# chto/linna

Hardware: AMD Instinct MI355X
Metric: emulator log-likelihood evals/sec (higher is better)
Workload: dtype f32; 1 GPU; 33-D Gaussian, 4x512 MLP emulator (33->512x4->33), nwalkers=4096 batched log-likelihood per GPU (BASELINE configs[1]); nwalkers_per_gpu=4096, launch=direct launches, parallelism=walkers sharded, 1 rank(s), no data-path collective

## Files before the change

### include/linna_hip.h

```cpp
#ifndef LINNA_HIP_H
#define LINNA_HIP_H
#include <stddef.h>
#include <stdint.h>

#ifdef __cplusplus
extern "C" {
#endif

#define LINNA_ABI_VERSION 12

typedef struct linna_ctx linna_ctx_t;
typedef struct linna_net linna_net_t;
typedef struct linna_logprob linna_logprob_t;
typedef struct linna_graph linna_graph_t;

int linna_abi_version(void);
const char* linna_last_error(void);
#define LINNA_OK 0
#define LINNA_ERR_INVALID (-1)
#define LINNA_ERR_HIP (-2)
#define LINNA_ERR_UNSUPPORTED (-3)
#define LINNA_ERR_INTERNAL (-4)
int linna_debug_raise(int kind);
int linna_ctx_create(int device, linna_ctx_t** out);
// ... 57 lines not shown
int linna_resblock_fwd(linna_ctx_t* ctx, const float* X, int ldx, const float* W1, const float* b1,
                       const float* W2, const float* b2, const float* Ws, float* T, int ldt,
                       float* Y, int ldy, int B, int K, int C, int N, void* stream);
int linna_linear_bwd(linna_ctx_t* ctx, const float* dY, int lddy, const float* X, int ldx,
                     const float* W, int ldw, float* dX, int lddx, const float* Xmask, int ldxm,
                     float* dW, int lddw, float* db, int B, int K, int N, float scale, void* stream);

#define LINNA_LD(k) (((k) + 3) & ~3)
#define LINNA_OP_LINEAR 0
#define LINNA_OP_RESBLOCK 1
#define LINNA_OP_INSKIP 2

typedef struct {
    uint32_t struct_size;
    int op;
    int K, C, N;
    int relu;
    float alpha;
    const float *W, *b;
    const float *W1, *b1, *W2, *b2, *Ws;
    float *gW, *gb, *gW1, *gb1, *gW2, *gb2, *gWs;
} linna_layer_t;

typedef struct {
    const float* cscale; const float* cshift;
    int cexp; const float* cpost; const float* cshift2;
} linna_colmap_t;

int linna_net_create(linna_ctx_t* ctx, const linna_layer_t* layers, int nlayers, int in_size,
                     linna_net_t** out);
int linna_net_destroy(linna_net_t* net);
int linna_net_prepare(linna_net_t* net, int backward, int input_grad);
size_t linna_net_fwd_ws_bytes(const linna_net_t* net, int B);
size_t linna_net_bwd_ws_bytes(const linna_net_t* net, int B);
int linna_net_forward(linna_net_t* net, const float* X, int ldx, int B, void* ws, float* OUT, int ldo,
                      const linna_colmap_t* outmap, void* stream);
int linna_net_backward(linna_net_t* net, const float* X, int ldx, int B, void* fwd_ws, void* bwd_ws,
                       const float* dOUT, int lddo, float* dX, int lddx, int param_grads, void* stream);
int linna_net_train_launches(const linna_net_t* net, int B);
int linna_net_set_train_precision(linna_net_t* net, int precision);
int linna_net_train_precision(const linna_net_t* net, int* out);
int linna_net_stream_state(const linna_net_t* net, int* fwd, int* dx, int* dx_input);

int linna_prior_map_fwd(linna_ctx_t* ctx, const float* Z, int ldz, int B, int nin, const int* is_flat,
                        const float* a1, const float* a2, const int* log10_flag, const float* xmean,
                        const float* xstd, float* X, int ldx, float* THETA, int ldt, void* stream);
int linna_prior_map_bwd(linna_ctx_t* ctx, const float* Z, int ldz, int B, int nin, const int* is_flat,
                        const float* a1, const float* a2, const int* log10_flag, const float* xstd,
                        const float* dX, int lddx, float* dZ, int lddz, void* stream);

int linna_gauss_loglike_diag(linna_ctx_t* ctx, const float* D, int ldd, int B, int nout, const float* w,
                             const float* Z, int ldz, int nin, float temperature, float* out,
                             void* stream);
int linna_gauss_loglike_dense(linna_ctx_t* ctx, const float* D, int ldd, int B, int nout,
                              const float* S, int lds, const float* Z, int ldz, int nin,
                              float temperature, float* scratch, float* out, void* stream);

typedef struct {
    uint32_t struct_size;
    int nin, nout;
    const int* is_flat; const float* a1; const float* a2;
    const int* log10_flag; const float* xmean; const float* xstd;
    linna_colmap_t outmap;
    const float* S; int lds;
    const float* Ssym;
    const float* w;
    const float* gscale;
    float temperature;
    const float* Sfac;
} linna_logprob_desc_t;

int linna_logprob_create(linna_ctx_t* ctx, linna_net_t* net, const linna_logprob_desc_t* desc,
                         linna_logprob_t** out);
int linna_logprob_destroy(linna_logprob_t* lp);
int linna_weights_changed(linna_ctx_t* ctx);
#define LINNA_PRECISION_FP32 0
#define LINNA_PRECISION_BF16 1
int linna_logprob_set_precision(linna_logprob_t* lp, int precision);
int linna_logprob_precision(const linna_logprob_t* lp, int* out);
int linna_logprob_set_grad_precision(linna_logprob_t* lp, int precision);
int linna_logprob_grad_precision(const linna_logprob_t* lp, int* out);
int linna_engine_rows(int rows);
int linna_dense_tri(int mode);
int linna_slice_fusion(int mask);
int linna_program_describe(const linna_layer_t* layers, int nlayers, int in_size, int rows, int dense_nout, char* buf,
                           size_t n);
int linna_program_describe_grad_bf16(const linna_layer_t* layers, int nlayers, int in_size, int rows, char* buf, size_t n);
size_t linna_logprob_ws_bytes(const linna_logprob_t* lp, int B, int with_grad);
int linna_logprob_eval(linna_logprob_t* lp, const float* Z, int ldz, int B, void* ws, float* lnP,
                       float* THETA, int ldt, void* stream);
int linna_logprob_eval_if(linna_logprob_t* lp, const float* Z, int ldz, int B, void* ws, float* lnP,
                          float* THETA, int ldt, const int* gate, void* stream);
int linna_logprob_eval_slice_points(linna_logprob_t* lp, const float* coords, int ldc, int ndim, const int* S_idx,
                                    int ns, const float* DIR, int ldd, const float* w, int nrep, float* lnP,
                                    const int* gate, void* stream);
int linna_logprob_grad(linna_logprob_t* lp, const float* Z, int ldz, int B, void* ws, float* lnP,
                       float* G, int ldg, void* stream);
int linna_logprob_grad_leapfrog(linna_logprob_t* lp, float* Q, int ldq, int B, void* ws, float* lnP, float* G, int ldg,
                                float* P, int ldp, const float* mass, float eps_kick, float eps_drift, void* stream);

typedef struct {
    uint32_t struct_size;
    int nout;
    const float* sigma; const float* ymean; const float* ystd;
    const float* data_norm;
    const float* Cinv; int ldc;
    int ylog;
} linna_loss_desc_t;

size_t linna_loss_scratch_bytes(int B, int nout);
int linna_chi2_md(linna_ctx_t* ctx, const linna_loss_desc_t* d, const float* Y, int ldy, int nrows,
                  float* scratch, float* den, void* stream);
int linna_chi2_ratio_loss_fwd_bwd(linna_ctx_t* ctx, const linna_loss_desc_t* d, const float* PRED,
                                  int ldp, const float* Y, int ldy, const float* den, const int* ROWS,
                                  int B, float* scratch, float* loss_rows, float* loss_mean,
                                  float* dPRED, int lddp, float inv_batch, void* stream);
int linna_net_prepare_loss(linna_net_t* net, const linna_loss_desc_t* d);
int linna_loss_targets(linna_ctx_t* ctx, const linna_loss_desc_t* d, const float* Y, int ldy, int nrows, float* YN, int ldyn,
                       void* stream);
int linna_net_forward_loss(linna_net_t* net, const linna_loss_desc_t* d, const float* X, int ldx, const int* ROWS, int B,
                           const int* log10_flag, const float* xmean, const float* xstd, float* XB, int ldxb, void* ws,
                           float* PRED, int ldp, const float* YN, int ldyn, const float* den, float inv_batch,
                           float* loss_rows, float* loss_mean, float* dPRED, int lddp,
                           float* hyper, int* step_dev, float beta1, float beta2, void* stream);
int linna_net_train_step(linna_net_t* net, const linna_loss_desc_t* d, const float* X, int ldx, const int* ROWS, int B,
                         const int* log10_flag, const float* xmean, const float* xstd, float* XB, int ldxb, void* fwd_ws,
                         float* PRED, int ldp, const float* YN, int ldyn, const float* den, float inv_batch,
                         float* loss_rows, float* loss_mean, float* dPRED, int lddp, void* bwd_ws,
                         float* hyper, int* step_dev, float beta1, float beta2, void* stream);
int linna_val_rows(linna_ctx_t* ctx, const linna_loss_desc_t* d, const float* PRED, int ldp,
                   const float* Y, int ldy, const float* den, int B, float* scratch, float* loss_rows,
                   float* frac_rows, void* stream);
int linna_val_metrics(linna_ctx_t* ctx, const float* loss_rows, const float* frac_rows, int n, const float* last_train_loss,
                      float* out, void* stream);
int linna_gather_xform(linna_ctx_t* ctx, const float* X, int ldx, const int* ROWS, int B, int nin,
                       const int* log10_flag, const float* xmean, const float* xstd, float* XB, int ldxb,
                       void* stream);
int linna_adamw_step(linna_ctx_t* ctx, float* p, const float* g, float* m, float* v, size_t n,
                     float* hyper, int* step_dev, float beta1, float beta2, float eps,
                     int prepared ,
                     void* stream);
int linna_net_adamw_step(linna_net_t* net, int B, float* p, const float* g, float* m, float* v, size_t n,
                         float* hyper, int* step_dev, float beta1, float beta2, float eps, int prepared, void* stream);
int linna_net_train_step_update(linna_net_t* net, const linna_loss_desc_t* d, const float* X, int ldx, const int* ROWS, int B,
                                const int* log10_flag, const float* xmean, const float* xstd, float* XB, int ldxb,
                                void* fwd_ws, float* PRED, int ldp, const float* YN, int ldyn, const float* den,
                                float inv_batch, float* loss_rows, float* loss_mean, float* dPRED, int lddp, void* bwd_ws,
                                float* params, float* m, float* v, size_t n, float* hyper, int* step_dev, float beta1,
                                float beta2, float eps, void* stream);

int linna_stretch_propose(linna_ctx_t* ctx, const float* coords, int ldc, int ndim, const int* S_idx,
                          int ns, const float* ccoords, int ldcc, const int* C_idx, int nc, uint64_t seed,
                          const int* step_dev, int stream_id, float a, float* Q, int ldq, float* factors,
                          void* stream);
int linna_stretch_accept(linna_ctx_t* ctx, float* coords, int ldc, int ndim, float* logp,
                         const int* S_idx, int ns, const float* Q, int ldq, const float* logp_new,
                         const float* factors, uint64_t seed, const int* step_dev, int stream_id,
                         int* naccept, void* stream);
int linna_stretch_half_step(linna_logprob_t* lp, float* coords, int ldc, int ndim, float* logp,
                            const int* S_idx, int ns, const float* ccoords, int ldcc, const int* C_idx,
                            int nc, uint64_t seed, const int* step_dev, int step_offset, int stream_id,
                            float a, int* naccept, void* stream);
int linna_hmc_init(linna_ctx_t* ctx, int B, int ndim, const float* mass, uint64_t seed,
                   const int* step_dev, const float* lnp, const float* P0, int ldp0, float* P, int ldp,
                   float* H0, void* stream);
int linna_hmc_start(linna_ctx_t* ctx, int B, int ndim, const float* mass, uint64_t seed, const int* step_dev,
// ... 102 lines not shown
```

### linna_amd/_lib.py

```python
import ctypes as C
import os

import torch

_HERE = os.path.dirname(os.path.abspath(__file__))
LIB_PATH = os.environ.get("LINNA_LIB_PATH") or os.path.join(_HERE, "liblinna_hip.so")
ABI_VERSION = 12

c_float_p = C.c_void_p
c_int_p = C.c_void_p


class _Sized(C.Structure):

    def __init__(self, *a, **k):
        C.Structure.__init__(self, *a, **k)
        self.struct_size = C.sizeof(type(self))


def sized_array(cls, n):
    arr = (cls * n)()
    for i in range(n):
        arr[i].struct_size = C.sizeof(cls)
    return arr
# ... 21 lines not shown
                ("gW", C.c_void_p), ("gb", C.c_void_p), ("gW1", C.c_void_p), ("gb1", C.c_void_p),
                ("gW2", C.c_void_p), ("gb2", C.c_void_p), ("gWs", C.c_void_p)]


class ColMap(C.Structure):
    _fields_ = [("cscale", C.c_void_p), ("cshift", C.c_void_p), ("cexp", C.c_int), ("cpost", C.c_void_p),
                ("cshift2", C.c_void_p)]


class LogprobDesc(_Sized):
    _fields_ = [("struct_size", C.c_uint32), ("nin", C.c_int), ("nout", C.c_int), ("is_flat", C.c_void_p), ("a1", C.c_void_p), ("a2", C.c_void_p),
                ("log10_flag", C.c_void_p), ("xmean", C.c_void_p), ("xstd", C.c_void_p), ("outmap", ColMap),
                ("S", C.c_void_p), ("lds", C.c_int), ("Ssym", C.c_void_p), ("w", C.c_void_p), ("gscale", C.c_void_p),
                ("temperature", C.c_float), ("Sfac", C.c_void_p)]


class HmcState(_Sized):
    _fields_ = [("struct_size", C.c_uint32), ("B", C.c_int), ("ld", C.c_int), ("seed", C.c_uint64), ("step_dev", C.c_void_p),
                ("mass", C.c_void_p), ("X", C.c_void_p), ("lnp", C.c_void_p), ("G", C.c_void_p), ("P", C.c_void_p),
                ("Q", C.c_void_p), ("lnp_new", C.c_void_p), ("Gnew", C.c_void_p), ("H0", C.c_void_p)]


class LossDesc(_Sized):
    _fields_ = [("struct_size", C.c_uint32), ("nout", C.c_int), ("sigma", C.c_void_p), ("ymean", C.c_void_p), ("ystd", C.c_void_p),
                ("data_norm", C.c_void_p), ("Cinv", C.c_void_p), ("ldc", C.c_int), ("ylog", C.c_int)]


OP_LINEAR, OP_RESBLOCK, OP_INSKIP = 0, 1, 2
COMM_ID_BYTES = 128
LAY_K, LAY_MN = 0, 1

_V, _I, _F, _SZ, _U64 = C.c_void_p, C.c_int, C.c_float, C.c_size_t, C.c_uint64
_I64, _D = C.c_int64, C.c_double
_PV = C.POINTER(C.c_void_p)

_SIGNATURES = {
    "linna_abi_version": (_I, []),
    "linna_last_error": (C.c_char_p, []),
    "linna_debug_raise": (_I, [_I]),
    "linna_ctx_create": (_I, [_I, _PV]),
    "linna_ctx_destroy": (_I, [_V]),
    "linna_stream_sync": (_I, [_V]),
    "linna_graph_begin": (_I, [_V]),
    "linna_graph_end": (_I, [_V, _PV]),
    "linna_graph_launch": (_I, [_V, _V]),
    "linna_graph_destroy": (_I, [_V]),
    "linna_event_create": (_I, [_PV]),
    "linna_event_record": (_I, [_V, _V]),
    "linna_event_elapsed_ms": (_I, [_V, _V, C.POINTER(C.c_float)]),
    "linna_event_destroy": (_I, [_V]),
    "linna_comm_unique_id": (_I, [_V]),
    "linna_comm_init": (_I, [_V, _I, _I, _V]),
    "linna_comm_destroy": (_I, [_V]),
    "linna_comm_info": (_I, [_V, C.POINTER(C.c_int), C.POINTER(C.c_int), C.POINTER(C.c_int)]),
    "linna_allreduce_sum_f32": (_I, [_V, _V, _SZ, _V]),
    "linna_allgather_f32": (_I, [_V, _V, _V, _SZ, _V]),
    "linna_broadcast_f32": (_I, [_V, _V, _SZ, _I, _V]),
    "linna_gemm_f32": (_I, [_V, C.POINTER(Gemm), _V]),
    "linna_gemm_dot_slots": (_I, [_I, _I]),
    "linna_linear_fwd": (_I, [_V, _V, _I, _V, _I, _V, _V, _I, _I, _I, _I, _I, _F, _V, _I, _V]),
    "linna_resblock_fwd": (_I, [_V, _V, _I, _V, _V, _V, _V, _V, _V, _I, _V, _I, _I, _I, _I, _I, _V]),
    "linna_linear_bwd": (_I, [_V, _V, _I, _V, _I, _V, _I, _V, _I, _V, _I, _V, _I, _V, _I, _I, _I, _F, _V]),
    "linna_net_create": (_I, [_V, C.POINTER(Layer), _I, _I, _PV]),
    "linna_net_destroy": (_I, [_V]),
    "linna_net_prepare": (_I, [_V, _I, _I]),
    "linna_net_fwd_ws_bytes": (_SZ, [_V, _I]),
    "linna_net_bwd_ws_bytes": (_SZ, [_V, _I]),
    "linna_net_forward": (_I, [_V, _V, _I, _I, _V, _V, _I, C.POINTER(ColMap), _V]),
    "linna_net_backward": (_I, [_V, _V, _I, _I, _V, _V, _V, _I, _V, _I, _I, _V]),
    "linna_net_stream_state": (_I, [_V, _V, _V, _V]),
    "linna_prior_map_fwd": (_I, [_V, _V, _I, _I, _I, _V, _V, _V, _V, _V, _V, _V, _I, _V, _I, _V]),
    "linna_prior_map_bwd": (_I, [_V, _V, _I, _I, _I, _V, _V, _V, _V, _V, _V, _I, _V, _I, _V]),
    "linna_gauss_loglike_diag": (_I, [_V, _V, _I, _I, _I, _V, _V, _I, _I, _F, _V, _V]),
    "linna_gauss_loglike_dense": (_I, [_V, _V, _I, _I, _I, _V, _I, _V, _I, _I, _F, _V, _V, _V]),
    "linna_logprob_create": (_I, [_V, _V, C.POINTER(LogprobDesc), _PV]),
    "linna_logprob_destroy": (_I, [_V]),
    "linna_weights_changed": (_I, [_V]),
    "linna_logprob_set_precision": (_I, [_V, _I]),
    "linna_logprob_precision": (_I, [_V, _V]),
    "linna_logprob_set_grad_precision": (_I, [_V, _I]),
    "linna_logprob_grad_precision": (_I, [_V, _V]),
    "linna_engine_rows": (_I, [_I]),
    "linna_dense_tri": (_I, [_I]),
    "linna_slice_fusion": (_I, [_I]),
    "linna_net_train_launches": (_I, [_V, _I]),
    "linna_net_set_train_precision": (_I, [_V, _I]),
    "linna_net_train_precision": (_I, [_V, _V]),
    "linna_program_describe": (_I, [_V, _I, _I, _I, _I, _V, C.c_size_t]),
    "linna_program_describe_grad_bf16": (_I, [_V, _I, _I, _I, _V, C.c_size_t]),
    "linna_logprob_ws_bytes": (_SZ, [_V, _I, _I]),
    "linna_logprob_eval": (_I, [_V, _V, _I, _I, _V, _V, _V, _I, _V]),
    "linna_logprob_grad": (_I, [_V, _V, _I, _I, _V, _V, _V, _I, _V]),
    "linna_logprob_grad_leapfrog": (_I, [_V, _V, _I, _I, _V, _V, _V, _I, _V, _I, _V, _F, _F, _V]),
    "linna_loss_scratch_bytes": (_SZ, [_I, _I]),
    "linna_chi2_md": (_I, [_V, C.POINTER(LossDesc), _V, _I, _I, _V, _V, _V]),
    "linna_chi2_ratio_loss_fwd_bwd": (_I, [_V, C.POINTER(LossDesc), _V, _I, _V, _I, _V, _V, _I, _V, _V, _V, _V, _I, _F, _V]),
    "linna_net_prepare_loss": (_I, [_V, C.POINTER(LossDesc)]),
    "linna_loss_targets": (_I, [_V, C.POINTER(LossDesc), _V, _I, _I, _V, _I, _V]),
    "linna_net_forward_loss": (_I, [_V, C.POINTER(LossDesc), _V, _I, _V, _I, _V, _V, _V, _V, _I, _V, _V, _I, _V, _I, _V, _F, _V, _V, _V, _I,
                                    _V, _V, _F, _F, _V]),
    "linna_net_train_step": (_I, [_V, C.POINTER(LossDesc), _V, _I, _V, _I, _V, _V, _V, _V, _I, _V, _V, _I, _V, _I, _V, _F, _V, _V, _V, _I,
                                  _V, _V, _V, _F, _F, _V]),
    "linna_net_train_step_update": (_I, [_V, C.POINTER(LossDesc), _V, _I, _V, _I, _V, _V, _V, _V, _I, _V, _V, _I, _V, _I, _V, _F, _V, _V, _V, _I,
                                         _V, _V, _V, _V, _SZ, _V, _V, _F, _F, _F, _V]),
    "linna_val_rows": (_I, [_V, C.POINTER(LossDesc), _V, _I, _V, _I, _V, _I, _V, _V, _V, _V]),
    "linna_val_metrics": (_I, [_V, _V, _V, _I, _V, _V, _V]),
    "linna_gather_xform": (_I, [_V, _V, _I, _V, _I, _I, _V, _V, _V, _V, _I, _V]),
    "linna_adamw_step": (_I, [_V, _V, _V, _V, _V, _SZ, _V, _V, _F, _F, _F, _I, _V]),
    "linna_net_adamw_step": (_I, [_V, _I, _V, _V, _V, _V, _SZ, _V, _V, _F, _F, _F, _I, _V]),
    "linna_stretch_propose": (_I, [_V, _V, _I, _I, _V, _I, _V, _I, _V, _I, _U64, _V, _I, _F, _V, _I, _V, _V]),
    "linna_stretch_accept": (_I, [_V, _V, _I, _I, _V, _V, _I, _V, _I, _V, _V, _U64, _V, _I, _V, _V]),
    "linna_logprob_eval_if": (_I, [_V, _V, _I, _I, _V, _V, _V, _I, _V, _V]),
    "linna_logprob_eval_slice_points": (_I, [_V, _V, _I, _I, _V, _I, _V, _I, _V, _I, _V, _V, _V]),
    "linna_stretch_half_step": (_I, [_V, _V, _I, _I, _V, _V, _I, _V, _I, _V, _I, _U64, _V, _I, _I, _F, _V, _V]),
    "linna_stretch_run": (_I, [_V, _V, _I, _I, _V, _I, _V, _I, _I, _U64, _V, _I, _F, _V, _V, _V, _V]),
    "linna_chain_append_t": (_I, [_V, _V, _I, _I, _I, _I, _I, _V, _I, _I64, _V]),
    "linna_acorr_update": (_I, [_V, _V, _I, _I, _I, _I64, _I64, _I64, _I64, _I, _I, _V, _V, _I, _V]),
    "linna_acorr_scratch_bytes": (_SZ, [_I, _I, _I]),
    "linna_acorr_tau": (_I, [_V, _V, _I, _I, _I, _I, _I64, _I64, _I, _V, _V, _D, _V, _V, _V]),
    "linna_chain_meanstd": (_I, [_V, _V, _I, _I, _I, _I64, _I64, _I64, _V, _V]),
    "linna_hmc_init": (_I, [_V, _I, _I, _V, _U64, _V, _V, _V, _I, _V, _I, _V, _V]),
    "linna_hmc_start": (_I, [_V, _I, _I, _V, _U64, _V, _V, _V, _I, _V, _I, _F, _F, _V, _I, _V, _I, _V, _I, _V, _V]),
    "linna_hmc_kick_drift": (_I, [_V, _I, _I, _V, _F, _F, _V, _I, _V, _I, _V, _I, _V]),
    "linna_hmc_accept": (_I, [_V, _I, _I, _V, _U64, _V, _V, _V, _I, _V, _I, _V, _V, _I, _V, _V, _I, _V, _V, _V, _V]),
    "linna_hmc_start_eps": (_I, [_V, _I, _I, _V, _U64, _V, _I, _V, _V, _I, _V, _I, _V, _F, _F, _V, _I, _V, _I, _V, _I, _V, _V]),
    "linna_hmc_kick_drift_eps": (_I, [_V, _I, _I, _V, _V, _F, _F, _V, _I, _V, _I, _V, _I, _V]),
    "linna_logprob_grad_leapfrog_eps": (_I, [_V, _V, _I, _I, _V, _V, _V, _I, _V, _I, _V, _V, _F, _F, _V]),
    "linna_hmc_accept_adapt": (_I, [_V, _I, _I, _V, _U64, _V, _I, _V, _V, _I, _V, _I, _V, _V, _I, _V, _V, _I, _V, _V, _V, _V,
                                    _V, _V, _V, _V, _V, _I, _F, _V, _V, _V]),
    "linna_hmc_run": (_I, [_V, _V, _V, _V, _V, _V, _V, _V, _I, _F, _I, _I, _I, _V, _V, _V, _V, _V]),
    "linna_hmc_find_epsilon": (_I, [_V, _V, _V, _V, _V, _V, _V, _I, _I, _V]),
    "linna_hmc_moments": (_I, [_V, _I, _I, _V, _I, _V, _V]),
    "linna_hmc_mass_from_moments": (_I, [_V, _I, _V, _V, _I, _V]),
    "linna_hmc_run_moments": (_I, [_V, _V, _V, _V, _V, _V, _V, _V, _I, _F, _I, _I, _I, _V, _V, _V, _V, _V, _V]),
    "linna_hmc_comoments_doubles": (_SZ, [_I]),
    "linna_hmc_comoments": (_I, [_V, _I, _I, _V, _I, _V, _V]),
    "linna_hmc_chol_from_comoments": (_I, [_V, _I, _V, _V, _I, _V, _I, _V]),
    "linna_hmc_kick_drift_dense": (_I, [_V, _I, _I, _V, _I, _V, _F, _F, _V, _I, _V, _I, _V, _I, _V, _I, _V]),
    "linna_hmc_run_dense": (_I, [_V, _V, _V, _V, _I, _V, _V, _V, _V, _V, _I, _F, _I, _I, _I, _V, _V, _V, _V, _V, _V]),
    "linna_hmc_find_epsilon_dense": (_I, [_V, _V, _V, _V, _I, _V, _V, _V, _V, _I, _I, _V]),
    "linna_step_increment": (_I, [_V, _V, _V]),
    "linna_slice_init": (_I, [_V, _V, _V, _I, _V, _I, _V, _I, _I, _V, _U64, _V, _I, _V, _I, _V, _V, _V, _V, _I, _V]),
    "linna_slice_points": (_I, [_V, _V, _I, _I, _V, _I, _V, _I, _V, _V, _I, _I, _V]),
    "linna_slice_expand": (_I, [_V, _V, _V, _V, _V, _V, _V, _I, _V, _I, _V]),
    "linna_slice_draw": (_I, [_V, _V, _V, _V, _V, _V, _I, _U64, _V, _I, _I, _I, _V]),
    "linna_slice_shrink": (_I, [_V, _V, _V, _V, _V, _V, _V, _V, _V, _I, _V, _I, _I, _V]),
    "linna_slice_commit": (_I, [_V, _V, _I, _I, _V, _V, _I, _V, _I, _V, _V, _V]),
    "linna_slice_half_step": (_I, [_V, _V, _I, _I, _V, _V, _I, _V, _I, _V, _I, _V, _U64, _V, _I, _V, _I, _V, _I, _V, _I, _V, _V, _V, _V, _V, _V, _V, _I, _I, _V, _I, _V]),
}
EXPORTED = tuple(_SIGNATURES)

_lib = None


class LinnaHipError(RuntimeError):
    pass


def load(missing_ok=False):
    global _lib
    if _lib is not None:
        return _lib
    if not os.path.exists(LIB_PATH):
        raise LinnaHipError("liblinna_hip.so not found at %s -- run `python -c 'import __graft_entry__ as g; g.build()'` "
                            "(hipcc --offload-arch=gfx950); there is no CPU fallback" % LIB_PATH)
    lib = C.CDLL(LIB_PATH)
# ... 45 lines not shown

def ptr(t, dtype=torch.float32):
    if t is None:
        return None
    if not t.is_cuda:
        raise LinnaHipError("expected a device tensor")
    if t.dtype != dtype:
        raise LinnaHipError("expected dtype %s, got %s" % (dtype, t.dtype))
    if not t.is_contiguous():
        raise LinnaHipError("expected a contiguous tensor")
    return C.c_void_p(t.data_ptr())


def iptr(t):
    return ptr(t, torch.int32)


def ld4(w):
    return (int(w) + 3) & ~3


class _Stage(object):
    __slots__ = ("name", "t0")

    def __init__(self, name):
        self.name = name

    def __enter__(self):
        if stage_profile.current is not None:
            import time
            self.t0 = time.perf_counter()
        return self

    def __exit__(self, *exc):
        d = stage_profile.current
        if d is not None:
            import time
            d[self.name] = d.get(self.name, 0.0) + time.perf_counter() - self.t0
        return False


def stage(name):
    return _Stage(name)


class stage_profile(object):
    current = None

    def __init__(self, d):
        self.d = d

    def __enter__(self):
        self.prev, stage_profile.current = stage_profile.current, self.d
        return self.d

    def __exit__(self, *exc):
        stage_profile.current = self.prev
        return False


class quiet_gc(object):

    def __enter__(self):
        import gc
        self.on = gc.isenabled() and os.environ.get("LINNA_QUIET_GC", "1") != "0"
        if self.on:
            gc.freeze()
        return self

    def __exit__(self, *exc):
        import gc
        if self.on:
            gc.unfreeze()
        return False


def slice_fusion(mask=-1):
    prev = load().linna_slice_fusion(int(mask))
    if prev < 0:
        check(prev)
    return prev


def engine_rows(rows=0):
    prev = load().linna_engine_rows(int(rows))
    if prev < 0:
        check(prev)
    return prev
```

### linna_amd/csrc/api.hip

```cpp
#include "common.h"

#include <stdarg.h>
#include <stdio.h>
#include <string.h>
#include <cstring>
#include <string>
#include <vector>
#include <atomic>
#include <new>
#include <stdlib.h>

namespace linna {

static thread_local std::string g_err;

void set_error(const char* fmt, ...) {
    char buf[512];
    va_list ap;
    va_start(ap, fmt);
    vsnprintf(buf, sizeof buf, fmt, ap);
    va_end(ap);
    g_err = buf;
}

// ... 820 lines not shown
    a.M = B; a.N = nout; a.dotwith = D; a.lddot = ldd; a.dot_partial = scratch; a.dot_slots = slots;
    if (cov.factored) a.flags |= LINNA_GEMM_DOT_SELF;
    TRY(gemm_launch(a, S(stream)));
    return launch_loglike_finish(scratch, slots, slots, B, Z, ldz, nin, T, out, S(stream));
}
int linna_gauss_loglike_dense(linna_ctx_t*, const float* D, int ldd, int B, int nout, const float* Sm, int lds,
                              const float* Z, int ldz, int nin, float T, float* scratch, float* out, void* stream) try {
    return loglike_dense_impl(D, ldd, B, nout, NsDense{Sm, lds, nullptr, nullptr}, Z, ldz, nin, T, scratch, out, stream);
} LINNA_CATCH_INT

}

struct linna_logprob {
    linna_ctx* ctx;
    linna_net* net;
    linna_logprob_desc_t d;
    StreamCopy packed;
    bool grad_fused = false;
    StreamCopy packed_g2;
    bool grad2 = false;
    bool dense_fused = false;
    bool fused_on = true;
    int dense_tri = 2;
    NsDense dense() const { return NsDense{d.Sfac ? d.Sfac : d.S, d.lds, d.outmap.cscale, d.outmap.cshift, d.Sfac ? 1 : 0, dense_tri}; }
    int precision = LINNA_PRECISION_FP32;
    StreamCopy packed_bf;
    bool bf16() const { return precision == LINNA_PRECISION_BF16; }
    int grad_precision = LINNA_PRECISION_FP32;
    StreamCopy packed_gbf;
    NsKind kind() const { return bf16() ? NS_SERVE_BF16 : dense_fused ? NS_SERVE_DENSE : NS_SERVE; }
};

struct LpLayout { size_t x0, fwd, d, part, dh, bwd, dx, total; int slots; };
static LpLayout lp_layout(const linna_logprob* lp, int B, int with_grad) {
    LpLayout L;
    size_t off = 0;
    auto take = [&](size_t nfloats) { size_t o = off; off += (nfloats + 3) & ~(size_t)3; return o; };
    L.x0 = take((size_t)B * ld4(lp->d.nin));
    L.fwd = take(linna_net_fwd_ws_bytes(lp->net, B) / sizeof(float));
    L.d = take((size_t)B * ld4(lp->d.nout));
    L.slots = gemm_slots(B, lp->d.nout);
    L.part = take((size_t)B * L.slots);
    L.dh = L.bwd = L.dx = 0;
    if (with_grad) {
        L.dh = take((size_t)B * ld4(lp->d.nout));
        L.bwd = take(linna_net_bwd_ws_bytes(lp->net, B) / sizeof(float));
        L.dx = take((size_t)B * ld4(lp->d.nin));
    }
    L.total = off;
    return L;
}

static int lp_refresh_stream(linna_logprob* lp, int B, void* stream, const float** packed, int* rows) {
    *rows = net_stream_rows(B);
    const NsDense dn = lp->dense();
    return stream_copy_refresh(lp->bf16() ? lp->packed_bf : lp->packed, lp->net, *rows, stream, packed, lp->kind(),
                               lp->kind() == NS_SERVE_DENSE ? &dn : nullptr);
}
static NsInput lp_input(const linna_logprob_desc_t& d) { return NsInput{d.nin, d.is_flat, d.a1, d.a2, d.log10_flag, d.xmean, d.xstd}; }
static NsOutput lp_output(const linna_logprob* lp) {
    const linna_logprob_desc_t& d = lp->d;
    if (lp->kind() == NS_SERVE_DENSE) return NsOutput{nullptr, nullptr, nullptr, nullptr, nullptr, d.temperature};
    return NsOutput{d.outmap.cscale, d.outmap.cshift, d.outmap.cexp ? d.outmap.cpost : nullptr, d.outmap.cexp ? d.outmap.cshift2 : nullptr,
                    d.w, d.temperature};
}
struct LpRun { const float* Z; int ldz; int B; float* lnP; const int* gate = nullptr; float* TH = nullptr; int ldt = 0; float* D = nullptr; int ldd = 0; };
static int lp_launch(const linna_logprob* lp, const float* packed, int rows, const LpRun& r, const NsMove* mv, const NsGrad* gr, void* stream) {
    const NsDense dn = lp->dense();
    return launch_net_stream(lp->kind(), net_layers(lp->net, lp->kind()), packed, r.Z, r.ldz, r.B, lp_input(lp->d), lp_output(lp), r.lnP, r.D,
                             r.ldd, r.TH, r.ldt, mv, gr, r.gate, rows, lp->kind() == NS_SERVE_DENSE ? &dn : nullptr, S(stream));
}
static bool lp_runs_fused_move(const linna_logprob* lp) {
    const linna_logprob_desc_t& d = lp->d;
    return lp->fused_on && (lp->bf16() ? lp->packed_bf.ready() : lp->packed.ready()) &&
           !(d.outmap.cexp && (!d.w || !d.outmap.cpost || !d.outmap.cshift2)) && (d.w || lp->dense_fused) && d.nin <= 64;
}
static int lp_likelihood(const linna_logprob* lp, const LpRun& r, float* w, const LpLayout& L, void* stream) {
    const linna_logprob_desc_t& d = lp->d;
    const int ldd = ld4(d.nout);
    if (d.w) return launch_loglike_diag(w + L.d, ldd, r.B, d.nout, d.w, r.Z, r.ldz, d.nin, d.temperature, r.lnP, S(stream));
    return loglike_dense_impl(w + L.d, ldd, r.B, d.nout, lp->dense(), r.Z, r.ldz, d.nin, d.temperature, w + L.part, r.lnP, stream);
}

static int lp_forward(linna_logprob* lp, const LpRun& r, float* w, const LpLayout& L, void* stream, bool keep_activations) {
    const linna_logprob_desc_t& d = lp->d;
    const int ldx = ld4(d.nin), ldd = ld4(d.nout), B = r.B;
    if (lp->bf16()) {
        if (keep_activations || !lp->fused_on || !lp->packed_bf.ready() || !d.w || (d.outmap.cexp && (!d.outmap.cpost || !d.outmap.cshift2))) {
            set_error("logprob: this bf16 log-probability cannot run the whole-network kernel here (LINNA_DISABLE_FUSED, or no diagonal likelihood)");
            return LINNA_ERR_UNSUPPORTED;
        }
        const float* packed = nullptr; int rows = 16;
        TRY(lp_refresh_stream(lp, B, stream, &packed, &rows));
        return lp_launch(lp, packed, rows, r, nullptr, nullptr, stream);
    }
    if (!keep_activations && lp->fused_on && lp->packed.ready() && (!d.outmap.cexp || (d.outmap.cpost && d.outmap.cshift2 && !lp->dense_fused))) {
        const float* packed = nullptr; int rows = 16;
        TRY(lp_refresh_stream(lp, B, stream, &packed, &rows));
        if (lp->dense_fused) return lp_launch(lp, packed, rows, r, nullptr, nullptr, stream);
        TRY(lp_launch(lp, packed, rows, LpRun{r.Z, r.ldz, B, d.w ? r.lnP : nullptr, r.gate, r.TH, r.ldt, d.w ? nullptr : w + L.d, ldd}, nullptr, nullptr, stream));
        return d.w ? LINNA_OK : lp_likelihood(lp, r, w, L, stream);
    }
    TRY(launch_prior_map_fwd(r.Z, r.ldz, B, d.nin, d.is_flat, d.a1, d.a2, d.log10_flag, d.xmean, d.xstd, w + L.x0, ldx, r.TH, r.ldt, S(stream)));
    TRY(linna_net_forward(lp->net, w + L.x0, ldx, B, w + L.fwd, w + L.d, ldd, &d.outmap, stream));
    return lp_likelihood(lp, r, w, L, stream);
}

extern "C" {

int linna_logprob_create(linna_ctx_t* ctx, linna_net_t* net, const linna_logprob_desc_t* desc, linna_logprob_t** out) try {
    if (!net || !desc || !out) { set_error("logprob_create: null argument"); return LINNA_ERR_INVALID; }
    CHECK_STRUCT(desc, linna_logprob_desc_t, "logprob_create");
    if (desc->nin != net->in_size || desc->nout != net->out_size) {
        set_error("logprob_create: network is %d->%d, descriptor says %d->%d", net->in_size, net->out_size, desc->nin, desc->nout);
        return LINNA_ERR_INVALID;
    }
    if (!desc->w && !desc->S) { set_error("logprob_create: need S (dense) or w (diagonal)"); return LINNA_ERR_INVALID; }
    if (!(desc->temperature > 0.f)) { set_error("logprob_create: temperature must be > 0"); return LINNA_ERR_INVALID; }
    linna_logprob* lp = new linna_logprob{ctx, net, *desc};
    lp->dense_tri = net_stream_dense_tri(-1);
    lp->fused_on = !env_is("LINNA_DISABLE_FUSED", '1');
    const NsDense dn = lp->dense();
    const bool want_dense = !desc->w && desc->S && !desc->outmap.cexp && !env_is("LINNA_DENSE_FUSED", '0');
    const NsPlan dense = want_dense ? net_stream_plan(NS_SERVE_DENSE, net->Lfull.data(), (int)net->Lfull.size(), net->in_size, &dn)
                                    : NsPlan{false, 0, false, nullptr};
    const NsPlan serve = net_stream_plan(NS_SERVE, net->Lfull.data(), (int)net->Lfull.size(), net->in_size);
    if (dense.ok) {
        lp->dense_fused = true;
        if (lp->packed.alloc(dense.packed_floats) != LINNA_OK) {
            set_error("logprob_create: hipMalloc(weight stream) failed");
            delete lp; return LINNA_ERR_HIP;
        }
    } else if (serve.ok) {
        lp->grad_fused = serve.grad_ok && !desc->outmap.cexp && !env_is("LINNA_DISABLE_FUSED_GRAD", '1');
        if (lp->packed.alloc(serve.packed_floats) != LINNA_OK) {
            set_error("logprob_create: hipMalloc(weight stream) failed");
            delete lp; return LINNA_ERR_HIP;
        }
    }
    if (!lp->grad_fused && desc->w && desc->gscale && !desc->outmap.cexp && !net->has_inskip && !env_is("LINNA_DISABLE_FUSED_GRAD", '1')) {
        const NsPlan g2 = net_stream_plan(NS_GRAD_INPUT, net->L.data(), (int)net->L.size(), net->in_size);
        if (g2.ok && lp->packed_g2.alloc(g2.packed_floats) == LINNA_OK) lp->grad2 = true;
    }
    *out = lp;
    return LINNA_OK;
} LINNA_CATCH_INT
int linna_logprob_destroy(linna_logprob_t* lp) try {
    if (lp) { lp->packed.release(); lp->packed_g2.release(); lp->packed_bf.release(); lp->packed_gbf.release(); }
    delete lp;
    return LINNA_OK;
} LINNA_CATCH_INT
int linna_weights_changed(linna_ctx_t*) try { g_weights_epoch.fetch_add(1); return LINNA_OK; } LINNA_CATCH_INT
int linna_logprob_set_precision(linna_logprob_t* lp, int precision) try {
    if (!lp) { set_error("logprob_set_precision: null handle"); return LINNA_ERR_INVALID; }
    TRY(check_precision(precision, "logprob_set_precision"));
    if (precision == LINNA_PRECISION_FP32) { lp->precision = precision; lp->grad_precision = LINNA_PRECISION_FP32; return LINNA_OK; }
    const linna_net* n = lp->net;
    if (!lp->d.w) { set_error("logprob_set_precision: bf16 needs a diagonal likelihood (a dense covariance is served in fp32 only)"); return LINNA_ERR_UNSUPPORTED; }
    const NsPlan bf = net_stream_plan(NS_SERVE_BF16, n->Lfull.data(), (int)n->Lfull.size(), n->in_size);
    if (!bf.ok) {
        set_error("logprob_set_precision: no bf16 engine for this network: %s", bf.why ? bf.why : "not eligible");
        return LINNA_ERR_UNSUPPORTED;
    }
    if (!lp->packed_bf.ready() && lp->packed_bf.alloc(bf.packed_floats) != LINNA_OK) {
        set_error("logprob_set_precision: hipMalloc(bf16 weight stream) failed");
        return LINNA_ERR_HIP;
    }
    lp->precision = precision;
    return LINNA_OK;
} LINNA_CATCH_INT
int linna_logprob_precision(const linna_logprob_t* lp, int* out) try {
    if (!lp || !out) { set_error("logprob_precision: null argument"); return LINNA_ERR_INVALID; }
    *out = lp->precision;
    return LINNA_OK;
} LINNA_CATCH_INT
int linna_logprob_set_grad_precision(linna_logprob_t* lp, int precision) try {
    if (!lp) { set_error("logprob_set_grad_precision: null handle"); return LINNA_ERR_INVALID; }
    TRY(check_precision(precision, "logprob_set_grad_precision"));
    if (precision == LINNA_PRECISION_FP32) { lp->grad_precision = precision; return LINNA_OK; }
    if (!lp->bf16()) {
        set_error("logprob_set_grad_precision: a bf16 gradient needs a bf16 handle (linna_logprob_set_precision first): lnP has one surface per handle");
        return LINNA_ERR_INVALID;
    }
    const linna_net* n = lp->net;
    if (lp->d.outmap.cexp) { set_error("logprob_set_grad_precision: no bf16 gradient: the ypositive (exp) output map has no gradient path"); return LINNA_ERR_UNSUPPORTED; }
    if (!lp->d.w || !lp->d.gscale) { set_error("logprob_set_grad_precision: no bf16 gradient: it needs a diagonal likelihood with gscale"); return LINNA_ERR_UNSUPPORTED; }
    const NsPlan g = net_stream_plan(NS_GRAD_INPUT_BF16, n->Lfull.data(), (int)n->Lfull.size(), n->in_size);
    if (!g.ok) {
        set_error("logprob_set_grad_precision: no bf16 gradient for this network: %s", g.why ? g.why : "not eligible");
        return LINNA_ERR_UNSUPPORTED;
    }
    if (!lp->packed_gbf.ready() && lp->packed_gbf.alloc(g.packed_floats) != LINNA_OK) {
        set_error("logprob_set_grad_precision: hipMalloc(bf16 gradient weight stream) failed");
        return LINNA_ERR_HIP;
    }
    lp->grad_precision = precision;
    return LINNA_OK;
} LINNA_CATCH_INT
int linna_logprob_grad_precision(const linna_logprob_t* lp, int* out) try {
    if (!lp || !out) { set_error("logprob_grad_precision: null argument"); return LINNA_ERR_INVALID; }
    *out = lp->grad_precision;
    return LINNA_OK;
} LINNA_CATCH_INT
int linna_program_describe_grad_bf16(const linna_layer_t* layers, int nlayers, int in_size, int rows, char* buf, size_t n) try {
    if (!layers || nlayers < 1 || !buf || !n) { set_error("program_describe_grad_bf16: bad arguments"); return LINNA_ERR_INVALID; }
    TRY(check_layers(layers, nlayers, "program_describe_grad_bf16"));
    return net_stream_describe(NS_GRAD_INPUT_BF16, layers, nlayers, in_size, nullptr, rows, buf, n);
} LINNA_CATCH_INT
int linna_program_describe(const linna_layer_t* layers, int nlayers, int in_size, int rows, int dense_nout, char* buf, size_t n) try {
    if (!layers || nlayers < 1 || !buf || !n) { set_error("program_describe: bad arguments"); return LINNA_ERR_INVALID; }
    TRY(check_layers(layers, nlayers, "program_describe"));
    static float dummy;
    if (dense_nout == -1) return net_stream_describe(NS_GRAD_INPUT, layers, nlayers, in_size, nullptr, rows, buf, n);
    const int dn_cols = dense_nout < -1 ? -dense_nout : dense_nout;
    NsDense dn{&dummy, (dn_cols + 3) & ~3, nullptr, nullptr, dense_nout < -1 ? 1 : 0, net_stream_dense_tri(-1)};
    if (dn_cols > 0) return net_stream_describe(NS_SERVE_DENSE, layers, nlayers, in_size, &dn, rows, buf, n);
    return net_stream_describe(NS_SERVE, layers, nlayers, in_size, nullptr, rows, buf, n);
} LINNA_CATCH_INT
int linna_dense_tri(int mode) try {
    if (mode < -1 || mode > 2) { set_error("linna_dense_tri: %d (-1 query, 0, 1 or 2)", mode); return LINNA_ERR_INVALID; }
    return net_stream_dense_tri(mode);
} LINNA_CATCH_INT
static std::atomic<int> g_slice_fusion{7};
static bool slice_derive_enabled() { return (g_slice_fusion.load() & 1) != 0; }
int linna_slice_fusion(int mode) try {
    if (mode < -1 || mode > 7) { set_error("linna_slice_fusion: %d (-1 query, or a mask of bits 0-2)", mode); return LINNA_ERR_INVALID; }
    return mode < 0 ? g_slice_fusion.load() : g_slice_fusion.exchange(mode);
} LINNA_CATCH_INT
int linna_engine_rows(int rows) try {
    const int prev = net_stream_force_rows(rows);
    if (prev < 0) { set_error("linna_engine_rows: %d (0, 4, 8 or 16)", rows); return LINNA_ERR_INVALID; }
    if (prev != rows) g_weights_epoch.fetch_add(1);
    return prev;
} LINNA_CATCH_INT
size_t linna_logprob_ws_bytes(const linna_logprob_t* lp, int B, int with_grad) try {
    return (lp_layout(lp, B, with_grad).total + 16) * sizeof(float);
} LINNA_CATCH_SIZE

int linna_logprob_eval(linna_logprob_t* lp, const float* Z, int ldz, int B, void* ws, float* lnP, float* TH, int ldt,
                       void* stream) try {
    if (!lp || !Z || !ws || !lnP || B < 1) { set_error("logprob_eval: bad arguments"); return LINNA_ERR_INVALID; }
    return lp_forward(lp, LpRun{Z, ldz, B, lnP, nullptr, TH, ldt}, static_cast<float*>(ws), lp_layout(lp, B, 0), stream, false);
} LINNA_CATCH_INT

int linna_logprob_eval_if(linna_logprob_t* lp, const float* Z, int ldz, int B, void* ws, float* lnP, float* TH, int ldt,
                          const int* gate, void* stream) try {
    if (!lp || !Z || !ws || !lnP || B < 1) { set_error("logprob_eval_if: bad arguments"); return LINNA_ERR_INVALID; }
    return lp_forward(lp, LpRun{Z, ldz, B, lnP, gate, TH, ldt}, static_cast<float*>(ws), lp_layout(lp, B, 0), stream, false);
} LINNA_CATCH_INT

struct SliceDerive { const float* Z0; const float* L; const float* R; const float* Ze; int m, nt; uint64_t seed; const int* step_dev; int stream_id; const int* flags; };
struct SlicePoints { const float* coords; int ldc, ndim; const int* S_idx; int ns; const float* DIR; int ldd; };
static int lp_eval_slice_points(linna_logprob_t* lp, const SlicePoints& pt, const float* w, int nrep, float* lnP, const int* gate,
                                const int* list, const int* count, int mul, int b_engine, void* stream, const SliceDerive* sd = nullptr,
                                const SliceBegin* sb = nullptr) {
    if (!lp || !pt.coords || !pt.S_idx || !pt.DIR || !w || !lnP || pt.ns < 1 || nrep < 1) {
        set_error("logprob_eval_slice_points: bad arguments"); return LINNA_ERR_INVALID;
    }
    if (pt.ndim != lp->d.nin) { set_error("logprob_eval_slice_points: ndim %d, log-probability has %d parameters", pt.ndim, lp->d.nin); return LINNA_ERR_INVALID; }
    if (!lp_runs_fused_move(lp)) {
        set_error("logprob_eval_slice_points: this log-probability does not run the whole-network kernel");
        return LINNA_ERR_UNSUPPORTED;
    }
    const float* packed = nullptr; int rows = 16;
    TRY(lp_refresh_stream(lp, b_engine > 0 ? b_engine : nrep * pt.ns, stream, &packed, &rows));
    NsMove mv{const_cast<float*>(pt.coords), pt.ldc, nullptr, pt.S_idx, w, 0, list, pt.ns, 0ull, count, mul, 0, 0.f, nullptr, 1};
    mv.sb = sb;
    if (sd) {
        mv.sl_Z0 = sd->Z0; mv.sl_L = sd->L; mv.sl_R = sd->R; mv.sl_Zt = sd->Ze; mv.sl_m = sd->m; mv.sl_nt = sd->nt;
        mv.sl_seed = sd->seed; mv.sl_step = sd->step_dev; mv.sl_stream = sd->stream_id; mv.sl_flags = sd->flags;
    }
    return lp_launch(lp, packed, rows, LpRun{pt.DIR, pt.ldd, nrep * pt.ns, lnP, gate}, &mv, nullptr, stream);
}
int linna_logprob_eval_slice_points(linna_logprob_t* lp, const float* coords, int ldc, int ndim, const int* S_idx, int ns,
                                    const float* DIR, int ldd, const float* w, int nrep, float* lnP, const int* gate,
                                    void* stream) try {
    return lp_eval_slice_points(lp, SlicePoints{coords, ldc, ndim, S_idx, ns, DIR, ldd}, w, nrep, lnP, gate, nullptr, nullptr, 0, 0, stream);
} LINNA_CATCH_INT

int linna_slice_half_step(linna_logprob_t* lp, float* coords, int ldc, int ndim, float* logp, const int* S_idx, int ns,
                          const float* ccoords, int ldcc, const int* C_idx, int nc, const float* mu, uint64_t seed,
                          int* step_dev, int half, const int* m_sched, int nexp_rounds, const int* nt_sched, int nshr_rounds,
                          float* DIR, int ldd, float* state, int* flags, float* W, float* Wd, float* Zt, int* list, int* counters,
                          int zero_totals, int bump_step, const int* expect_rows, int maxsteps, void* stream) try {
    if (!lp || !coords || !logp || !S_idx || !ccoords || !C_idx || !mu || !step_dev || !DIR || !state || !flags || !W || !Wd ||
        !Zt || !list || !counters || ns < 1 || nc < 2 || !m_sched || !nt_sched || nexp_rounds < 1 || nshr_rounds < 1 || (half != 0 && half != 1)) {
        set_error("slice_half_step: bad arguments"); return LINNA_ERR_INVALID;
    }
    if (maxsteps < 1) { set_error("slice_half_step: maxsteps %d < 1", maxsteps); return LINNA_ERR_INVALID; }
    for (int r = 0; r < nexp_rounds; ++r)
        if (m_sched[r] < 1 || m_sched[r] > 32) { set_error("slice_half_step: m_sched[%d] = %d (1 to 32 bracket ends per side)", r, m_sched[r]); return LINNA_ERR_INVALID; }
    for (int r = 0; r < nshr_rounds; ++r)
        if (nt_sched[r] < 1 || nt_sched[r] > 64) { set_error("slice_half_step: nt_sched[%d] = %d (1 to 64 trials)", r, nt_sched[r]); return LINNA_ERR_INVALID; }
    if (ndim != lp->d.nin) { set_error("slice_half_step: ndim %d, log-probability has %d parameters", ndim, lp->d.nin); return LINNA_ERR_INVALID; }
    if (!lp_runs_fused_move(lp)) {
        set_error("slice_half_step: this log-probability does not run the whole-network kernel");
        return LINNA_ERR_UNSUPPORTED;
    }
    float* const Z0 = state; float* const L = state + ns; float* const R = state + 2 * ns;
    float* const Wacc = state + 3 * ns; float* const Zacc = state + 4 * ns;
// ... 610 lines not shown
```

### linna_amd/csrc/common.h

```cpp
#pragma once
#include <hip/hip_runtime.h>
#include <stdint.h>
#include <exception>
#include "../../include/linna_hip.h"


typedef float f32x4 __attribute__((ext_vector_type(4)));
typedef float f32x16 __attribute__((ext_vector_type(16)));

namespace linna {

struct U4 { uint32_t x, y, z, w; };
__device__ __forceinline__ U4 philox4x32_10(U4 c, uint32_t k0, uint32_t k1) {
#pragma unroll
    for (int r = 0; r < 10; ++r) {
        const uint64_t p0 = (uint64_t)0xD2511F53u * c.x;
        const uint64_t p1 = (uint64_t)0xCD9E8D57u * c.z;
        U4 n;
        n.x = (uint32_t)(p1 >> 32) ^ c.y ^ k0;
        n.y = (uint32_t)p1;
        n.z = (uint32_t)(p0 >> 32) ^ c.w ^ k1;
        n.w = (uint32_t)p0;
        c = n;
        k0 += 0x9E3779B9u; k1 += 0xBB67AE85u;
// ... 201 lines not shown
                            float* dP, int lddp, unsigned* counter, hipStream_t s);
int launch_loss_rows(int mode, const float* partial, int slots_ld, int nslots, int B, const float* den, const int* ROWS,
                     float floorv, float* out, hipStream_t s);
int launch_loss_grad(const float* U, int ldu, const float* Y, int ldy, const int* ROWS, int B, int nout,
                     const float* data_norm, const float* den, float inv_batch, float* dP, int lddp, hipStream_t s);
int launch_sum_scale(const float* v, int n, float scale, float* out, hipStream_t s);
int launch_sum_scale_prepare(const float* v, int n, float scale, float* out, int* step_dev, float* hyper, float b1, float b2,
                             hipStream_t s);
int launch_val_frac(const float* partial, int slots_ld, int nslots, int B, const float* den, float* frac, hipStream_t s);
int launch_val_metrics(const float* loss, const float* frac, int n, const float* last, float* out, hipStream_t s);
int launch_gather_xform(const float* X, int ldx, const int* ROWS, int B, int nin, const int* lg, const float* xmean,
                        const float* xstd, float* XB, int ldxb, hipStream_t s);
int launch_colsum(const float* dZ, int ld, int B, int N, float scale, float* db, hipStream_t s);
int launch_adamw(float* p, const float* g, float* m, float* v, size_t n, float* hyper, int* step_dev, float b1, float b2,
                 float eps, hipStream_t s);
int launch_adamw_prepare(float* hyper, int* step_dev, float b1, float b2, hipStream_t s);
int launch_stretch_propose(const float* coords, int ldc, int ndim, const int* S, int ns, const float* ccoords, int ldcc,
                           const int* C, int nc, uint64_t seed, const int* step_dev, int stream_id, float a, float* Q,
                           int ldq, float* factors, hipStream_t s);
int launch_stretch_accept(float* coords, int ldc, int ndim, float* logp, const int* S, int ns, const float* Q, int ldq,
                          const float* lp_new, const float* factors, uint64_t seed, const int* step_dev, int stream_id,
                          int* naccept, hipStream_t s);
int launch_hmc_start(int B, int ndim, const float* mass, uint64_t seed, const int* step_dev, const float* lnp, const float* P0,
                     int ldp0, const float* G, int ldg, float ek, float ed, const float* X, int ldx, float* P, int ldp, float* Q,
                     int ldq, float* H0, hipStream_t s, const float* eps = nullptr, int step_off = 0);
int launch_hmc_kick_drift(int B, int ndim, const float* mass, float ek, float ed, const float* G, int ldg, float* P,
                          int ldp, float* Q, int ldq, hipStream_t s, const float* eps = nullptr);
struct HmcAdapt { float* eps; float* epsbar; float* Hbar; const float* mu; int* m; int Madapt; float delta; };
int launch_hmc_accept(int B, int ndim, const float* mass, uint64_t seed, const int* step_dev, int step_off, const float* H0,
                      const float* P, int ldp, const float* Qn, int ldq, const float* lnp_new, const float* Gn, int ldg,
                      const float* U, float* X, int ldx, float* lnp, float* G, int* naccept, float* alpha,
                      const HmcAdapt& ad, float* chain, float* logps, hipStream_t s);
int launch_hmc_find_eps_init(int B, int ndim, uint64_t seed, const int* step_dev, int step_off, float* R0, int ldr, float* eps,
                             int* state, hipStream_t s);
int launch_hmc_find_eps(int B, int ndim, const float* mass, const float* H0, const float* P, int ldp, const float* lnp_new,
                        const float* Gn, int ldg, float* eps, int* state, int* nactive, hipStream_t s);
int launch_hmc_moments(int B, int ndim, const float* X, int ldx, double* mom, hipStream_t s);
int launch_hmc_mass_from_moments(int ndim, double* mom, float* mass, int reset, hipStream_t s);
int launch_hmc_comoments(int B, int ndim, const float* X, int ldx, double* mom, hipStream_t s);
int launch_hmc_chol_from_comoments(int ndim, double* mom, float* Cm, int ldc, int* info, int reset, hipStream_t s);
int launch_hmc_kick_drift_dense(int B, int ndim, const float* Cm, int ldc, const float* eps, float ek, float ed, const float* G,
                                int ldg, float* W, int ldw, const float* X, int ldx, float* Q, int ldq, hipStream_t s);
int launch_slice_points(const float* coords, int ldc, int ndim, const int* S, int ns, const float* DIR, int ldd,
                        const float* w, float* Q, int ldq, int nrep, hipStream_t s);
int launch_slice_expand(const float* Z0, const float* ZL, const float* ZR, float* L, float* R, int* flags, int ns,
                        int* counters, int slot, hipStream_t s);
int launch_slice_draw(const float* L, const float* R, const int* S, float* W, const int* flags, int ns, uint64_t seed,
                      const int* step_dev, int stream_id, int round, int ntrial, hipStream_t s);
int launch_slice_shrink(const float* Z0, const float* Zt, float* L, float* R, const float* W, int* flags, float* Wacc,
                        float* Zacc, int ns, int* counters, int slot, int ntrial, hipStream_t s);
int launch_slice_begin(const SliceBegin& b, const int* S, int ns, int ndim, float* W, hipStream_t s);
int launch_slice_expand_multi(const float* Z0, const float* Zt, float* L, float* R, const int* S, int* flags, int ns, int m,
                              int m_next, int* counters, int slot, int prev_slot, float* W, float* Wd, int* list, uint64_t seed,
                              const int* step_dev, int stream_id_shrink, int ntrial, hipStream_t s);
int launch_slice_shrink_multi(const SliceRound& a, hipStream_t s);
int launch_slice_commit(float* coords, int ldc, int ndim, float* logp, const int* S, int ns, const float* DIR, int ldd,
                        const float* Wacc, const float* Zacc, hipStream_t s);
int launch_step_increment(int* step, hipStream_t s);

struct NsDense { const float* S; int lds; const float* cscale; const float* cshift; int factored = 0;
                 int tri = 2; };
int net_stream_dense_tri(int mode);
enum NsKind {
    NS_SERVE,
    NS_SERVE_DENSE,
    NS_SERVE_BF16,
    NS_STORE,
    NS_TRAIN_FWD,
    NS_DX,
    NS_DX_INPUT,
    NS_GRAD_INPUT,
    NS_TRAIN_STEP,
    NS_TRAIN_STEP_BF16,
    NS_GRAD_INPUT_BF16,
};
inline bool ns_kind_full_layers(NsKind k) { return k == NS_SERVE || k == NS_SERVE_DENSE || k == NS_SERVE_BF16; }
struct NsPlan { bool ok; size_t packed_floats; bool grad_ok; const char* why; };
NsPlan net_stream_plan(NsKind kind, const linna_layer_t* layers, int nl, int in_size, const NsDense* dn = nullptr);
int net_stream_rows(int B);
int net_stream_force_rows(int rows);
int launch_net_stream_pack(NsKind kind, const linna_layer_t* layers, int nl, int in_size, float* packed, int rows, const NsDense* dn,
                           hipStream_t s);
int net_stream_describe(NsKind kind, const linna_layer_t* layers, int nl, int in_size, const NsDense* dn, int rows, char* buf, size_t n);
struct NsNet { const linna_layer_t* layers; int nl, in_size; };
struct NsInput { int nin; const int* is_flat; const float* a1; const float* a2; const int* lg; const float* xmean; const float* xstd; };
struct NsOutput { const float* cscale; const float* cshift; const float* cpost; const float* cshift2; const float* w; float T; };
struct NsOpBufs { float* y; int ldy; float* t; int ldt; const float* x; int ldx; const float* gate; float* dprev; int ldp; float* dt; int lddt; };
struct NsPost { const float* rows; int n; float scale; float* out; int* step; float* hyper; float b1, b2; };
int launch_net_stream_dx(const NsNet& net, const float* packed, const float* dOUT, int lddo, int B, const NsOpBufs* ops, int with_input,
                         int rows, hipStream_t s, const NsPost* post = nullptr);
struct NsMove {
    float* coords; int ldc; float* logp; const int* S;
    const float* cc; int ldcc; const int* C; int nc;
    unsigned long long seed; const int* step; int step_off; int stream; float a; int* naccept;
    int slice;
    float* chain = nullptr; float* lps = nullptr;
    const float* sl_Z0 = nullptr; const float* sl_L = nullptr; const float* sl_R = nullptr; const float* sl_Zt = nullptr;
    int sl_m = 0, sl_nt = 0; unsigned long long sl_seed = 0; const int* sl_step = nullptr; int sl_stream = 0;
    const int* sl_flags = nullptr;
    const SliceBegin* sb = nullptr;
};
int launch_net_stream_store(const NsNet& net, const float* packed, const float* X, int ldx, int B, const NsOpBufs* ops,
                            const float* cscale, const float* cshift, int rows, hipStream_t s);
struct NsTrainLoss { const float* YN; int ldyn;
                     const float* den; float inv_batch; float* loss_rows; float* dP; int lddp; };
struct NsBatch { const float* X; int ldx; const int* ROWS; int B; const int* lg; const float* xmean; const float* xstd; float* XB; int ldxb; };
int launch_loss_targets(const float* Y, int ldy, int n, const linna_loss_desc_t& d, float* YN, int ldyn, hipStream_t s);
int launch_net_stream_train(const NsNet& net, const float* packed, const NsBatch& b, const NsOpBufs* ops, const NsTrainLoss& L,
                            const NsDense& dn, int rows, hipStream_t s);
int launch_net_stream_train_bwd(const NsNet& net, const float* packed, const NsBatch& b, const NsOpBufs* ops, const NsTrainLoss& L,
                                const NsDense& dn, int rows, hipStream_t s, const NsPost* post,
                                bool bf = false);
struct NsLeap { float* P; int ldp; float* Q; const float* mass; float ek, ed; const float* eps; };
struct NsGrad { const float* gscale; float* G; int ldg; NsLeap leap; };
constexpr int AS_MAXR = 26, AS_MAXW = 14, AS_MAXB = 12;
struct AsPlace { float* out; float scale; int trans, koff, ncols, type, ncg, steps, G, first0, first1; };
struct AsMat { int N, ld; AsPlace pl[2]; };
struct AsBias { float* out; float scale; int N; };
struct AsRange { unsigned off4, n4, blk0; short kind, idx; };
struct AsArgs { AsRange r[AS_MAXR]; AsMat w[AS_MAXW]; AsBias b[AS_MAXB]; int nr, small; unsigned nblocks; };
__device__ __forceinline__ size_t as_slot(const AsPlace& q, int small, int nn, int kk) {
    const int nl = nn & 63, ks = kk >> 4, kr = kk & 15;
    int w, g;
    if (q.type == 0) { w = (nn & 511) >> 6; g = ((nn >> 9) ? q.first1 : q.first0) + ks; }
    else { const int kp = ks / q.steps; w = kp * q.ncg + (nn >> 6); g = q.first0 + (ks - kp * q.steps); }
    const int t = small ? kr >> 2 : nl >> 4, lane = small ? nl : (nl & 15) + 16 * (kr >> 2);
    return ((((size_t)w * q.G + g) * 4 + t) * 64 + lane) * 4 + (kr & 3);
}
__device__ __forceinline__ size_t as_slot_bf16(const AsPlace& q, int nn, int kk) {
    const int nl = nn & 63, ks = kk >> 5, kr = kk & 31;
    int w, g;
    if (q.type == 0) { w = (nn & 511) >> 6; g = ((nn >> 9) ? q.first1 : q.first0) + ks; }
    else { const int kp = ks / q.steps; w = kp * q.ncg + (nn >> 6); g = q.first0 + (ks - kp * q.steps); }
    return ((((size_t)w * q.G + g) * 4 + (kr >> 3)) * 64 + nl) * 8 + (kr & 7);
}
typedef __bf16 bf16x4_t __attribute__((ext_vector_type(4)));
__device__ __forceinline__ void adamw_one(float& pi, float gi, float& mi, float& vi, float lr, float wd, float bc1, float sbc2,
                                          float beta1, float beta2, float eps) {
    pi = pi * (1.f - lr * wd);
    mi = mi + (gi - mi) * (1.f - beta1);
    vi = vi * beta2 + (1.f - beta2) * gi * gi;
    const float denom = sqrtf(vi) / sbc2 + eps;
    pi = pi - (lr / bc1) * (mi / denom);
}
int net_stream_adamw_args(const linna_layer_t* layers, int nl, int in_size, int rows, const float* params, size_t nflat,
                          float* s_fwd, const NsDense* dn, float* s_dx, AsArgs* out, int merged = 0);
int launch_adamw_streams(const AsArgs& a, float* p, const float* g, float* m, float* v, const float* hyper, float b1, float b2,
                         float eps, hipStream_t s, bool bf = false);
int launch_net_stream_grad2(const NsNet& net, const float* packed, const float* Z, int ldz, int B, const NsInput& in, const NsOutput& out,
                            float* lnP, const NsGrad& gr, int rows, hipStream_t s, bool bf = false);
int launch_net_stream(NsKind kind, const NsNet& net, const float* packed, const float* Z, int ldz, int B, const NsInput& in,
                      const NsOutput& out, float* lnP, float* D, int ldd, float* TH, int ldt, const NsMove* mv, const NsGrad* gr,
                      const int* gate, int rows, const NsDense* dn, hipStream_t s);

int launch_chain_append_t(const float* block, int ldb, int nsteps, int nw, int ndim, int wstride, float* CT, int nwp,
                          int64_t row0, hipStream_t s);
int launch_acorr_update(const float* CT, int nd, int nwp, int nwc, int64_t a0, int64_t a1, int64_t lo, int64_t hi, int k0, int k1,
                        double* S, double* T, int remove, hipStream_t s);
size_t acorr_scratch_doubles(int nser, int kuse, int nd);
int launch_acorr_tau(const float* CT, int ndim, int nwp, int nwc, int nlive, int64_t lo, int64_t hi, int kuse, const double* S,
                     const double* T, double c, double* scratch, double* out, hipStream_t s);
int launch_chain_meanstd(const float* CT, int ndim, int nwp, int nws, int64_t t0, int64_t tm, int64_t t1, double* out,
                         hipStream_t s);

int gemm_slots(int M, int N);
int gemm_launch(const GemmArgs& a, hipStream_t stream);
struct GemmGroupProb { const float* A; const float* B; float* C; float* db; int lda, ldb, ldc, K, M, N; float alpha; int first; };
constexpr int GEMM_GROUP_MAX = 48;
struct GemmGroupArgs { GemmGroupProb p[GEMM_GROUP_MAX]; int nprob; };
constexpr int GEMM_UPD_MAX = 16;
struct GemmGroupArgsS { GemmGroupProb p[GEMM_UPD_MAX]; int nprob; };
struct GemmUpdate { long long pdiff, mdiff, vdiff;
                    const float* hyper; float beta1, beta2, eps; int small;
                    AsPlace pl[GEMM_UPD_MAX][2]; AsBias bias[GEMM_UPD_MAX]; };
struct GemmUpd1 { long long pdiff, mdiff, vdiff; const float* hyper; float beta1, beta2, eps; int small; AsPlace pl[2]; AsBias bias; };
struct GemmPost { const float* rows; int n; float scale; float* out; };
int gemm_launch_group_update(const GemmGroupArgsS& g, const GemmUpdate& u, int nblocks, hipStream_t stream, const GemmPost* post = nullptr,
                             bool bf = false);
bool gemm_group_ok(const GemmArgs& a);
int gemm_group_blocks(const GemmArgs& a);
int gemm_launch_group(const GemmGroupArgs& g, int nblocks, hipStream_t stream, const GemmPost* post = nullptr);

}
```

### linna_amd/csrc/net_program.h

```cpp
#pragma once
#include "common.h"
#include <memory>
#include <vector>

namespace linna {

constexpr int NS_ROWS = 16;
constexpr int NS_NW = 8;
constexpr int NS_NT = 4;
constexpr int NS_MAXSEG = 20;
constexpr int NS_MAXRUN = 40;
constexpr unsigned NS_STEP_B = NS_NT * 1024;
constexpr int NS_LDS_BYTES = 160 * 1024;
constexpr int AS_BLOCK = 64;
enum { NS_WIDE = 0, NS_SPLIT = 1, NS_SIDE = 2 };

struct NsSeg {
    int type, steps, passes, bias_off;
    int dst_col, relu, kslice, zext;
    int ncg_log2;
    int mask_store, mask_apply;
    int x0_n;
    int x0_col;
    int kcl, side_off;
};

struct NsPackSeg {
    const float* Wa; int lda, Ka, Kapad;
    const float* Wb; int ldb, Kb; float alpha;
    const float* b; float bscale;
    const float* b2; float b2scale;
    int N, type, steps, passes, bias_off, bias_pad, ncg;
    int transA;
    int transB;
    const float* rscale; const float* rshift;
    int kc, side_off;
    int koff2;
};

struct NsProgram {
    std::vector<NsPackSeg> pack;
    std::vector<NsSeg> seg;
    int G = 0, LD = 0, kpad0 = 0, nout = 0, bias_total = 0;
    int Gstride = 0, nseg_f = 0, mask_slots = 0;
    size_t packed_floats = 0;
    int dense = 0, u_col = 0, u_same = 0;
    int x0_keep = 0;
    size_t side_f4 = 0;
    bool bf = false;
    int f32seg = -1;
    bool ok = false, grad_ok = false;
    bool dxi_ok = false;
    bool train_ok = false;
    std::vector<int> seg_op, seg_hidden;
    size_t lds_for(int rows, bool grad) const;
};

int ns_seg_steps(const NsSeg& s);
int ns_forced_rows_resolved();
typedef std::shared_ptr<const NsProgram> NsProgramRef;
NsProgramRef ns_program(NsKind kind, const linna_layer_t* layers, int nl, int in_size, const NsDense* dn, int rows);

int ns_seg_cols(const NsProgram& p, const linna_layer_t* layers, int i);
struct NsGates {
    int gbit[NS_MAXSEG], mbit[NS_MAXSEG];
    int ncols = 0;
    bool ok = true;
    size_t lds0 = 0, lds = 0;
};
NsGates ns_gates(const NsProgram& p, const linna_layer_t* layers, int nl, int rows);
}
```

### linna_amd/csrc/net_program.hip

```cpp
#include "net_program.h"
#include <stdlib.h>
#include <algorithm>
#include <atomic>
#include <cstring>
#include <mutex>
#include <string>
#include <unordered_map>

namespace linna {

size_t NsProgram::lds_for(int rows, bool grad) const {
    size_t b = (size_t)(2 * rows * LD + ((bias_total + 3) & ~3)) * sizeof(float) + 128 + (x0_keep ? 4096 : 0);
#ifdef NS_STAMPS
    b += NS_NW * 32 * 8;
#endif
    return b + (grad ? (size_t)mask_slots * 64 * NS_NW * sizeof(unsigned) : 0);
}

static int ceil16(int k) { return (k + 15) & ~15; }
int ns_seg_steps(const NsSeg& s) {
    if (s.type == NS_WIDE && s.zext < 0) return 2 * s.steps - 60;
    return s.type == NS_WIDE && s.zext > 0 ? s.steps + (s.passes - 1) * s.zext : s.steps * s.passes;
}
static int ns_switch(std::atomic<int>& sw, const char* name, int dflt, bool (*valid)(int)) {
// ... 296 lines not shown
    NsLowered lo = ns_lower(layers, nl, in_size, o, dn);
    p.x0_keep = lo.x0_keep; p.dense = lo.dense; p.u_col = lo.u_col; p.u_same = lo.u_same;
    if (!lo.ok) return p;
    const int nfwd = lo.nfwd;
    int x0_seg = -1;
    for (int i = 0; i < (int)lo.lins.size(); ++i) if (lo.lins[i].x0_col) x0_seg = i;
    const NsShapeCtx ctx{o, o.dense ? dn : nullptr, nfwd, lo.f32seg, o.forward && !lo.mlp_grad && o.bwd != NS_BWD_INPUT && o.bwd != NS_BWD_TRAIN, x0_seg};
    NsShaper sh;
    for (const Lin& L : lo.lins) if (!ns_shape(sh, L, ctx)) return p;
    const int slots = lo.mlp_grad ? ns_append_mlp_grad(sh, lo.lins, ctx) : -1;
    p.seg = std::move(sh.seg); p.pack = std::move(sh.pack);
    int maxext = 0;
    if (!ns_written_columns(p, sh.in_ext, &maxext)) return p;
    if (p.kpad0 > (!o.forward ? 1024 : o.bf ? 512 : 256)) return p;
    p.bf = o.bf; p.f32seg = lo.f32seg;
    p.nout = lo.lins[nfwd - 1].N;
    p.Gstride = sh.G; p.nseg_f = nfwd; p.grad_ok = slots >= 0; p.mask_slots = std::max(slots, 0);
    for (int i = 0; i < nfwd; ++i) if (p.seg[i].type != NS_SIDE) p.G += ns_seg_steps(p.seg[i]);
    for (const Lin& L : lo.lins) { p.seg_op.push_back(L.op); p.seg_hidden.push_back(L.same_buf ? 1 : 0); }
    p.dxi_ok = o.bwd == NS_BWD_INPUT;
    p.train_ok = o.bwd == NS_BWD_TRAIN;
    p.bias_total = sh.bias_off;
    p.ok = ns_sizes(p, maxext);
    return p;
}

static std::atomic<int> g_forced_rows{-1};
int ns_forced_rows_resolved() { return ns_switch(g_forced_rows, "LINNA_NS_ROWS", 0, [](int v) { return v == 4 || v == 8 || v == 16; }); }
int net_stream_force_rows(int rows) {
    if (rows != 0 && rows != 4 && rows != 8 && rows != 16) return -1;
    (void)ns_forced_rows_resolved();
    return g_forced_rows.exchange(rows);
}

static bool ns_side(NsKind kind, int rows) {
    return rows == 16 && (kind == NS_SERVE || kind == NS_SERVE_DENSE || kind == NS_GRAD_INPUT);
}

static NsProgram ns_build_kind(NsKind kind, const linna_layer_t* layers, int nl, int in_size, const NsDense* dn, bool side) {
    NsBuildOpts o;
    o.side = side;
    switch (kind) {
    case NS_SERVE: case NS_STORE: o.bwd = NS_BWD_MLP; break;
    case NS_SERVE_DENSE: case NS_TRAIN_FWD: o.dense = true; break;
    case NS_SERVE_BF16: o.bf = true; if (dn) return NsProgram(); break;
    case NS_DX: o.forward = false; break;
    case NS_DX_INPUT: o.forward = false; o.dx_first = 0; break;
    case NS_GRAD_INPUT: o.bwd = NS_BWD_INPUT; break;
    case NS_GRAD_INPUT_BF16: o.bwd = NS_BWD_INPUT; o.bf = true; if (dn) return NsProgram(); break;
    case NS_TRAIN_STEP: case NS_TRAIN_STEP_BF16: o.dense = true; o.bwd = NS_BWD_TRAIN; o.bf = kind == NS_TRAIN_STEP_BF16; break;
    }
    NsProgram p = ns_build_one(layers, nl, in_size, o, dn);
    if (!p.ok && o.bwd == NS_BWD_MLP) {
        o.bwd = NS_BWD_NONE;
        p = ns_build_one(layers, nl, in_size, o, dn);
    }
    if (side && !(p.ok && (kind != NS_GRAD_INPUT || p.dxi_ok))) return ns_build_kind(kind, layers, nl, in_size, dn, false);
    return p;
}
NsProgramRef ns_program(NsKind kind, const linna_layer_t* layers, int nl, int in_size, const NsDense* dn, int rows) {
    static std::mutex mu;
    static std::unordered_map<std::string, NsProgramRef> cache;
    const bool side = ns_side(kind, rows);
    std::string key;
    key.reserve((size_t)nl * sizeof(linna_layer_t) + 64);
    key.append(reinterpret_cast<const char*>(layers), (size_t)nl * sizeof(linna_layer_t));
    const int hdr[4] = {nl, in_size, (int)kind, side ? 1 : 0};
    key.append(reinterpret_cast<const char*>(hdr), sizeof(hdr));
    if (dn) {
        const void* const ptrs[3] = {dn->S, dn->cscale, dn->cshift};
        key.append(reinterpret_cast<const char*>(ptrs), sizeof(ptrs));
        key.append(reinterpret_cast<const char*>(&dn->lds), sizeof(int));
        key.append(reinterpret_cast<const char*>(&dn->factored), sizeof(int));
        key.append(reinterpret_cast<const char*>(&dn->tri), sizeof(int));
    }
    std::lock_guard<std::mutex> lock(mu);
    auto it = cache.find(key);
    if (it != cache.end()) return it->second;
    if (cache.size() >= 256) cache.clear();
    NsProgramRef p = std::make_shared<const NsProgram>(ns_build_kind(kind, layers, nl, in_size, dn, side));
    cache.emplace(std::move(key), p);
    return p;
}

int ns_seg_cols(const NsProgram& p, const linna_layer_t* layers, int i) {
    const linna_layer_t& l = layers[p.seg_op[i]];
    return p.seg_hidden[i] ? l.C : i < p.nseg_f ? l.N : l.K;
}
NsGates ns_gates(const NsProgram& p, const linna_layer_t* layers, int nl, int rows) {
    NsGates g;
    for (int i = 0; i < NS_MAXSEG; ++i) g.gbit[i] = g.mbit[i] = -1;
    for (int i = 0; i < p.nseg_f; ++i) {
        const int op = p.seg_op[i];
        if (op >= nl || (!p.seg_hidden[i] && op == nl - 1)) continue;
        g.gbit[i] = g.ncols;
        g.ncols += (ns_seg_cols(p, layers, i) + 63) & ~63;
    }
    for (int i = p.nseg_f; i < (int)p.seg.size(); ++i) {
        const int op = p.seg_op[i];
        const bool hidden = p.seg_hidden[i] != 0;
        if (!hidden && !(op > 0 && (layers[op - 1].op == LINNA_OP_RESBLOCK || layers[op - 1].relu))) continue;
        const int src = hidden ? op : op - 1;
        for (int j = 0; j < p.nseg_f; ++j)
            if (p.seg_op[j] == src && (p.seg_hidden[j] != 0) == hidden) g.mbit[i] = g.gbit[j];
        if (g.mbit[i] < 0) g.ok = false;
    }
    g.lds0 = (p.lds_for(rows, true) + 7) & ~(size_t)7;
    g.lds = g.lds0 + (size_t)rows * (g.ncols / 32) * sizeof(unsigned);
    return g;
}

static const char* ns_bf16_refusal(const NsProgram& p, const linna_layer_t* layers, int nl, int in_size) {
    int width = 0;
    for (int i = 0; i < nl; ++i) width = std::max(width, std::max(layers[i].N, layers[i].op == LINNA_OP_RESBLOCK ? layers[i].C : 0));
    if (in_size > 256) return "more than 256 network inputs: outside the whole-network kernel";
    if (width > 1024) return "a layer wider than 1024: outside the whole-network kernel";
    if (nl < 1 || layers[0].op != LINNA_OP_LINEAR) return "the first op is not a linear layer (the bf16 input split needs one)";
    if (!p.ok) return "the network does not fit the bf16 program of the whole-network kernel";
    return nullptr;
}
NsPlan net_stream_plan(NsKind kind, const linna_layer_t* layers, int nl, int in_size, const NsDense* dn) {
    const NsProgramRef pref = ns_program(kind, layers, nl, in_size, dn, 0);
    const NsProgram& p = *pref;
    NsPlan r{p.ok, p.packed_floats, p.grad_ok, nullptr};
    if (kind == NS_TRAIN_STEP) r.ok = p.ok && p.train_ok;
    if (kind == NS_TRAIN_STEP_BF16) {
        r.why = ns_bf16_refusal(p, layers, nl, in_size);
        if (!r.why && !p.train_ok) r.why = "the network has no merged training step (one layer only)";
        r.ok = r.why == nullptr;
    }
    if (kind == NS_GRAD_INPUT) {
        r.ok = p.ok && p.dxi_ok && ns_gates(p, layers, nl, NS_ROWS).lds <= (size_t)NS_LDS_BYTES;
        r.packed_floats = std::max(r.packed_floats, ns_program(kind, layers, nl, in_size, dn, 16)->packed_floats);
    }
    if (kind == NS_SERVE_BF16) { r.why = ns_bf16_refusal(p, layers, nl, in_size); r.ok = r.why == nullptr; }
    if (kind == NS_GRAD_INPUT_BF16) {
        bool inskip = false;
        for (int i = 0; i < nl; ++i) inskip = inskip || layers[i].op == LINNA_OP_INSKIP;
        if (inskip) r.why = "an input-skip network has no one-launch gradient";
        else if (in_size > 64 || (nl >= 1 && layers[nl - 1].N > 64)) r.why = "more than 64 network inputs or outputs: outside the one-launch gradient";
        else r.why = ns_bf16_refusal(p, layers, nl, in_size);
        if (!r.why && !p.dxi_ok) r.why = "the network has no forward + dX program";
        if (!r.why && ns_gates(p, layers, nl, NS_ROWS).lds > (size_t)NS_LDS_BYTES) r.why = "the sign bits of the one-launch gradient do not fit the LDS";
        r.ok = r.why == nullptr;
    }
    return r;
}

int net_stream_describe(NsKind kind, const linna_layer_t* layers, int nl, int in_size, const NsDense* dn, int rows, char* buf, size_t n) {
    const NsProgramRef pref = ns_program(kind, layers, nl, in_size, dn, rows);
    const NsProgram& p = *pref;
    std::string out = p.ok ? "ok" : "not eligible";
    char line[160];
    snprintf(line, sizeof line, " G %d Gstride %d nseg_f %d LD %d kpad0 %d packed_floats %zu grad %d\n", p.G, p.Gstride, p.nseg_f, p.LD,
             p.kpad0, p.packed_floats, (int)p.grad_ok);
    out += line;
    for (size_t i = 0; p.ok && i < p.seg.size(); ++i) {
        const NsSeg& g = p.seg[i];
        snprintf(line, sizeof line, "%s steps %d passes %d ncg %d kc %d dst %d zext %d N %d\n",
                 g.type == NS_WIDE ? "WIDE" : g.type == NS_SPLIT ? "SPLIT" : "SIDE", g.steps, g.passes, 1 << g.ncg_log2, 1 << g.kcl, g.dst_col,
                 g.zext, p.pack[i].N);
        out += line;
    }
    if (p.ok && (kind == NS_GRAD_INPUT || kind == NS_GRAD_INPUT_BF16)) {
        const NsGates g = ns_gates(p, layers, nl, NS_ROWS);
        snprintf(line, sizeof line, "lds %zu of %d bytes with %d sign-bit columns: %s\n", g.lds, NS_LDS_BYTES, g.ncols,
// ... 104 lines not shown
```

### linna_amd/csrc/net_stream.hip

```cpp
#include "net_program.h"
#include <stdlib.h>
#include <type_traits>
#include <cstring>
#include <algorithm>

namespace linna {

typedef __bf16 bf16x8 __attribute__((ext_vector_type(8)));
typedef short s16x4 __attribute__((ext_vector_type(4)));

#ifndef NS_R
#define NS_R 6
#endif
#ifndef NS_PRE
#define NS_PRE 2
#endif
struct NsArgs {
    const float* Z; int ldz; int B; int nin;
    const int* is_flat; const float* a1; const float* a2; const int* lg;
    const float* xmean; const float* xstd;
    const float* packed;
    int G, nseg, LD, kpad0, nout, bias_total;
    int Gstride, nseg_f;
    const float* gscale; float* Gout; int ldg;
// ... 78 lines not shown
        const int g = (int)(q % p.G);
        const int w = (int)(q / p.G);
        int r = 0;
        while (r + 1 < p.nrun && g >= p.run_first[r + 1]) ++r;
        const NsPackSeg& S = p.seg[p.run_seg[r]];
        const int s = g - p.run_first[r];
        const int nl = p.small ? lane : 16 * t + (lane & 15), kl = p.small ? 4 * t : 4 * (lane >> 4);
        int n, k0;
        if (S.type == NS_WIDE && S.koff2 < 0) {
            const int n0 = S.steps - 4 * w, blk = s < n0 ? w : 15 - w;
            n = 64 * blk + nl; k0 = 16 * (s < n0 ? s : s - n0) + 64 * blk + kl;
        } else if (S.type == NS_WIDE) { n = 512 * p.run_pass[r] + 64 * w + nl; k0 = 16 * s + kl + (p.run_pass[r] ? S.koff2 : 0); }
        else { n = 64 * (w % S.ncg) + nl; k0 = 16 * ((w / S.ncg) * S.steps + s) + kl; }
        f32x4 v = {0.f, 0.f, 0.f, 0.f};
        if (n < S.N && S.Wa && !S.transA && k0 + 3 < S.Ka && (S.lda & 3) == 0 && (reinterpret_cast<uintptr_t>(S.Wa) & 15) == 0) {
            v = *reinterpret_cast<const f32x4*>(S.Wa + (size_t)n * S.lda + k0);
            if (S.rscale) { const float r = S.rscale[n]; v = f32x4{v[0] * r, v[1] * r, v[2] * r, v[3] * r}; }
        } else if (n < S.N) {
#pragma unroll
            for (int e = 0; e < 4; ++e) {
                const int k = k0 + e;
                if (k < S.Kapad) {
                    if (k < S.Ka) v[e] = !S.Wa ? (k == n ? 1.f : 0.f) : S.transA ? S.Wa[(size_t)k * S.lda + n] : S.Wa[(size_t)n * S.lda + k];
                } else if (k - S.Kapad < S.Kb) {
                    v[e] = S.alpha * (S.transB ? S.Wb[(size_t)(k - S.Kapad) * S.ldb + n] : S.Wb[(size_t)n * S.ldb + (k - S.Kapad)]);
                }
            }
            if (S.rscale) { const float r = S.rscale[n]; v = f32x4{v[0] * r, v[1] * r, v[2] * r, v[3] * r}; }
        }
        reinterpret_cast<f32x4*>(p.out)[idx] = v;
        return;
    }
    const size_t j = idx - nw4;
    if (j >= (size_t)p.bias_total) return;
    int si = 0;
    while (si + 1 < p.nseg && (int)j >= p.seg[si + 1].bias_off) ++si;
    const NsPackSeg& S = p.seg[si];
    const int c = (int)j - S.bias_off;
    float bv = (c < S.N && S.b) ? S.bscale * S.b[c] : 0.f;
    if (c < S.N && S.b2) bv += S.b2scale * S.b2[c];
    if (c < S.N && S.rscale) bv *= S.rscale[c];
    if (c < S.N && S.rshift) bv += S.rshift[c];
    p.out[nw4 * 4 + j] = bv;
}

__global__ void ns_pack_side_kernel(NsPackArgs p) {
    const size_t idx = (size_t)blockIdx.x * blockDim.x + threadIdx.x;
    size_t base = 0;
    for (int si = 0; si < p.nseg; ++si) {
        const NsPackSeg& S = p.seg[si];
        if (S.type != NS_SIDE) continue;
        const size_t n4 = (size_t)NS_NW * S.steps * NS_NT * 64;
        if (idx >= base + n4) { base += n4; continue; }
        size_t q = idx - base;
        const int lane = (int)(q & 63); q >>= 6;
        const int t = (int)(q % NS_NT); q /= NS_NT;
        const int st = (int)(q % S.steps);
        const int w = (int)(q / S.steps);
        const int tpc = NS_NT / S.kc;
        const int n = 16 * (t % tpc) + (lane & 15);
        const int k0 = 16 * (S.kc * (w * S.steps + st) + t / tpc) + 4 * (lane >> 4);
        f32x4 v = {0.f, 0.f, 0.f, 0.f};
        if (n < S.N) {
#pragma unroll
            for (int e = 0; e < 4; ++e) {
                const int k = k0 + e;
                if (S.Wa) { if (k < S.Ka) v[e] = S.Wa[(size_t)n * S.lda + k]; }
                else if (k < S.Kb) v[e] = S.alpha * (S.transB ? S.Wb[(size_t)k * S.ldb + n] : S.Wb[(size_t)n * S.ldb + k]);
            }
        }
        reinterpret_cast<f32x4*>(p.out + S.side_off)[idx - base] = v;
        return;
    }
}

__device__ __forceinline__ float ns_prior_theta(float z, int flat, float a1, float a2) {
    float u = 0.5f * (1.f + erff(z / 1.41421356237309515f));
    asm volatile("" : "+v"(u));
    return (flat ? u : z) * a2 + a1;
}

template <int R, int MOVE, bool GRAD, int STORE, int ROWS, bool BF = false>
__global__ __launch_bounds__(64 * NS_NW, 1) void net_stream_kernel(NsArgs a) {
    constexpr bool EPS = false;
#include "net_stream_body.inc"
}
template <int R, int MOVE, bool GRAD, int STORE, int ROWS, bool BF>
__global__ __launch_bounds__(64 * NS_NW, 1) void net_stream_eps_kernel(NsArgs a) {
    static_assert(!BF && GRAD && (STORE == 0 || STORE == 2) && MOVE == 0, "the fp32 one-launch gradients only");
    constexpr bool EPS = true;
#include "net_stream_body.inc"
}
template <int R, int MOVE, bool GRAD, int STORE, int ROWS, bool BF>
__global__ __launch_bounds__(64 * NS_NW, 1) void net_stream_train_bf16_kernel(NsArgs a) {
    static_assert(BF && GRAD && STORE == 3 && ROWS == 4 && MOVE == 0, "the bf16 training step only");
    constexpr bool EPS = false;
#include "net_stream_body.inc"
}
template <int R, int MOVE, bool GRAD, int STORE, int ROWS, bool BF>
__global__ __launch_bounds__(64 * NS_NW, 1) void net_stream_slice_bf16_kernel(NsArgs a) {
    static_assert(BF && !GRAD && STORE == 0 && MOVE == 2, "the bf16 slice evaluation only");
    constexpr bool EPS = false;
#define NS_BODY_SLICE_BF16
#include "net_stream_body.inc"
#undef NS_BODY_SLICE_BF16
}
template <int R, int MOVE, bool GRAD, int STORE, int ROWS, bool BF>
__global__ __launch_bounds__(64 * NS_NW, 1) void net_stream_grad_bf16_kernel(NsArgs a) {
    static_assert(BF && GRAD && STORE == 2 && MOVE == 0, "the bf16 one-launch gradient only");
    constexpr bool EPS = false;
#define NS_BODY_GRAD_BF16
#include "net_stream_body.inc"
#undef NS_BODY_GRAD_BF16
}
template <int R, int MOVE, bool GRAD, int STORE, int ROWS, bool BF>
__global__ __launch_bounds__(64 * NS_NW, 1) void net_stream_eps_bf16_kernel(NsArgs a) {
    static_assert(BF && GRAD && STORE == 2 && MOVE == 0, "the bf16 one-launch gradient only");
    constexpr bool EPS = true;
#define NS_BODY_GRAD_BF16
#include "net_stream_body.inc"
#undef NS_BODY_GRAD_BF16
}

int net_stream_rows(int B) {
    const int forced = ns_forced_rows_resolved();
    if (forced) return forced;
    static int ncu = 0;
    if (!ncu) {
        int dev = 0; hipDeviceProp_t pr;
        ncu = (hipGetDevice(&dev) == hipSuccess && hipGetDeviceProperties(&pr, dev) == hipSuccess && pr.multiProcessorCount > 0)
                  ? pr.multiProcessorCount : 256;
    }
    return B <= 4 * ncu ? 4 : B <= 8 * ncu ? 8 : 16;
}

int launch_net_stream_pack(NsKind kind, const linna_layer_t* layers, int nl, int in_size, float* packed, int rows, const NsDense* dn,
                           hipStream_t s) {
    const NsProgramRef pref = ns_program(kind, layers, nl, in_size, dn, rows);
    const NsProgram& p = *pref;
    if (!p.ok) { set_error("net_stream: network not eligible"); return LINNA_ERR_UNSUPPORTED; }
    NsPackArgs a;
    ::memset(static_cast<void*>(&a), 0, sizeof(a));
    a.nseg = (int)p.seg.size(); a.G = p.Gstride; a.bias_total = p.bias_total; a.out = packed;
    a.small = rows < 16;
    a.bf = p.bf ? 1 : 0; a.f32seg = p.f32seg;
    int nrun = 0, first = 0;
    for (int i = 0; i < a.nseg; ++i) {
        a.seg[i] = p.pack[i];
        if (p.seg[i].type == NS_SIDE) continue;
        if (p.seg[i].type == NS_WIDE && p.seg[i].zext < 0) {
            a.run_seg[nrun] = i; a.run_pass[nrun] = 0; a.run_first[nrun] = first;
            first += ns_seg_steps(p.seg[i]); ++nrun;
            continue;
        }
        for (int ps = 0; ps < p.seg[i].passes; ++ps) {
            a.run_seg[nrun] = i; a.run_pass[nrun] = ps; a.run_first[nrun] = first;
            first += (ps > 0 && p.seg[i].type == NS_WIDE && p.seg[i].zext > 0) ? p.seg[i].zext : p.seg[i].steps; ++nrun;
        }
    }
    a.run_first[nrun] = first; a.nrun = nrun;
    const size_t total = (size_t)NS_NW * p.Gstride * NS_NT * 64 + (size_t)p.bias_total;
    hipLaunchKernelGGL(ns_pack_kernel, dim3((unsigned)((total + 255) / 256)), dim3(256), 0, s, a);
    if (p.side_f4) hipLaunchKernelGGL(ns_pack_side_kernel, dim3((unsigned)((p.side_f4 + 255) / 256)), dim3(256), 0, s, a);
    return check_hip(hipGetLastError(), "net_stream pack launch");
}

template <void (*Kernel)(NsArgs)>
static int ns_launch(const NsArgs& a, int nblocks, size_t lds_bytes, hipStream_t s, const char* what) {
    static bool attr_set = false;
    if (!attr_set) {
        const int rc = check_hip(hipFuncSetAttribute(reinterpret_cast<const void*>(Kernel), hipFuncAttributeMaxDynamicSharedMemorySize, NS_LDS_BYTES),
                                 "hipFuncSetAttribute");
        if (rc != LINNA_OK) return rc;
        attr_set = true;
    }
    hipLaunchKernelGGL(Kernel, dim3(nblocks), dim3(64 * NS_NW), lds_bytes, s, a);
    return check_hip(hipGetLastError(), what);
}
template <int MOVE, bool GRAD, int STORE, int ROWS, bool BF = false, bool EPS = false>
static int ns_launch_rows(const NsArgs& a, int B, size_t lds_bytes, hipStream_t s, int extra = 0) {
    if constexpr (EPS) return ns_launch<net_stream_eps_kernel<NS_R, MOVE, GRAD, STORE, ROWS, BF>>(a, (B + ROWS - 1) / ROWS + extra, lds_bytes, s, "net_stream launch");
    else return ns_launch<net_stream_kernel<NS_R, MOVE, GRAD, STORE, ROWS, BF>>(a, (B + ROWS - 1) / ROWS + extra, lds_bytes, s, "net_stream launch");
}
template <int MOVE, bool GRAD, int STORE = 0, bool BF = false, bool EPS = false>
static int ns_launch_kernel(const NsArgs& a0, int B, const NsProgram& p, int rows, hipStream_t s, int extra = 0, size_t lds_extra = 0) {
    const size_t lds = p.lds_for(rows, GRAD) + lds_extra;
#ifdef NS_STAMPS
    NsArgs a = a0;
    a.stamps = getenv("LINNA_FUSED_STAMPS") ? reinterpret_cast<unsigned long long*>(strtoull(getenv("LINNA_FUSED_STAMPS"), nullptr, 16)) : nullptr;
    if (!a.stamps) { set_error("net_stream: NS_STAMPS build needs LINNA_FUSED_STAMPS"); return LINNA_ERR_INVALID; }
#else
    const NsArgs& a = a0;
#endif
    if (rows == 4) return ns_launch_rows<MOVE, GRAD, STORE, 4, BF, EPS>(a, B, lds, s, extra);
    if constexpr (BF) {
        if (rows == 8) return ns_launch_rows<MOVE, GRAD, STORE, 8, BF, EPS>(a, B, lds, s, extra);
        if (rows == 16) return ns_launch_rows<MOVE, GRAD, STORE, 16, BF, EPS>(a, B, lds, s, extra);
    } else if constexpr (STORE == 3 && GRAD) {
    } else {
        if (rows == 8) return ns_launch_rows<MOVE, GRAD, STORE, 8, false, EPS>(a, B, lds, s, extra);
        if (rows == 16) return ns_launch_rows<MOVE, GRAD, STORE, 16, false, EPS>(a, B, lds, s, extra);
    }
    set_error("net_stream: %d rows per workgroup", rows);
    return LINNA_ERR_INVALID;
}
template <int ROWS>
static int ns_launch_slice_bf16_rows(const NsArgs& a, int B, size_t lds_bytes, hipStream_t s) {
    return ns_launch<net_stream_slice_bf16_kernel<NS_R, 2, false, 0, ROWS, true>>(a, (B + ROWS - 1) / ROWS, lds_bytes, s, "net_stream bf16 slice launch");
}
static int ns_launch_slice_bf16(const NsArgs& a, int B, const NsProgram& p, int rows, hipStream_t s) {
#ifdef NS_STAMPS
    set_error("net_stream: the NS_STAMPS build has no bf16 slice evaluation"); return LINNA_ERR_UNSUPPORTED;
#endif
    const size_t lds = p.lds_for(rows, false);
    if (rows == 4) return ns_launch_slice_bf16_rows<4>(a, B, lds, s);
    if (rows == 8) return ns_launch_slice_bf16_rows<8>(a, B, lds, s);
    if (rows == 16) return ns_launch_slice_bf16_rows<16>(a, B, lds, s);
    set_error("net_stream: %d rows per workgroup", rows);
    return LINNA_ERR_INVALID;
}

__device__ __forceinline__ void as_update(f32x4& P4, const f32x4& G4, f32x4& M4, f32x4& V4, float lr, float wd, float bc1,
                                          float sbc2, float beta1, float beta2, float eps) {
#pragma unroll
    for (int e = 0; e < 4; ++e) {
        const float gi = G4[e];
        float pi = P4[e] * (1.f - lr * wd);
        float mi = M4[e];
        mi = mi + (gi - mi) * (1.f - beta1);
        const float vi = V4[e] * beta2 + (1.f - beta2) * gi * gi;
        const float denom = sqrtf(vi) / sbc2 + eps;
        pi = pi - (lr / bc1) * (mi / denom);
        P4[e] = pi; M4[e] = mi; V4[e] = vi;
    }
}

template <bool BF = false>
__global__ __launch_bounds__(AS_BLOCK) void adamw_streams_kernel(AsArgs a, float* __restrict__ p, const float* __restrict__ g,
                                                            float* __restrict__ m, float* __restrict__ v,
                                                            const float* __restrict__ hyper, float beta1, float beta2, float eps) {
    int ri = 0;
    while (ri + 1 < a.nr && blockIdx.x >= a.r[ri + 1].blk0) ++ri;
    const AsRange R = a.r[ri];
    const unsigned it = (blockIdx.x - R.blk0) * AS_BLOCK + threadIdx.x;
    if (it >= R.n4) return;
    const float lr = hyper[0], wd = hyper[1], bc1 = hyper[2], sbc2 = hyper[3];
    if (R.kind == 1) {
        const size_t i = ((size_t)R.off4 + it) * 4;
        const f32x4 G4 = *reinterpret_cast<const f32x4*>(g + i);
        f32x4 P4 = *reinterpret_cast<const f32x4*>(p + i), M4 = *reinterpret_cast<const f32x4*>(m + i), V4 = *reinterpret_cast<const f32x4*>(v + i);
        as_update(P4, G4, M4, V4, lr, wd, bc1, sbc2, beta1, beta2, eps);
        *reinterpret_cast<f32x4*>(p + i) = P4; *reinterpret_cast<f32x4*>(m + i) = M4; *reinterpret_cast<f32x4*>(v + i) = V4;
        const AsBias B = a.b[R.idx];
        if (B.out) {
#pragma unroll
            for (int e = 0; e < 4; ++e)
                if ((int)(4 * it) + e < B.N) B.out[4 * it + e] = B.scale * P4[e];
        }
        return;
    }
    const AsMat& W = a.w[R.idx];
    const unsigned ld4 = (unsigned)W.ld >> 2;
    const int n0 = 4 * (int)(it / ld4), k0 = 4 * (int)(it % ld4);
    f32x4 P4[4], G4[4], M4[4], V4[4];
#pragma unroll
    for (int r = 0; r < 4; ++r) {
        const size_t i = (size_t)R.off4 * 4 + (size_t)min(n0 + r, W.N - 1) * W.ld + k0;
        G4[r] = *reinterpret_cast<const f32x4*>(g + i); P4[r] = *reinterpret_cast<const f32x4*>(p + i);
        M4[r] = *reinterpret_cast<const f32x4*>(m + i); V4[r] = *reinterpret_cast<const f32x4*>(v + i);
    }
#pragma unroll
    for (int r = 0; r < 4; ++r) {
        as_update(P4[r], G4[r], M4[r], V4[r], lr, wd, bc1, sbc2, beta1, beta2, eps);
        if (n0 + r < W.N) {
            const size_t i = (size_t)R.off4 * 4 + (size_t)(n0 + r) * W.ld + k0;
            *reinterpret_cast<f32x4*>(p + i) = P4[r]; *reinterpret_cast<f32x4*>(m + i) = M4[r]; *reinterpret_cast<f32x4*>(v + i) = V4[r];
// ... 3 lines not shown
    }
#pragma unroll
    for (int j = 0; j < 2; ++j) {
        const AsPlace& q = W.pl[j];
        if (!q.out) continue;
        if constexpr (BF) {
            __bf16* const ob = reinterpret_cast<__bf16*>(q.out);
            if (!q.trans) {
#pragma unroll
                for (int r = 0; r < 4; ++r)
#pragma unroll
                    for (int e = 0; e < 4; ++e)
                        if (n0 + r < W.N && k0 + e < q.ncols) ob[as_slot_bf16(q, n0 + r, q.koff + k0 + e)] = (__bf16)(q.scale * P4[r][e]);
            } else {
#pragma unroll
                for (int e = 0; e < 4; ++e)
                    if (k0 + e < q.ncols)
                        *reinterpret_cast<bf16x4_t*>(ob + as_slot_bf16(q, k0 + e, q.koff + n0)) =
                            bf16x4_t{(__bf16)(q.scale * P4[0][e]), (__bf16)(q.scale * P4[1][e]), (__bf16)(q.scale * P4[2][e]), (__bf16)(q.scale * P4[3][e])};
            }
            continue;
        }
        if (!q.trans) {
#pragma unroll
            for (int r = 0; r < 4; ++r)
                if (n0 + r < W.N)
                    *reinterpret_cast<f32x4*>(q.out + as_slot(q, a.small, n0 + r, q.koff + k0)) =
                        f32x4{q.scale * P4[r][0], q.scale * P4[r][1], q.scale * P4[r][2], q.scale * P4[r][3]};
        } else {
#pragma unroll
            for (int e = 0; e < 4; ++e)
                if (k0 + e < q.ncols)
                    *reinterpret_cast<f32x4*>(q.out + as_slot(q, a.small, k0 + e, q.koff + n0)) =
                        f32x4{q.scale * P4[0][e], q.scale * P4[1][e], q.scale * P4[2][e], q.scale * P4[3][e]};
        }
    }
}
int launch_adamw_streams(const AsArgs& a, float* p, const float* g, float* m, float* v, const float* hyper, float b1, float b2,
                         float eps, hipStream_t s, bool bf) {
    if (bf) hipLaunchKernelGGL(adamw_streams_kernel<true>, dim3(a.nblocks), dim3(AS_BLOCK), 0, s, a, p, g, m, v, hyper, b1, b2, eps);
    else hipLaunchKernelGGL(adamw_streams_kernel<false>, dim3(a.nblocks), dim3(AS_BLOCK), 0, s, a, p, g, m, v, hyper, b1, b2, eps);
    return check_hip(hipGetLastError(), "adamw_streams launch");
}

static NsArgs ns_args(const NsProgram& p, const float* packed, const float* Z, int ldz, int B, int nin, bool full) {
    NsArgs a;
    ::memset(static_cast<void*>(&a), 0, sizeof(a));
    a.Z = Z; a.ldz = ldz; a.B = B; a.nin = nin;
    a.packed = packed;
    a.Gstride = p.Gstride; a.nseg_f = p.nseg_f;
    a.G = full ? p.Gstride : p.G;
    a.nseg = full ? (int)p.seg.size() : p.nseg_f;
    a.LD = p.LD; a.kpad0 = p.kpad0; a.nout = p.nout; a.bias_total = p.bias_total;
    a.T = 1.f;
    for (int i = 0; i < (int)p.seg.size(); ++i) a.seg[i] = p.seg[i];
    return a;
}
static void ns_store_table(NsArgs& a, const NsProgram& p, const NsNet& net, const NsOpBufs* ops, int lo, int hi, bool dx) {
    for (int i = lo; i < hi; ++i) {
        const int op = p.seg_op[i];
        if (op >= net.nl) continue;
        const NsOpBufs& b = ops[op];
        const linna_layer_t& l = net.layers[op];
        a.gn[i] = p.seg_hidden[i] ? l.C : dx ? l.K : l.N;
        if (!dx) { a.gout[i] = p.seg_hidden[i] ? b.t : b.y; a.gld[i] = p.seg_hidden[i] ? b.ldt : b.ldy; }
        else if (p.seg_hidden[i]) { a.gout[i] = b.dt; a.gld[i] = b.lddt; a.gmask[i] = b.t; a.gmld[i] = b.ldt; }
        else { a.gout[i] = b.dprev; a.gld[i] = b.ldp; a.gmask[i] = b.gate; a.gmld[i] = b.ldx; }
    }
}
static bool ns_set_gates(NsArgs& a, const NsGates& g, const NsProgram& p, int rows, size_t* lds_extra) {
    for (int i = 0; i < NS_MAXSEG; ++i) { a.gbit[i] = g.gbit[i]; a.mbit[i] = g.mbit[i]; }
    a.nbw = g.ncols / 32;
    a.bits_off = (int)(g.lds0 / sizeof(float));
    *lds_extra = g.lds - p.lds_for(rows, true);
    return g.ok && g.lds <= (size_t)NS_LDS_BYTES;
}
static void ns_set_input(NsArgs& a, const NsInput& in) {
    a.is_flat = in.is_flat; a.a1 = in.a1; a.a2 = in.a2; a.lg = in.lg; a.xmean = in.xmean; a.xstd = in.xstd;
}
static void ns_set_grad(NsArgs& a, const NsGrad& gr) {
    a.gscale = gr.gscale; a.Gout = gr.G; a.ldg = gr.ldg;
    const NsLeap& l = gr.leap;
    a.hm_p = l.P; a.hm_ldp = l.ldp; a.hm_q = l.Q; a.hm_mass = l.mass; a.hm_ek = l.ek; a.hm_ed = l.ed; a.hm_eps = l.eps;
}

int launch_net_stream(NsKind kind, const NsNet& net, const float* packed, const float* Z, int ldz, int B, const NsInput& in,
                      const NsOutput& out, float* lnP, float* D, int ldd, float* TH, int ldt, const NsMove* mv, const NsGrad* gr,
                      const int* gate, int rows, const NsDense* dn, hipStream_t s) {
    const bool bf = kind == NS_SERVE_BF16;
    if ((kind == NS_SERVE_DENSE) != (dn != nullptr) || !(kind == NS_SERVE || kind == NS_SERVE_DENSE || bf)) {
        set_error("net_stream: not a serving program"); return LINNA_ERR_INVALID;
    }
    const NsProgramRef pref = ns_program(kind, net.layers, net.nl, net.in_size, dn, rows);
    const NsProgram& p = *pref;
    if ((out.cpost != nullptr) != (out.cshift2 != nullptr) || (out.cpost && (dn || gr))) {
        set_error("net_stream: the exp output map needs cpost and cshift2, and has no dense / gradient program"); return LINNA_ERR_INVALID;
    }
    if (!p.ok) { set_error("net_stream: network not eligible"); return LINNA_ERR_UNSUPPORTED; }
    if (dn && (out.w || gr || out.cscale || out.cshift)) { set_error("net_stream: the dense program carries its own output map and has no fused gradient"); return LINNA_ERR_INVALID; }
    if (mv && (in.nin > 64 || (!out.w && !dn))) { set_error("net_stream: fused sampler moves need <= 64 parameters and a log-likelihood in the launch"); return LINNA_ERR_UNSUPPORTED; }
    if (gr && (!p.grad_ok || !out.w || !lnP || !gr->gscale || !gr->G || mv)) { set_error("net_stream: no fused gradient for this network / likelihood"); return LINNA_ERR_UNSUPPORTED; }
    NsArgs a = ns_args(p, packed, Z, ldz, B, in.nin, gr != nullptr);
    ns_set_input(a, in);
    a.cscale = out.cscale; a.cshift = out.cshift; a.w = out.w; a.T = out.T;
    a.cpost = out.cpost; a.cshift2 = out.cshift2;
    a.dense = p.dense ? (dn && dn->factored ? 2 : 1) : 0; a.u_col = p.u_col; a.u_same = p.u_same; a.x0_keep = p.x0_keep;
    a.lnP = lnP; a.D = D; a.ldd = ldd; a.TH = TH; a.ldt = ldt;
    a.gate = gate;
    if (mv) {
        a.mv_coords = mv->coords; a.mv_ldc = mv->ldc; a.mv_logp = mv->logp; a.mv_S = mv->S;
        a.mv_cc = mv->cc; a.mv_ldcc = mv->ldcc; a.mv_C = mv->C; a.mv_nc = mv->nc;
        a.mv_seed = mv->seed; a.mv_step = mv->step; a.mv_step_off = mv->step_off; a.mv_stream = mv->stream; a.mv_a = mv->a; a.mv_naccept = mv->naccept;
        a.mv_chain = mv->chain; a.mv_lps = mv->lps;
        a.sl_Z0 = mv->sl_Z0; a.sl_L = mv->sl_L; a.sl_R = mv->sl_R; a.sl_Zt = mv->sl_Zt; a.sl_m = mv->sl_m; a.sl_nt = mv->sl_nt;
        a.sl_seed = mv->sl_seed; a.sl_step = mv->sl_step; a.sl_stream = mv->sl_stream; a.sl_flags = mv->sl_flags;
        if (mv->sb) a.sb = *mv->sb;
        if (mv->slice) {
            if (bf) return ns_launch_slice_bf16(a, B, p, rows, s);
            return ns_launch_kernel<2, false>(a, B, p, rows, s);
        }
        if (bf) return ns_launch_kernel<1, false, 0, true>(a, B, p, rows, s);
        return ns_launch_kernel<1, false>(a, B, p, rows, s);
    }
    if (bf && gr) { set_error("net_stream: no bf16 gradient"); return LINNA_ERR_UNSUPPORTED; }
    if (bf) return ns_launch_kernel<0, false, 0, true>(a, B, p, rows, s);
    if (gr) {
        ns_set_grad(a, *gr);
        if (a.hm_p && a.hm_eps) return ns_launch_kernel<0, true, 0, false, true>(a, B, p, rows, s);
        return ns_launch_kernel<0, true>(a, B, p, rows, s);
    }
    return ns_launch_kernel<0, false>(a, B, p, rows, s);
}

int launch_net_stream_store(const NsNet& net, const float* packed, const float* X, int ldx, int B, const NsOpBufs* ops,
                            const float* cscale, const float* cshift, int rows, hipStream_t s) {
    const NsProgramRef pref = ns_program(NS_STORE, net.layers, net.nl, net.in_size, nullptr, rows);
    const NsProgram& p = *pref;
    if (!p.ok) { set_error("net_stream: network not eligible"); return LINNA_ERR_UNSUPPORTED; }
    NsArgs a = ns_args(p, packed, X, ldx, B, net.in_size, false);
    a.is_flat = reinterpret_cast<const int*>(X); a.a1 = X; a.a2 = X; a.lg = nullptr; a.xmean = X; a.xstd = X;
    a.cscale = cscale; a.cshift = cshift;
    ns_store_table(a, p, net, ops, 0, p.nseg_f, false);
    return ns_launch_kernel<0, false, 1>(a, B, p, rows, s);
}


int launch_net_stream_grad2(const NsNet& net, const float* packed, const float* Z, int ldz, int B, const NsInput& in, const NsOutput& out,
                            float* lnP, const NsGrad& gr, int rows, hipStream_t s, bool bf) {
    const NsProgramRef pref = ns_program(bf ? NS_GRAD_INPUT_BF16 : NS_GRAD_INPUT, net.layers, net.nl, net.in_size, nullptr, rows);
    const NsProgram& p = *pref;
    if (!p.ok || !p.dxi_ok) { set_error("net_stream: no forward + dX program for this network"); return LINNA_ERR_UNSUPPORTED; }
    if (!out.w || !lnP || !gr.gscale || !gr.G) { set_error("net_stream: the one-launch gradient needs a diagonal covariance"); return LINNA_ERR_INVALID; }
    NsArgs a = ns_args(p, packed, Z, ldz, B, in.nin, true);
    ns_set_input(a, in);
    a.cscale = out.cscale; a.cshift = out.cshift; a.w = out.w; a.T = out.T; a.lnP = lnP;
    ns_set_grad(a, gr);
    const NsGates g = ns_gates(p, net.layers, net.nl, rows);
    for (int i = 0; i < (int)p.seg.size(); ++i) if (i >= p.nseg_f || g.gbit[i] >= 0) a.gn[i] = ns_seg_cols(p, net.layers, i);
    size_t lds_extra = 0;
    if (!ns_set_gates(a, g, p, rows, &lds_extra)) {
        set_error(g.ok ? "net_stream: the one-launch gradient's sign bits do not fit the LDS" : "net_stream: a gate of the one-launch gradient has no producer");
        return LINNA_ERR_UNSUPPORTED;
    }
    if (bf) {
#ifdef NS_STAMPS
        set_error("net_stream: the NS_STAMPS build has no bf16 gradient"); return LINNA_ERR_UNSUPPORTED;
#endif
        const size_t lds = p.lds_for(rows, true) + lds_extra;
        const char* const what = "net_stream bf16 gradient launch";
        if (a.hm_p && a.hm_eps) {
            if (rows == 4) return ns_launch<net_stream_eps_bf16_kernel<NS_R, 0, true, 2, 4, true>>(a, (B + 3) / 4, lds, s, what);
            if (rows == 8) return ns_launch<net_stream_eps_bf16_kernel<NS_R, 0, true, 2, 8, true>>(a, (B + 7) / 8, lds, s, what);
            if (rows == 16) return ns_launch<net_stream_eps_bf16_kernel<NS_R, 0, true, 2, 16, true>>(a, (B + 15) / 16, lds, s, what);
        }
        if (rows == 4) return ns_launch<net_stream_grad_bf16_kernel<NS_R, 0, true, 2, 4, true>>(a, (B + 3) / 4, lds, s, what);
        if (rows == 8) return ns_launch<net_stream_grad_bf16_kernel<NS_R, 0, true, 2, 8, true>>(a, (B + 7) / 8, lds, s, what);
        if (rows == 16) return ns_launch<net_stream_grad_bf16_kernel<NS_R, 0, true, 2, 16, true>>(a, (B + 15) / 16, lds, s, what);
        set_error("net_stream: %d rows per workgroup", rows);
        return LINNA_ERR_INVALID;
    }
    if (a.hm_p && a.hm_eps) return ns_launch_kernel<0, true, 2, false, true>(a, B, p, rows, s, 0, lds_extra);
    return ns_launch_kernel<0, true, 2>(a, B, p, rows, s, 0, lds_extra);
}

static NsArgs ns_train_args(const NsProgram& p, bool full, const NsNet& net, const float* packed, const NsBatch& b, const NsOpBufs* ops,
                            const NsTrainLoss& L) {
    NsArgs a = ns_args(p, packed, b.X, b.ldx, b.B, net.in_size, full);
    a.is_flat = reinterpret_cast<const int*>(b.xmean); a.a1 = b.xmean; a.a2 = b.xmean;
    a.lg = b.lg; a.xmean = b.xmean; a.xstd = b.xstd;
    a.dense = p.dense; a.u_col = p.u_col; a.u_same = p.u_same;
    ns_store_table(a, p, net, ops, 0, p.nseg_f, false);
    a.t_rows = b.ROWS; a.t_xb = b.XB; a.t_ldxb = b.ldxb;
    a.t_Y = L.YN; a.t_ldy = L.ldyn;
    a.t_den = L.den; a.t_inv_batch = L.inv_batch; a.t_loss_rows = L.loss_rows; a.t_dP = L.dP; a.t_lddp = L.lddp;
    return a;
}

int launch_net_stream_train(const NsNet& net, const float* packed, const NsBatch& b, const NsOpBufs* ops, const NsTrainLoss& L,
                            const NsDense& dn, int rows, hipStream_t s) {
    const NsProgramRef pref = ns_program(NS_TRAIN_FWD, net.layers, net.nl, net.in_size, &dn, rows);
    const NsProgram& p = *pref;
    if (!p.ok || !p.dense) { set_error("net_stream: network + loss not eligible"); return LINNA_ERR_UNSUPPORTED; }
    const NsArgs a = ns_train_args(p, false, net, packed, b, ops, L);
    return ns_launch_kernel<0, false, 3>(a, b.B, p, rows, s);
}

int launch_net_stream_train_bwd(const NsNet& net, const float* packed, const NsBatch& b, const NsOpBufs* ops, const NsTrainLoss& L,
                                const NsDense& dn, int rows, hipStream_t s, const NsPost* post, bool bf) {
    const NsProgramRef pref = ns_program(bf ? NS_TRAIN_STEP_BF16 : NS_TRAIN_STEP, net.layers, net.nl, net.in_size, &dn, rows);
    const NsProgram& p = *pref;
    if (!p.ok || !p.train_ok || !p.dense) { set_error("net_stream: network + loss have no one-launch training program"); return LINNA_ERR_UNSUPPORTED; }
    if (rows != 4) { set_error(bf ? "net_stream: the bf16 training step runs on the 4-row engine (batches of up to 1024 rows)"
                                  : "net_stream: the one-launch training step runs on the 4-row engine"); return LINNA_ERR_UNSUPPORTED; }
    NsArgs a = ns_train_args(p, true, net, packed, b, ops, L);
// ... 36 lines not shown
```

### linna_amd/csrc/net_stream_body.inc

```
    constexpr int NT = NS_NT, NW = NS_NW;
    constexpr int RG = 32;
    constexpr bool SM = ROWS < 16;
    constexpr int RS = SM ? ROWS / 4 : 1;
    constexpr int NQ = SM ? RS : NT;
    constexpr int NACC = SM ? 4 * RS : NT;
#ifdef NS_BODY_SLICE_BF16
    static_assert(BF && !GRAD && STORE == 0 && MOVE == 2, "bf16: the slice evaluation");
#elif defined(NS_BODY_GRAD_BF16)
    static_assert(BF && GRAD && STORE == 2 && MOVE == 0, "bf16: lnP and its gradient in one launch");
#else
    static_assert(!BF || (!GRAD && STORE == 0 && MOVE != 2) || (GRAD && STORE == 3 && MOVE == 0 && ROWS == 4),
                  "bf16: serving, the fused stretch move and the merged training step (4-row engine)");
#endif
    constexpr bool BFT = BF && GRAD && STORE == 3;
    constexpr int AK = BF ? 2 : 1;
    constexpr bool K4 = !SM && !BF && (STORE == 0 || (GRAD && STORE == 2));
    constexpr bool TRB = GRAD && STORE == 3;
    constexpr bool DXE = STORE == 2 || TRB;
    constexpr bool G2 = GRAD && STORE == 2;
    constexpr bool LB = G2;
    constexpr bool LATE_REFILL = true;
    constexpr bool RNAN = STORE == 1;
    auto relu_f = [](float v) { if constexpr (RNAN) return isnan(v) ? v : fmaxf(v, 0.f); else return fmaxf(v, 0.f); };
    static_assert(ROWS == 16 || ROWS == 8 || ROWS == 4, "rows per workgroup");
    static_assert(R % 2 == 0, "the A double buffer alternates with the ring slot parity");
    extern __shared__ __attribute__((aligned(16))) float smem[];
    const int LD = a.LD, ABUF = ROWS * LD;
    constexpr bool KA = STORE == 3 || STORE == 1 || GRAD;
    const NsArgs* const ka = KA ? reinterpret_cast<const NsArgs*>((const void*)__builtin_amdgcn_kernarg_segment_ptr()) : &a;
    float* const act = smem;
    float* const lbias = smem + 2 * ABUF;
    unsigned* const lbits = reinterpret_cast<unsigned*>(smem + a.bits_off);
    const int nbw = a.nbw;
    const int tid = threadIdx.x, lane = tid & 63;
    const int wave = __builtin_amdgcn_readfirstlane(tid >> 6);
    const int li = lane & 15, kq = lane >> 4;
    const int row0 = blockIdx.x * ROWS;
    if (a.gate && a.gate[0] == 0) return;
    int mv_rows = a.B;
    if constexpr (MOVE == 2) {
        if (a.mv_C) {
            mv_rows = a.mv_step[0] * a.mv_step_off;
            if (row0 >= mv_rows) return;
        }
    }
    if constexpr ((STORE == 2 && !GRAD) || TRB) {
        if ((a.p_n > 0 || a.p_step) && blockIdx.x == gridDim.x - 1) {
            float* const part = smem;
            float acc0 = 0.f, acc1 = 0.f;
            for (int i = tid; i < a.p_n; i += 1024) acc0 += a.p_rows[i];
            for (int i = tid + 512; i < a.p_n; i += 1024) acc1 += a.p_rows[i];
#pragma unroll
            for (int o = 32; o >= 1; o >>= 1) { acc0 += __shfl_xor(acc0, o, 64); acc1 += __shfl_xor(acc1, o, 64); }
            if (lane == 0) { part[wave] = acc0; part[8 + wave] = acc1; }
            __syncthreads();
            if (tid == 0 && a.p_out) {
                float t = 0.f;
                for (int w = 0; w < 16; ++w) t += part[w];
                a.p_out[0] = t * a.p_scale;
            }
            if (tid == 64 && a.p_step) {
                const int t = ++a.p_step[0];
                a.p_hyper[2] = (float)(1.0 - pow((double)a.p_b1, (double)t));
                a.p_hyper[3] = (float)sqrt(1.0 - pow((double)a.p_b2, (double)t));
            }
            return;
        }
    }
#ifdef NS_STAMPS
    unsigned long long* const lstamp = reinterpret_cast<unsigned long long*>(lbias + ((a.bias_total + 3) & ~3) + 32 + (a.x0_keep ? 1024 : 0)) + wave * 32;
    int nstamp = 0;
#define NS_STAMP() do { const unsigned long long t_ = __builtin_readcyclecounter(); \
        if (lane == 0 && nstamp < 32) lstamp[nstamp] = t_; ++nstamp; } while (0)
#define NS_STAMPS_FLUSH() do { if (lane < 32) a.stamps[((size_t)blockIdx.x * NW + wave) * 32 + lane] = lane < nstamp ? lstamp[lane] : 0ull; } while (0)
#else
#define NS_STAMP() do {} while (0)
#define NS_STAMPS_FLUSH() do {} while (0)
#endif
    NS_STAMP();

    const int prt = tid / RG, pc0 = tid % RG;
    const bool prow = prt < ROWS;
    const int pr = SM ? min(prt, ROWS - 1) : prt;
    int grow = min(row0 + pr, a.B - 1);
    if constexpr (MOVE == 2) {
        if (a.mv_C) grow = a.mv_C[min(row0 + pr, mv_rows - 1)];
    }
    int zsrc = grow;
    float zden = 1.f;
    if constexpr (STORE == 3) {
        zsrc = a.t_rows ? a.t_rows[grow] : grow;
        zden = a.t_den[zsrc];
    }
    const int kpad0 = a.kpad0, nin = a.nin, nout = a.nout, nseg = a.nseg;
    const int nlast = (TRB ? a.nseg_f : nseg) - 2;
    constexpr int ZPRE = 2;
    float zr[ZPRE], za1[ZPRE], za2[ZPRE], zxm[ZPRE], zxs[ZPRE]; int zfl[ZPRE], zlg[ZPRE];
    const int* const lgp = a.lg ? a.lg : a.is_flat;
    int mv_wk = 0; float mv_factor = 0.f, mv_lnp_old = 0.f, mv_logu = 0.f;
    if constexpr (MOVE == 1) {
        mv_wk = a.mv_S[grow];
        const U4 rb = walker_bits(a.mv_seed, (uint32_t)mv_wk, (uint32_t)(a.mv_step[0] + a.mv_step_off), (uint32_t)a.mv_stream, 0u);
        const float t = (a.mv_a - 1.f) * u01(rb.x) + 1.f;
        const float zf = t * t / a.mv_a;
        const int j = (int)(((uint64_t)rb.y * (uint64_t)a.mv_nc) >> 32);
        const int wc = a.mv_C[j];
        mv_factor = ((float)nin - 1.f) * logf(zf);
        mv_logu = logf(u01(rb.z));
        mv_lnp_old = a.mv_logp[mv_wk];
#pragma unroll
        for (int i = 0; i < ZPRE; ++i) {
            const int c = min(pc0 + i * RG, nin - 1);
            const float cr = a.mv_cc[(size_t)wc * a.mv_ldcc + c], sx = a.mv_coords[(size_t)mv_wk * a.mv_ldc + c];
            zr[i] = cr - (cr - sx) * zf;
        }
    }
    if constexpr (MOVE == 2) {
        const int k = grow % a.mv_nc;
        const int wk = a.mv_S[k];
        float wgt;
        if (a.sb.logp) {
            const SliceBegin& b = a.sb;
            const int jt = grow / a.mv_nc;
            const U4 rb = walker_bits(b.seed, (uint32_t)wk, (uint32_t)b.step[0], (uint32_t)b.half, 0u);
            const int ia = (int)(((uint64_t)rb.x * (uint64_t)b.nc) >> 32);
            int ib = (int)(((uint64_t)rb.y * (uint64_t)(b.nc - 1)) >> 32);
            ib += (ib >= ia);
            const int wa = b.C[ia], wb = b.C[ib];
            const float mu = b.mu[0];
            const float l = -u01(rb.w);
            wgt = jt < b.m ? l - (float)jt : l + 1.f + (float)(jt - b.m);
            const bool first = jt == 0 && prow && row0 + pr < a.B;
#pragma unroll
            for (int i = 0; i < ZPRE; ++i) {
                const int c = min(pc0 + i * RG, nin - 1);
                const float dir = mu * (b.cc[(size_t)wa * b.ldcc + c] - b.cc[(size_t)wb * b.ldcc + c]);
                zr[i] = a.mv_coords[(size_t)wk * a.mv_ldc + c] + wgt * dir;
                if (first && pc0 + i * RG < nin) b.DIR[(size_t)k * b.ldd + c] = dir;
            }
            if (first && pc0 == 0) {
                b.Z0[k] = b.logp[wk] + logf(u01(rb.z));
                b.L[k] = l; b.R[k] = l + 1.f;
                int J, K;
                slice_budget(b.seed, (uint32_t)wk, (uint32_t)b.step[0], (uint32_t)b.half, b.maxsteps, J, K);
                b.flags[3 * k] = J; b.flags[3 * k + 1] = K; b.flags[3 * k + 2] = 1;
            }
            if (blockIdx.x == 0 && tid == 0) {
                for (int i = 0; i < b.nslots; ++i) {
                    b.counters[4 + b.nslots + i] += b.counters[4 + i];
                    b.counters[4 + i] = 0;
                }
                b.counters[4 + 2 * b.nslots] += 1;
                if (b.zero_totals) { b.counters[0] = 0; b.counters[1] = 0; }
            }
        } else {
        if (a.sl_Zt) {
            const int ns_ = a.mv_nc, m = a.sl_m, jt = grow / ns_;
            const float z0 = a.sl_Z0[k];
            const float zend = a.sl_Zt[(size_t)min(pc0, 2 * m - 1) * ns_ + k];
            const unsigned long long bal = __ballot(pc0 < 2 * m && zend > z0);
            const unsigned bits = (unsigned)(bal >> (lane & 32));
            const unsigned lm = bits & ((1u << m) - 1u), rm = (bits >> m) & ((1u << m) - 1u);
            const int nl = min(__builtin_ctz(~lm), a.sl_flags[3 * k]), nr = min(__builtin_ctz(~rm), a.sl_flags[3 * k + 1]);
            float l = a.sl_L[k], r = a.sl_R[k];
            for (int j = 0; j < m; ++j) {
                if (j < nl) l -= 1.f;
                if (j < nr) r += 1.f;
            }
            const U4 tb = walker_bits(a.sl_seed, (uint32_t)wk, (uint32_t)a.sl_step[0], (uint32_t)a.sl_stream, (uint32_t)(pc0 + 1));
            const int myu = __float_as_int(u01(tb.x));
            wgt = 0.f;
            for (int jj = 0; jj < a.sl_nt; ++jj) {
                const int ulo = __builtin_amdgcn_readlane(myu, jj), uhi = __builtin_amdgcn_readlane(myu, 32 + jj);
                const float u = __int_as_float((lane & 32) ? uhi : ulo);
                const float w = l + u * (r - l);
                if (jj == jt) wgt = w;
                if (jj < jt) { if (w < 0.f) l = w; else r = w; }
            }
        } else {
            wgt = a.mv_cc[grow];
        }
#pragma unroll
        for (int i = 0; i < ZPRE; ++i) {
            const int c = min(pc0 + i * RG, nin - 1);
            zr[i] = a.mv_coords[(size_t)wk * a.mv_ldc + c] + wgt * a.Z[(size_t)k * a.ldz + c];
        }
        }
    }
#pragma unroll
    for (int i = 0; i < ZPRE; ++i) {
        const int c = min(pc0 + i * RG, nin - 1);
        if constexpr (MOVE == 0) zr[i] = a.Z[(size_t)(STORE == 3 ? zsrc : grow) * a.ldz + c];
        zfl[i] = a.is_flat[c]; za1[i] = a.a1[c]; za2[i] = a.a2[c];
        zlg[i] = lgp[c]; zxm[i] = a.xmean[c]; zxs[i] = a.xstd[c];
    }
    const int nb4 = (a.bias_total + 3) >> 2;
    const f32x4* const bsrc = reinterpret_cast<const f32x4*>(a.packed + (size_t)NW * a.Gstride * NT * 256);
    constexpr int BMAX = 3;
    f32x4 breg[BMAX];
#pragma unroll
    for (int i = 0; i < BMAX; ++i) {
        const int j = tid + i * 64 * NW;
        breg[i] = bsrc[min(j, nb4 - 1)];
    }
    constexpr int FIN = 2;
    const float* const csp = a.cscale ? a.cscale : a.xmean;
    const float* const ctp = a.cshift ? a.cshift : a.xmean;
    const float* const wtp = a.w ? a.w : a.xmean;
    float fcs[FIN], fct[FIN], fw[FIN], fgs[FIN];
#pragma unroll
    for (int i = 0; i < FIN; ++i) {
        const int cc = min(pc0 + i * RG, nout - 1);
        if constexpr (GRAD && !TRB) fgs[i] = a.gscale[cc]; else fgs[i] = 0.f;
        const int c1 = a.cscale ? cc : 0, c2 = a.cshift ? cc : 0, c3 = a.w ? cc : 0;
        const float cs = csp[c1], ct = ctp[c2], ww = wtp[c3];
        fcs[i] = a.cscale ? cs : 1.f; fct[i] = a.cshift ? ct : 0.f; fw[i] = a.w ? ww : 0.f;
    }

    const char* const wbase = reinterpret_cast<const char*>(a.packed) + (size_t)wave * a.Gstride * NS_STEP_B;
    const unsigned wlast = (unsigned)(a.G - 1) * NS_STEP_B;
    unsigned woff = 0;
    const unsigned voff = 16u * (unsigned)lane;
    f32x4 Bq[R][NT];
    auto wload = [&](int t) { return *reinterpret_cast<const f32x4*>(wbase + (size_t)(voff + woff) + t * 1024); };
    auto wadvance = [&]() { woff = min(woff + NS_STEP_B, wlast); };
    constexpr int PRE = NS_PRE < R ? NS_PRE : R;
    auto prefetch = [&](auto Uc) {
        constexpr int U = decltype(Uc)::value;
#pragma unroll
        for (int t = 0; t < NT; ++t) {
            Bq[U][t] = wload(t);
            __builtin_amdgcn_sched_barrier(0);
        }
        wadvance();
    };
#define NS_PF(U, LO, HI) if constexpr (U >= LO && U < HI) prefetch(std::integral_constant<int, U>{});
#define NS_PF_ALL(LO, HI) NS_PF(0, LO, HI) NS_PF(1, LO, HI) NS_PF(2, LO, HI) NS_PF(3, LO, HI) NS_PF(4, LO, HI) NS_PF(5, LO, HI) \
    NS_PF(6, LO, HI) NS_PF(7, LO, HI)
    NS_PF_ALL(0, PRE)
#ifdef NS_STAMPS_FINE
    NS_STAMP();
#endif

    float zz = 0.f;
    float theta[ZPRE];
#pragma unroll
    for (int i = 0; i < ZPRE; ++i) {
        const int c = pc0 + i * RG;
        const bool in = c < nin;
        const float z = in ? zr[i] : 0.f;
        zz += z * z;
        float th = ns_prior_theta(z, zfl[i], za1[i], za2[i]);
        float lt = log10f(th);
        asm volatile("" : "+v"(lt));
        theta[i] = th;
        const float t = (a.lg && zlg[i]) ? lt : th;
        float x = in ? (t - zxm[i]) / zxs[i] : 0.f;
        zz += 0.f * x;
        if constexpr ((STORE == 1 || STORE == 2) && !GRAD) x = z;
        if constexpr (STORE == 3) {
            float lz = log10f(z);
            asm volatile("" : "+v"(lz));
            const float tz = (a.lg && zlg[i]) ? lz : z;
            x = in ? (tz - zxm[i]) / zxs[i] : 0.f;
            if (prow && row0 + pr < a.B && c < a.t_ldxb)
                asm volatile("global_store_dword %0, %1, off" :: "v"(a.t_xb + (size_t)(row0 + pr) * a.t_ldxb + c), "v"(x) : "memory");
        }
        if constexpr (BF) {
            if (prow) {
                if (in) { const float hi = (float)(__bf16)x; act[pr * LD + c] = hi; act[pr * LD + nin + c] = x - hi; }
                else if (c >= 2 * nin && c < kpad0) act[pr * LD + c] = 0.f;
            }
        } else {
            if (c < kpad0 && prow) act[pr * LD + c] = x;
        }
    }
#ifdef NS_STAMPS_FINE
    NS_STAMP();
#endif
    if constexpr ((STORE == 1 || STORE == 2) && !GRAD) {
        const int wcols = kpad0 - ZPRE * RG;
        if (wcols > 0) {
            constexpr int CP = 4;
            for (int base = 0; base < ROWS * wcols; base += CP * 64 * NW) {
                float v[CP];
#pragma unroll
                for (int u = 0; u < CP; ++u) {
                    const int idx = min(base + u * 64 * NW + tid, ROWS * wcols - 1);
                    const int r = idx / wcols, c = ZPRE * RG + idx % wcols;
                    v[u] = a.Z[(size_t)min(row0 + r, a.B - 1) * a.ldz + min(c, nin - 1)];
                }
#pragma unroll
                for (int u = 0; u < CP; ++u) {
                    const int idx = base + u * 64 * NW + tid;
                    if (idx < ROWS * wcols) {
                        const int r = idx / wcols, c = ZPRE * RG + idx % wcols;
                        act[r * LD + c] = c < nin ? v[u] : 0.f;
                    }
                }
            }
        }
    } else
#pragma unroll 1
    for (int c = pc0 + ZPRE * RG; c < kpad0; c += RG) {
        float x = 0.f;
        if (c < nin) {
            const float z = a.Z[(size_t)grow * a.ldz + c];
            zz += z * z;
            const float th = ns_prior_theta(z, a.is_flat[c], a.a1[c], a.a2[c]);
            const float t = (a.lg && a.lg[c]) ? log10f(th) : th;
            x = (t - a.xmean[c]) / a.xstd[c];
            zz += 0.f * x;
            if constexpr ((STORE == 1 || STORE == 2) && !GRAD) x = z;
            if constexpr (STORE == 3) {
                const float zz3 = a.Z[(size_t)zsrc * a.ldz + c];
                x = (((a.lg && a.lg[c]) ? log10f(zz3) : zz3) - a.xmean[c]) / a.xstd[c];
            }
        }
        if constexpr (STORE == 3) {
            if (prow && row0 + pr < a.B && c < a.t_ldxb)
                asm volatile("global_store_dword %0, %1, off" :: "v"(a.t_xb + (size_t)(row0 + pr) * a.t_ldxb + c), "v"(x) : "memory");
        }
        if constexpr (BF) {
            if (prow) {
                if (c < nin) { const float hi = (float)(__bf16)x; act[pr * LD + c] = hi; act[pr * LD + nin + c] = x - hi; }
                else if (c >= 2 * nin) act[pr * LD + c] = 0.f;
            }
        } else {
            if (prow) act[pr * LD + c] = x;
        }
    }
    __builtin_amdgcn_sched_barrier(0);
#ifdef NS_STAMPS_FINE
    NS_STAMP();
#endif
    NS_PF_ALL(PRE, (LATE_REFILL ? R - 1 : R))
#undef NS_PF_ALL
#undef NS_PF
#pragma unroll
    for (int o = RG / 2; o >= 1; o >>= 1) zz += __shfl_xor(zz, o, 64);
#pragma unroll
    for (int i = 0; i < BMAX; ++i) {
        const int j = tid + i * 64 * NW;
        if (j < nb4) reinterpret_cast<f32x4*>(lbias)[j] = breg[i];
    }
    int* const lsrc = reinterpret_cast<int*>(lbias + ((a.bias_total + 3) & ~3));
    float* const lden = reinterpret_cast<float*>(lsrc + 16);
    if constexpr (STORE == 3) {
        if (prow && pc0 == 0) { lsrc[pr] = zsrc; lden[pr] = zden; }
    }
    float* const lx0 = lden + 16;
    if (a.x0_keep && prow) {
#pragma unroll
        for (int i = 0; i < ZPRE; ++i) {
            const int c = pc0 + i * RG;
            if constexpr (BF) lx0[pr * 64 + c] = c < nin ? act[pr * LD + c] + act[pr * LD + nin + c] : 0.f;
            else lx0[pr * 64 + c] = (c < kpad0) ? act[pr * LD + c] : 0.f;
        }
    }
    asm volatile("s_waitcnt lgkmcnt(0)" ::: "memory");
    __builtin_amdgcn_s_barrier();
    asm volatile("" ::: "memory");
    NS_STAMP();

    const uint32_t act_lds = (uint32_t)(uintptr_t)(__attribute__((address_space(3))) void*)act;
    f32x4 acc[NACC];
    f32x4 Aq[2][AK];
    const int sm_arow = (4 * ((lane >> 2) & 3) + (lane & 3)) % ROWS, sm_achunk = lane >> 4;
    int si = 0, pass = 0, P = 0, kleft;
    int s_type, s_steps, s_passes, s_bias, s_dst, s_relu, s_kslice, s_zext, s_ncgl, s_mstore = 0, s_mapply = 0, s_x0col = 0, s_x0n = 0, s_kcl = 0;
    unsigned* const lmask = reinterpret_cast<unsigned*>(lbias + ((a.bias_total + 3) & ~3));
    float lnp_grad = 0.f;
    float* s_gout = nullptr; int s_gld = 0, s_gn = 0;
    const float* s_gmask = nullptr; int s_gmld = 0;
    int s_gbit = -1, s_mbit = -1;
    auto gstore = [&](float* p, float v) { asm volatile("global_store_dword %0, %1, off" :: "v"(p), "v"(v) : "memory"); };
    uint32_t ap;
    auto a_read = [&](f32x4* dst) {
        asm volatile("ds_read_b128 %0, %1" : "=v"(dst[0]) : "v"(ap) : "memory");
        if constexpr (BF) asm volatile("ds_read_b128 %0, %1 offset:16" : "=v"(dst[1]) : "v"(ap) : "memory");
        if constexpr (BFT) ap += si == a.nseg_f - 1 ? 64 : 64 * AK;
        else ap += 64 * AK;
    };
    auto load_seg = [&]() {
        const NsSeg S = ka->seg[__builtin_amdgcn_readfirstlane(si)];
        s_type = S.type; kleft = s_steps = S.steps; s_passes = S.passes; s_bias = S.bias_off;
        s_dst = S.dst_col; s_relu = S.relu; s_kslice = S.kslice; s_zext = S.zext; s_ncgl = S.ncg_log2; s_x0col = S.x0_col; s_x0n = S.x0_n;
        if constexpr (GRAD) { s_mstore = S.mask_store; s_mapply = S.mask_apply; }
        if constexpr (STORE) { const int j = __builtin_amdgcn_readfirstlane(si); s_gout = ka->gout[j]; s_gld = ka->gld[j]; s_gn = ka->gn[j]; }
        if constexpr (DXE) { const int j = __builtin_amdgcn_readfirstlane(si); s_gmask = ka->gmask[j]; s_gmld = ka->gmld[j]; }
        if constexpr (LB) { const int j = __builtin_amdgcn_readfirstlane(si); s_gbit = ka->gbit[j]; s_mbit = ka->mbit[j]; }
    };
    auto begin_run = [&]() {
        const int arow = SM ? sm_arow : li, ak = AK * (SM ? 4 * sm_achunk : 4 * kq);
#pragma unroll
        for (int t = 0; t < NACC; ++t) acc[t] = f32x4{0.f, 0.f, 0.f, 0.f};
        if (s_type == NS_WIDE) {
            const int blk = s_zext < 0 ? (pass ? 15 - wave : wave) : 8 * pass + wave;
            if constexpr (SM) {
                const float b = lbias[s_bias + 64 * blk + lane];
#pragma unroll
                for (int r = 0; r < RS; ++r) acc[4 * r] = f32x4{b, b, b, b};
            } else {
#pragma unroll
                for (int t = 0; t < NT; ++t) {
                    const float b = lbias[s_bias + 16 * (4 * blk + t) + li];
                    acc[t] = f32x4{b, b, b, b};
                }
            }
            if (s_zext < 0) kleft = s_steps - 4 * blk;
            ap = act_lds + 4u * (uint32_t)(P * ABUF + arow * LD + ak + (s_zext < 0 ? 64 * blk : (pass ? s_kslice : 0)));
        } else {
            ap = act_lds + 4u * (uint32_t)(P * ABUF + arow * LD + ak + (wave >> s_ncgl) * s_kslice);
        }
        if constexpr (BFT) {
            if (si == a.nseg_f - 1) ap -= 4u * (uint32_t)(ak / 2);
        }
    };
    auto lds_barrier = [&]() {
        asm volatile("s_waitcnt lgkmcnt(0)" ::: "memory");
        __builtin_amdgcn_s_barrier();
        asm volatile("" ::: "memory");
    };
    load_seg();
    begin_run();
    a_read(Aq[0]);

    auto step = [&](auto Uc, auto Refill) {
        constexpr int U = decltype(Uc)::value;
        constexpr bool refill = decltype(Refill)::value;
        constexpr int RU = LATE_REFILL ? (U + R - 1) % R : U;
        if constexpr (BF) asm volatile("s_waitcnt lgkmcnt(0)" : "+v"(Aq[U & 1][0]), "+v"(Aq[U & 1][AK - 1]) :: "memory");
        else asm volatile("s_waitcnt lgkmcnt(0)" : "+v"(Aq[U & 1][0]) :: "memory");
        a_read(Aq[(U + 1) & 1]);
        const f32x4 av = Aq[U & 1][0];
        if constexpr (BF) {
            bf16x8 ab;
#pragma unroll
            for (int e = 0; e < 4; ++e) { ab[e] = (__bf16)Aq[U & 1][0][e]; ab[4 + e] = (__bf16)Aq[U & 1][AK - 1][e]; }
            if constexpr (SM) {
                auto bf_small = [&]() {
                    const s16x4 alo = __builtin_bit_cast(s16x4, __builtin_shufflevector(ab, ab, 0, 1, 2, 3));
                    const s16x4 ahi = __builtin_bit_cast(s16x4, __builtin_shufflevector(ab, ab, 4, 5, 6, 7));
#define NS_B4(r, c, h, A4) acc[4 * (r) + (c)] = __builtin_amdgcn_mfma_f32_4x4x4bf16_1k(A4, \
                __builtin_bit_cast(s16x4, __builtin_shufflevector(__builtin_bit_cast(bf16x8, Bq[U][c]), __builtin_bit_cast(bf16x8, Bq[U][c]), \
                                                                  4 * (h), 4 * (h) + 1, 4 * (h) + 2, 4 * (h) + 3)), acc[4 * (r) + (c)], 4, 4 * (c) + (r), 0);
#define NS_B4R(r, h, A4) NS_B4(r, 0, h, A4) NS_B4(r, 1, h, A4) NS_B4(r, 2, h, A4) NS_B4(r, 3, h, A4)
                    NS_B4R(0, 0, alo)
                    if constexpr (RS > 1) { NS_B4R(1, 0, alo) }
                    NS_B4R(0, 1, ahi)
                    if constexpr (RS > 1) { NS_B4R(1, 1, ahi) }
#undef NS_B4R
#undef NS_B4
                };
                if constexpr (BFT) {
                    if (si == a.nseg_f - 1) {
#define NS_M4(r, c, e) acc[4 * (r) + (c)] = __builtin_amdgcn_mfma_f32_4x4x1f32(av[e], Bq[U][c][e], acc[4 * (r) + (c)], 4, 4 * (c) + (r), 0);
#define NS_M4R(r, e) NS_M4(r, 0, e) NS_M4(r, 1, e) NS_M4(r, 2, e) NS_M4(r, 3, e)
#pragma unroll
                        for (int e = 0; e < 4; ++e) {
                            NS_M4R(0, e)
                            if constexpr (RS > 1) { NS_M4R(1, e) }
                        }
#undef NS_M4R
#undef NS_M4
                    } else {
                        bf_small();
                    }
                } else {
                    bf_small();
                }
                if constexpr (refill) {
#pragma unroll
                    for (int t = 0; t < NT; ++t) Bq[RU][t] = wload(t);
                }
            } else {
#pragma unroll
                for (int h = 0; h < NT; h += 2) {
                    acc[h] = __builtin_amdgcn_mfma_f32_16x16x32_bf16(ab, __builtin_bit_cast(bf16x8, Bq[U][h]), acc[h], 0, 0, 0);
                    acc[h + 1] = __builtin_amdgcn_mfma_f32_16x16x32_bf16(ab, __builtin_bit_cast(bf16x8, Bq[U][h + 1]), acc[h + 1], 0, 0, 0);
                    if constexpr (refill) {
                        Bq[RU][h] = wload(h);
                        Bq[RU][h + 1] = wload(h + 1);
                    }
                }
            }
        } else if constexpr (SM) {
#define NS_M4(r, c, e) acc[4 * (r) + (c)] = __builtin_amdgcn_mfma_f32_4x4x1f32(av[e], Bq[U][c][e], acc[4 * (r) + (c)], 4, 4 * (c) + (r), 0);
#define NS_M4R(r, e) NS_M4(r, 0, e) NS_M4(r, 1, e) NS_M4(r, 2, e) NS_M4(r, 3, e)
#pragma unroll
            for (int e = 0; e < 4; ++e) {
                NS_M4R(0, e)
                if constexpr (RS > 1) { NS_M4R(1, e) }
            }
#undef NS_M4R
#undef NS_M4
            if constexpr (refill) {
#pragma unroll
                for (int t = 0; t < NT; ++t) Bq[RU][t] = wload(t);
            }
        } else {
#pragma unroll
            for (int h = 0; h < NT; h += 2) {
#pragma unroll
                for (int s = 0; s < 4; ++s) {
                    acc[h] = __builtin_amdgcn_mfma_f32_16x16x4f32(av[s], Bq[U][h][s], acc[h], 0, 0, 0);
                    acc[h + 1] = __builtin_amdgcn_mfma_f32_16x16x4f32(av[s], Bq[U][h + 1][s], acc[h + 1], 0, 0, 0);
                }
                if constexpr (refill) {
                    Bq[RU][h] = wload(h);
                    Bq[RU][h + 1] = wload(h + 1);
                }
            }
        }
        if constexpr (refill) wadvance();
        if (--kleft == 0) {
            const int nxi = __builtin_amdgcn_readfirstlane(min(si + 1, nseg - 1));
            const NsSeg NX = ka->seg[nxi];
            float* nx_gout = nullptr; int nx_gld = 0, nx_gn = 0;
            const float* nx_gmask = nullptr; int nx_gmld = 0;
            if constexpr (STORE) { nx_gout = ka->gout[nxi]; nx_gld = ka->gld[nxi]; nx_gn = ka->gn[nxi]; }
            if constexpr (DXE) { nx_gmask = ka->gmask[nxi]; nx_gmld = ka->gmld[nxi]; }
            int nx_gbit = -1, nx_mbit = -1;
            if constexpr (LB) { nx_gbit = ka->gbit[nxi]; nx_mbit = ka->mbit[nxi]; }
            const int cur_steps = s_steps;
            auto take_seg = [&](const NsSeg& X) {
                s_type = X.type; s_steps = X.steps; s_passes = X.passes; s_bias = X.bias_off;
                s_dst = X.dst_col; s_relu = X.relu; s_kslice = X.kslice; s_zext = X.zext; s_ncgl = X.ncg_log2; s_x0col = X.x0_col; s_x0n = X.x0_n;
                if constexpr (K4) s_kcl = X.kcl;
                if constexpr (GRAD) { s_mstore = X.mask_store; s_mapply = X.mask_apply; }
                kleft = X.steps;
            };
            auto take_next = [&]() {
                take_seg(NX);
                if constexpr (STORE) { s_gout = nx_gout; s_gld = nx_gld; s_gn = nx_gn; }
                if constexpr (DXE) { s_gmask = nx_gmask; s_gmld = nx_gmld; }
                if constexpr (LB) { s_gbit = nx_gbit; s_mbit = nx_mbit; }
            };
            f32x4 sdw[2][NT];
            bool side_next = false;
            if constexpr (K4) {
#pragma unroll
                for (int s2 = 0; s2 < 2; ++s2)
#pragma unroll
                    for (int t = 0; t < NT; ++t) sdw[s2][t] = f32x4{0.f, 0.f, 0.f, 0.f};
                if (NX.type == NS_SIDE && si + 1 < nseg && (s_type != NS_WIDE || pass + 1 == s_passes)) {
                    side_next = true;
                    const char* const sb = reinterpret_cast<const char*>(a.packed + NX.side_off) + (size_t)wave * NX.steps * NS_STEP_B + voff;
#pragma unroll
                    for (int t = 0; t < NT; ++t)
                        asm volatile("global_load_dwordx4 %0, %1, off" : "=v"(sdw[0][t]) : "v"(sb + t * 1024) : "memory");
                    if (NX.steps > 1) {
#pragma unroll
                        for (int t = 0; t < NT; ++t)
                            asm volatile("global_load_dwordx4 %0, %1, off" : "=v"(sdw[1][t]) : "v"(sb + NS_STEP_B + t * 1024) : "memory");
                    }
                }
            }
            bool seg_done = true;
#ifdef NS_STAMPS_FINE
            const bool fine = si >= NS_STAMPS_FINE && si < NS_STAMPS_FINE + 4;
            if (fine) NS_STAMP();
#endif
            if constexpr (SM) {
#pragma unroll
                for (int q = 0; q < NQ; ++q) acc[q] = (acc[4 * q] + acc[4 * q + 1]) + (acc[4 * q + 2] + acc[4 * q + 3]);
            }
#define fin acc
#define q_row(q, e) (SM ? 4 * (q) + (e) : 4 * kq + (e))
#define q_col(q) (SM ? lane : 16 * (q) + li)
            if (s_type == NS_WIDE) {
                float* const nxt = act + (P ^ 1) * ABUF + s_dst + (s_zext < 0 ? 64 * (pass ? 15 - wave : wave) : 512 * pass + 64 * wave);
                float ty[NQ][4];
                if constexpr (STORE == 3) {
                    if (si == nlast) {
#pragma unroll
                        for (int t = 0; t < NQ; ++t) {
                            const int dc = min(512 * pass + 64 * wave + q_col(t), nout - 1);
#pragma unroll
                            for (int e = 0; e < 4; ++e) {
                                const float* py = a.t_Y + (size_t)lsrc[q_row(t, e)] * a.t_ldy + dc;
                                asm volatile("global_load_dword %0, %1, off" : "=v"(ty[t][e]) : "v"(py) : "memory");
                            }
                        }
#pragma unroll
                        for (int t = 0; t < NQ; ++t)
                            asm volatile("s_waitcnt vmcnt(0)" : "+v"(ty[t][0]), "+v"(ty[t][1]), "+v"(ty[t][2]), "+v"(ty[t][3]) :: "memory");
                    }
                }
                unsigned long long gw[SM ? NQ : 1][4];
                if constexpr (LB) {
                    if (s_mbit >= 0) {
                        const int cw = 512 * pass + 64 * wave, w0 = (s_mbit + cw) >> 5;
                        const bool mine = cw < ((s_gn + 63) & ~63);
#pragma unroll
                        for (int t = 0; t < (SM ? NQ : 1); ++t)
#pragma unroll
                            for (int e = 0; e < 4; ++e)
                                gw[t][e] = mine ? *reinterpret_cast<const unsigned long long*>(lbits + (SM ? 4 * t + e : 4 * kq + e) * nbw + w0) : 0ull;
                    }
                }
                if constexpr (DXE && !LB) {
                    if (s_gmask) {
#pragma unroll
                        for (int t = 0; t < NQ; ++t) {
                            const int mc = min(512 * pass + 64 * wave + q_col(t), s_gn - 1);
#pragma unroll
                            for (int e = 0; e < 4; ++e) {
                                const float* pg = s_gmask + (size_t)min(row0 + q_row(t, e), a.B - 1) * s_gmld + mc;
                                if constexpr (GRAD)
                                    asm volatile("global_load_dword %0, %1, off sc1" : "=v"(ty[t][e]) : "v"(pg) : "memory");
                                else
                                    asm volatile("global_load_dword %0, %1, off" : "=v"(ty[t][e]) : "v"(pg) : "memory");
                            }
                        }
#pragma unroll
                        for (int t = 0; t < NQ; ++t)
                            asm volatile("s_waitcnt vmcnt(0)" : "+v"(ty[t][0]), "+v"(ty[t][1]), "+v"(ty[t][2]), "+v"(ty[t][3]) :: "memory");
                    }
                }
                unsigned mbits = 0xFFFFu;
                if constexpr (GRAD) {
                    if (s_mapply) mbits = lmask[(s_mapply - 1 + pass) * (64 * NW) + threadIdx.x];
                    if (s_mstore) {
                        unsigned m = 0;
#pragma unroll
                        for (int t = 0; t < NQ; ++t)
#pragma unroll
                            for (int e = 0; e < 4; ++e) m |= (fin[t][e] > 0.f ? 1u : 0u) << (4 * t + e);
                        lmask[(s_mstore - 1 + pass) * (64 * NW) + threadIdx.x] = m;
                    }
                }
#pragma unroll
                for (int t = 0; t < NQ; ++t)
#pragma unroll
                    for (int e = 0; e < 4; ++e) {
                        float v = fin[t][e];
                        if constexpr (GRAD) v = ((mbits >> (4 * t + e)) & 1u) ? v : 0.f;
                        v = s_relu ? relu_f(v) : v;
                        if constexpr (LB) {
                            if (s_mbit >= 0 && !((gw[SM ? t : 0][e] >> (SM ? lane : 16 * t + li)) & 1ull)) v = 0.f;
                        } else if constexpr (DXE) {
                            if (s_gmask && !(ty[t][e] > 0.f)) v = 0.f;
                        }
                        float v_lds = v;
                        if constexpr (STORE == 3) {
                            if (si == nlast) {
                                const int dc = 512 * pass + 64 * wave + q_col(t);
                                const float yn = ty[t][e];
                                v_lds = dc < nout ? (isnan(yn) ? -0.f : (yn - v) + 0.f) : 0.f;
                            }
                        }
                        nxt[q_row(t, e) * LD + q_col(t)] = v_lds;
                        if constexpr (LB) {
                            if (s_gbit >= 0) {
                                const unsigned long long bb = __ballot(v > 0.f);
                                const int cw = 512 * pass + 64 * wave;
                                const bool mine = cw < ((s_gn + 63) & ~63);
                                const int c0 = s_gbit + cw;
                                if constexpr (SM) {
                                    if (lane == 0 && mine) *reinterpret_cast<unsigned long long*>(lbits + (4 * t + e) * nbw + (c0 >> 5)) = bb;
                                } else {
                                    if (li == 0 && mine) reinterpret_cast<unsigned short*>(lbits + (4 * kq + e) * nbw)[(c0 + 16 * t) >> 4] = (unsigned short)(bb >> (16 * kq));
                                }
                            }
                        }
                        if constexpr (STORE && !G2) {
                            const int grow_ = row0 + q_row(t, e), gcol = 512 * pass + 64 * wave + q_col(t);
                            if (s_gout && grow_ < a.B && gcol < s_gn) {
                                float vs = v;
                                if constexpr (STORE == 1)
                                    if (si == nseg - 1) vs = vs * (a.cscale ? a.cscale[gcol] : 1.f) + (a.cshift ? a.cshift[gcol] : 0.f);
                                gstore(s_gout + (size_t)grow_ * s_gld + gcol, vs);
                            }
                        }
                    }
#ifdef NS_STAMPS_FINE
                if (fine) NS_STAMP();
#endif
                if (++pass == s_passes) {
                    lds_barrier();
                    NS_STAMP();
                    P ^= 1; pass = 0; ++si;
                    take_next();
                } else {
                    kleft = s_zext > 0 ? s_zext : cur_steps;
                    seg_done = false;
                }
            } else {
                float* const part = act + (P ^ 1) * ABUF;
                constexpr int PW = ROWS * 64;
#pragma unroll
                for (int t = 0; t < NQ; ++t)
#pragma unroll
                    for (int e = 0; e < 4; ++e) {
                        const int rr = q_row(t, e);
                        part[wave * PW + rr * 64 + (q_col(t) ^ (SM ? 32 * (rr & 1) : 16 * kq))] = fin[t][e];
                    }
#ifdef NS_STAMPS_FINE
                if (fine) NS_STAMP();
#endif
                lds_barrier();
#ifdef NS_STAMPS_FINE
                if (fine) NS_STAMP();
#endif
                constexpr int RGS = SM ? 64 * NW / ROWS : RG;
                const int sr = SM ? tid / RGS : pr, sc0 = SM ? tid % RGS : pc0;
                const bool srow = SM ? true : prow;
                float* const cur = act + P * ABUF + sr * LD + s_dst;
                const int ncol = 64 << s_ncgl, nkp = NW >> s_ncgl;
                const int sw = SM ? 32 * (sr & 1) : 16 * (sr >> 2);
                constexpr int NGJ = 256 / RGS;
                float sg[NGJ];
                if constexpr (DXE && !LB) {
                    if (s_gmask) {
#pragma unroll
                        for (int j = 0; j < NGJ; ++j) {
                            const float* pg = s_gmask + (size_t)min(row0 + sr, a.B - 1) * s_gmld + min(sc0 + RGS * j, s_gn - 1);
                            if constexpr (GRAD)
                                asm volatile("global_load_dword %0, %1, off sc1" : "=v"(sg[j]) : "v"(pg) : "memory");
                            else
                                asm volatile("global_load_dword %0, %1, off" : "=v"(sg[j]) : "v"(pg) : "memory");
                        }
#pragma unroll
                        for (int j = 0; j < NGJ; ++j) asm volatile("s_waitcnt vmcnt(0)" : "+v"(sg[j]) :: "memory");
                    }
                }
                int gj = 0;
                if constexpr ((!LB && !DXE && !STORE) || (LB && !SM)) {
                    auto reduce4 = [&](auto NKc) {
                        constexpr int NK = decltype(NKc)::value;
                        for (int c = 4 * sc0; c < (srow ? s_zext : 0); c += 4 * RGS) {
                            f32x4 v = f32x4{0.f, 0.f, 0.f, 0.f};
                            if (c < ncol) {
                                const float* src = part + (c >> 6) * PW + sr * 64 + ((c & 63) ^ sw);
                                constexpr int CH = LB && NK > 4 ? 4 : NK;
                                const f32x4 b = *reinterpret_cast<const f32x4*>(lbias + s_bias + c);
#pragma unroll
                                for (int k0 = 0; k0 < NK; k0 += CH) {
                                    f32x4 x[CH];
#pragma unroll
                                    for (int kp = 0; kp < CH; ++kp) x[kp] = *reinterpret_cast<const f32x4*>(src + ((k0 + kp) << s_ncgl) * PW);
#pragma unroll
                                    for (int kp = 0; kp < CH; ++kp) v += x[kp];
                                }
                                v += b;
                                if (s_relu) v = f32x4{fmaxf(v[0], 0.f), fmaxf(v[1], 0.f), fmaxf(v[2], 0.f), fmaxf(v[3], 0.f)};
                            }
                            if constexpr (LB) {
                                const bool mine = c < ((s_gn + 63) & ~63);
                                if (s_mbit >= 0) {
                                    const unsigned nib = mine ? (lbits[sr * nbw + ((s_mbit + c) >> 5)] >> (c & 31)) & 0xFu : 0u;
#pragma unroll
                                    for (int e = 0; e < 4; ++e) v[e] = ((nib >> e) & 1u) ? v[e] : 0.f;
                                }
                                *reinterpret_cast<f32x4*>(cur + c) = v;
                                if (s_gbit >= 0) {
                                    unsigned w32 = ((v[0] > 0.f ? 1u : 0u) | (v[1] > 0.f ? 2u : 0u) | (v[2] > 0.f ? 4u : 0u) | (v[3] > 0.f ? 8u : 0u)) << (c & 31);
                                    w32 |= __shfl_xor(w32, 1, 64); w32 |= __shfl_xor(w32, 2, 64); w32 |= __shfl_xor(w32, 4, 64);
                                    if ((sc0 & 7) == 0 && mine) lbits[sr * nbw + ((s_gbit + c) >> 5)] = w32;
                                }
                            } else {
                                *reinterpret_cast<f32x4*>(cur + c) = v;
                            }
                        }
                    };
                    if (nkp == NW) reduce4(std::integral_constant<int, NW>{});
                    else if (nkp == NW / 2) reduce4(std::integral_constant<int, NW / 2>{});
                    else reduce4(std::integral_constant<int, 2>{});
// ... 52 lines not shown
                        constexpr int NJ = NGJ;
                        const int ysrc = lsrc[sr];
                        float sy[NJ];
#pragma unroll
                        for (int j = 0; j < NJ; ++j) {
                            const int c = min(sc0 + RGS * j, nout - 1);
                            asm volatile("global_load_dword %0, %1, off" : "=v"(sy[j]) : "v"(a.t_Y + (size_t)ysrc * a.t_ldy + c) : "memory");
                        }
#pragma unroll
                        for (int j = 0; j < NJ; ++j) asm volatile("s_waitcnt vmcnt(0)" : "+v"(sy[j]) :: "memory");
#pragma unroll
                        for (int j = 0; j < NJ; ++j) {
                            const int c = sc0 + RGS * j;
                            if (c < nout && srow) cur[c] = isnan(sy[j]) ? -0.f : (sy[j] - cur[c]) + 0.f;
                        }
                    }
                }
#ifdef NS_STAMPS_FINE
                if (fine) { asm volatile("s_waitcnt lgkmcnt(0)" ::: "memory"); NS_STAMP(); }
#endif
                lds_barrier();
                NS_STAMP();
                ++si;
                take_next();
            }
            if constexpr (GRAD) {
                if (seg_done && si == a.nseg_f) {
                    if constexpr (DXE && !LB)
                        asm volatile("s_waitcnt vmcnt(0)" ::: "memory");
                    if constexpr (TRB) {
                        {
                            const float* const F = act + P * ABUF + pr * LD;
                            const bool rok = prow && row0 + pr < a.B;
                            const float* const Dv = a.u_same ? F : act + (P ^ 1) * ABUF + pr * LD;
                            const float* const Uv = a.u_same ? F + a.u_col : F;
                            float chi = 0.f;
                            for (int c = pc0; c < nout; c += RG) chi += Dv[c] * Uv[c];
#pragma unroll
                            for (int o = RG / 2; o >= 1; o >>= 1) chi += __shfl_xor(chi, o, 64);
                            if (rok && pc0 == 0) gstore(a.t_loss_rows + row0 + pr, chi / lden[pr]);
                        }
                        lds_barrier();
                        {
                            constexpr int TPR = 64 * NW / ROWS;
                            const int fr = tid / TPR, fc = tid % TPR;
                            float* const Fr = act + P * ABUF + fr * LD;
                            const float* const Dr = a.u_same ? Fr : act + (P ^ 1) * ABUF + fr * LD;
                            const float* const Ur = a.u_same ? Fr + a.u_col : Fr;
                            const float dr = lden[fr];
                            const bool rowok = row0 + fr < a.B;
                            for (int c = fc; c < a.t_lddp; c += TPR) {
                                float g = 0.f;
                                if (c < nout && rowok) {
                                    const bool masked = __float_as_uint(Dr[c]) == 0x80000000u;
                                    g = masked ? 0.f : (-2.f * Ur[c]) * a.t_inv_batch / dr;
                                }
                                if (rowok) gstore(a.t_dP + (size_t)(row0 + fr) * a.t_lddp + c, g);
                                if (c < nout) Fr[c] = g;
                            }
                        }
                        lds_barrier();
                    } else {
                    float* const F = act + P * ABUF + pr * LD;
                    float chi = 0.f;
#pragma unroll
                    for (int i = 0; i < FIN; ++i) {
                        const int c = pc0 + i * RG;
                        if (c < nout && prow) {
                            const float d = F[c] * fcs[i] + fct[i];
                            chi += (d * fw[i]) * d;
                            F[c] = -(d * fw[i]) * fgs[i] / a.T;
                        }
                    }
#pragma unroll
                    for (int o = RG / 2; o >= 1; o >>= 1) chi += __shfl_xor(chi, o, 64);
                    lnp_grad = (-0.5f * chi) / a.T + (-0.5f * zz);
                    lds_barrier();
                    }
                }
            }
#undef fin
#undef q_row
#undef q_col
            if (seg_done && si < nseg && s_x0col > 0) {
                if (prow) {
                    float* const dstp = act + P * ABUF + pr * LD + s_x0col;
#pragma unroll
                    for (int i = 0; i < ZPRE; ++i)
                        if (pc0 + i * RG < s_x0n) dstp[pc0 + i * RG] = lx0[pr * 64 + pc0 + i * RG];
                }
                lds_barrier();
            }
            if constexpr (K4) {
                if (side_next && seg_done) {
#pragma unroll
                    for (int t = 0; t < NT; ++t) acc[t] = f32x4{0.f, 0.f, 0.f, 0.f};
                    const bool kc4 = s_kcl == 2, kc1 = s_kcl == 0;
                    const uint32_t abase = act_lds + 4u * (uint32_t)(P * ABUF + li * LD + 4 * kq + wave * s_kslice);
#pragma unroll
                    for (int s2 = 0; s2 < 2; ++s2) {
                        if (s2 < s_steps) {
                            const uint32_t as = abase + (uint32_t)s2 * (64u << s_kcl);
                            f32x4 af0, af1, af2 = f32x4{0.f, 0.f, 0.f, 0.f}, af3 = f32x4{0.f, 0.f, 0.f, 0.f};
                            asm volatile("ds_read_b128 %0, %1" : "=v"(af0) : "v"(as) : "memory");
                            af1 = f32x4{0.f, 0.f, 0.f, 0.f};
                            if (!kc1) asm volatile("ds_read_b128 %0, %1 offset:64" : "=v"(af1) : "v"(as) : "memory");
                            if (kc4) {
                                asm volatile("ds_read_b128 %0, %1 offset:128" : "=v"(af2) : "v"(as) : "memory");
                                asm volatile("ds_read_b128 %0, %1 offset:192" : "=v"(af3) : "v"(as) : "memory");
                            }
                            if (s2 == 0)
                                asm volatile("s_waitcnt vmcnt(0) lgkmcnt(0)"
                                             : "+v"(af0), "+v"(af1), "+v"(af2), "+v"(af3), "+v"(sdw[0][0]), "+v"(sdw[0][1]), "+v"(sdw[0][2]),
                                               "+v"(sdw[0][3]), "+v"(sdw[1][0]), "+v"(sdw[1][1]), "+v"(sdw[1][2]), "+v"(sdw[1][3]) :: "memory");
                            else
                                asm volatile("s_waitcnt lgkmcnt(0)" : "+v"(af0), "+v"(af1), "+v"(af2), "+v"(af3) :: "memory");
                            const f32x4 f1 = kc4 ? af1 : af0, f2 = kc4 ? af2 : kc1 ? af0 : af1, f3 = kc4 ? af3 : kc1 ? af0 : af1;
#pragma unroll
                            for (int e = 0; e < 4; ++e) {
                                acc[0] = __builtin_amdgcn_mfma_f32_16x16x4f32(af0[e], sdw[s2][0][e], acc[0], 0, 0, 0);
                                acc[1] = __builtin_amdgcn_mfma_f32_16x16x4f32(f1[e], sdw[s2][1][e], acc[1], 0, 0, 0);
                            }
#pragma unroll
                            for (int e = 0; e < 4; ++e) {
                                acc[2] = __builtin_amdgcn_mfma_f32_16x16x4f32(f2[e], sdw[s2][2][e], acc[2], 0, 0, 0);
                                acc[3] = __builtin_amdgcn_mfma_f32_16x16x4f32(f3[e], sdw[s2][3][e], acc[3], 0, 0, 0);
                            }
                        }
                    }
                    int treal = NT;
                    if (kc4) { acc[0] = (acc[0] + acc[1]) + (acc[2] + acc[3]); treal = 1; }
                    else if (!kc1) { acc[0] = acc[0] + acc[2]; acc[1] = acc[1] + acc[3]; treal = 2; }
                    float* const part = act + (P ^ 1) * ABUF;
                    constexpr int PW = ROWS * 64;
#pragma unroll
                    for (int t = 0; t < NT; ++t)
                        if (t < treal) {
#pragma unroll
                            for (int e = 0; e < 4; ++e) part[wave * PW + (4 * kq + e) * 64 + ((16 * t + li) ^ (16 * kq))] = acc[t][e];
                        }
#ifdef NS_STAMPS_FINE
                    if (fine) NS_STAMP();
#endif
                    lds_barrier();
#ifdef NS_STAMPS_FINE
                    if (fine) NS_STAMP();
#endif
                    {
                        float* const cur = act + P * ABUF + pr * LD + s_dst;
                        const int ncol = 16 * treal, sw = 16 * (pr >> 2);
                        for (int c = 4 * pc0; c < s_zext; c += 4 * RG) {
                            f32x4 v = f32x4{0.f, 0.f, 0.f, 0.f};
                            if (c < ncol) {
                                const float* src = part + pr * 64 + (c ^ sw);
                                constexpr int CH = LB ? 4 : NW;
                                const f32x4 b = *reinterpret_cast<const f32x4*>(lbias + s_bias + c);
#pragma unroll
                                for (int k0 = 0; k0 < NW; k0 += CH) {
                                    f32x4 x[CH];
#pragma unroll
                                    for (int kp = 0; kp < CH; ++kp) x[kp] = *reinterpret_cast<const f32x4*>(src + (k0 + kp) * PW);
#pragma unroll
                                    for (int kp = 0; kp < CH; ++kp) v += x[kp];
                                }
                                v += b;
                                if (s_relu) v = f32x4{fmaxf(v[0], 0.f), fmaxf(v[1], 0.f), fmaxf(v[2], 0.f), fmaxf(v[3], 0.f)};
                            }
                            if constexpr (LB) {
                                const bool mine = c < ((s_gn + 63) & ~63);
                                if (s_mbit >= 0) {
                                    const unsigned nib = mine ? (lbits[pr * nbw + ((s_mbit + c) >> 5)] >> (c & 31)) & 0xFu : 0u;
#pragma unroll
                                    for (int e = 0; e < 4; ++e) v[e] = ((nib >> e) & 1u) ? v[e] : 0.f;
                                }
                                *reinterpret_cast<f32x4*>(cur + c) = v;
                                if (s_gbit >= 0) {
                                    unsigned w32 = ((v[0] > 0.f ? 1u : 0u) | (v[1] > 0.f ? 2u : 0u) | (v[2] > 0.f ? 4u : 0u) | (v[3] > 0.f ? 8u : 0u)) << (c & 31);
                                    w32 |= __shfl_xor(w32, 1, 64); w32 |= __shfl_xor(w32, 2, 64); w32 |= __shfl_xor(w32, 4, 64);
                                    if ((pc0 & 7) == 0 && mine) lbits[pr * nbw + ((s_gbit + c) >> 5)] = w32;
                                }
                            } else {
                                *reinterpret_cast<f32x4*>(cur + c) = v;
                            }
                        }
                    }
#ifdef NS_STAMPS_FINE
                    if (fine) { asm volatile("s_waitcnt lgkmcnt(0)" ::: "memory"); NS_STAMP(); }
#endif
                    lds_barrier();
                    NS_STAMP();
                    ++si;
                    const int n2i = __builtin_amdgcn_readfirstlane(min(si, nseg - 1));
                    const NsSeg N2 = ka->seg[n2i];
                    take_seg(N2);
                    if constexpr (LB) { s_gbit = ka->gbit[n2i]; s_mbit = ka->mbit[n2i]; s_gn = ka->gn[n2i]; }
                }
            }
            if (si < nseg) {
                begin_run();
                a_read(Aq[(U + 1) & 1]);
            }
#ifdef NS_STAMPS_FINE
            if (fine) { asm volatile("s_waitcnt lgkmcnt(0)" ::: "memory"); NS_STAMP(); }
#endif
        }
    };
    using T_ = std::true_type; using F_ = std::false_type;
#define NS_STEP(U, RF) if constexpr (U < R) step(std::integral_constant<int, U>{}, RF{});
    const int ngroups = a.G / R, rem = a.G - ngroups * R;
#pragma unroll 1
    for (int it = 0; it < ngroups; ++it) {
        NS_STEP(0, T_) NS_STEP(1, T_) NS_STEP(2, T_) NS_STEP(3, T_) NS_STEP(4, T_) NS_STEP(5, T_) NS_STEP(6, T_) NS_STEP(7, T_)
    }
#define NS_TAIL(U) if constexpr (U < R - 1) { if (rem > U) step(std::integral_constant<int, U>{}, F_{}); }
    NS_TAIL(0) NS_TAIL(1) NS_TAIL(2) NS_TAIL(3) NS_TAIL(4) NS_TAIL(5) NS_TAIL(6)
#undef NS_STEP
#undef NS_TAIL
    if constexpr (BF) asm volatile("s_waitcnt lgkmcnt(0)" : "+v"(Aq[0][0]), "+v"(Aq[0][AK - 1]), "+v"(Aq[1][0]), "+v"(Aq[1][AK - 1]) :: "memory");
    else asm volatile("s_waitcnt lgkmcnt(0)" : "+v"(Aq[0][0]), "+v"(Aq[1][0]) :: "memory");
    NS_STAMP();

    if constexpr (((STORE == 1 || STORE == 2) && !GRAD) || TRB) { NS_STAMPS_FLUSH(); return; }
    if constexpr (STORE == 3) {
        const float* const F = act + P * ABUF + pr * LD;
        const bool rok = prow && row0 + pr < a.B;
        const float* const Dv = a.u_same ? F : act + (P ^ 1) * ABUF + pr * LD;
        const float* const Uv = a.u_same ? F + a.u_col : F;
        float chi = 0.f;
        for (int c = pc0; c < nout; c += RG) chi += Dv[c] * Uv[c];
#pragma unroll
        for (int o = RG / 2; o >= 1; o >>= 1) chi += __shfl_xor(chi, o, 64);
        if (rok && pc0 == 0) a.t_loss_rows[row0 + pr] = chi / lden[pr];
        {
            constexpr int TPR = 64 * NW / ROWS;
            const int fr = tid / TPR, fc = tid % TPR;
            if (row0 + fr < a.B) {
                const float* const Fr = act + P * ABUF + fr * LD;
                const float* const Dr = a.u_same ? Fr : act + (P ^ 1) * ABUF + fr * LD;
                const float* const Ur = a.u_same ? Fr + a.u_col : Fr;
                const float dr = lden[fr];
                for (int c = fc; c < a.t_lddp; c += TPR) {
                    float g = 0.f;
                    if (c < nout) {
                        const bool masked = __float_as_uint(Dr[c]) == 0x80000000u;
                        g = masked ? 0.f : (-2.f * Ur[c]) * a.t_inv_batch / dr;
                    }
                    a.t_dP[(size_t)(row0 + fr) * a.t_lddp + c] = g;
                }
            }
        }
        NS_STAMP();
        NS_STAMPS_FLUSH();
        return;
    }
    if constexpr (GRAD) {
        const float* const F = act + P * ABUF + pr * LD;
        const bool rok = prow && row0 + pr < a.B;
        if (rok) {
            float hm_ek = a.hm_ek, hm_ed = a.hm_ed;
            if constexpr (EPS) { const float e = a.hm_eps[row0 + pr]; hm_ek *= e; hm_ed *= e; }
#pragma unroll
            for (int j = 0; j < ZPRE; ++j) {
                const int c = pc0 + j * RG;
                if (c < nin) {
                    float g = F[c] / zxs[j];
                    if (a.lg && zlg[j]) g = g / (theta[j] * 2.30258509299404568f);
                    const float z = zr[j];
                    const float dth = zfl[j] ? za2[j] * (expf(-0.5f * z * z) * 0.398942280401432678f) : za2[j];
                    const float gz = g * dth - z;
                    a.Gout[(size_t)(row0 + pr) * a.ldg + c] = gz;
                    if (a.hm_p) {
                        float* const pp = a.hm_p + (size_t)(row0 + pr) * a.hm_ldp + c;
                        float pm = *pp;
                        if (a.hm_ek != 0.f) { pm += hm_ek * gz; *pp = pm; }
                        if (a.hm_ed != 0.f) a.hm_q[(size_t)(row0 + pr) * a.ldz + c] = z + hm_ed * (pm / a.hm_mass[c]);
                    }
                }
            }
            if (pc0 == 0) a.lnP[row0 + pr] = isnan(lnp_grad) ? -INFINITY : lnp_grad;
        }
        if constexpr (STORE == 2) { NS_STAMP(); NS_STAMPS_FLUSH(); }
        return;
    }
    {
        const float* const F = act + P * ABUF + pr * LD;
        const bool rok = prow && row0 + pr < a.B;
        float chi = 0.f;
        auto column = [&](int c, float cs, float ct, float ww) {
            float d = F[c] * cs + ct;
            if (a.cpost) d = expf(d) * a.cpost[c] + a.cshift2[c];
            if (a.D && rok) a.D[(size_t)(row0 + pr) * a.ldd + c] = isnan(zz) ? zz : d;
            chi += (d * ww) * d;
        };
        if (a.dense) {
            const float* const Dv = a.u_same ? F : act + (P ^ 1) * ABUF + pr * LD;
            const float* const U = a.u_same ? F + a.u_col : F;
            const bool fac = a.dense == 2;
            for (int c = pc0; c < nout; c += RG) {
                const float d = Dv[c];
                if (a.D && rok) a.D[(size_t)(row0 + pr) * a.ldd + c] = isnan(zz) ? zz : d;
                const float u = U[c];
                chi += (fac ? u : d) * u;
            }
        } else {
#pragma unroll
            for (int i = 0; i < FIN; ++i)
                if (pc0 + i * RG < nout) column(pc0 + i * RG, fcs[i], fct[i], fw[i]);
            for (int c = pc0 + FIN * RG; c < nout; c += RG)
                column(c, a.cscale ? a.cscale[c] : 1.f, a.cshift ? a.cshift[c] : 0.f, a.w ? a.w[c] : 0.f);
        }
#pragma unroll
        for (int o = RG / 2; o >= 1; o >>= 1) chi += __shfl_xor(chi, o, 64);
        float lnp_new = (-0.5f * chi) / a.T + (-0.5f * zz);
        lnp_new = isnan(lnp_new) ? -INFINITY : lnp_new;
        if constexpr (MOVE == 2) {
            if (a.lnP && pc0 == 0 && prow && row0 + pr < mv_rows) a.lnP[a.mv_C ? grow : row0 + pr] = lnp_new;
        } else {
            if (a.lnP && (a.w || a.dense) && pc0 == 0 && rok) a.lnP[row0 + pr] = lnp_new;
        }
        if constexpr (MOVE == 1) {
            const bool mv_acc = rok && mv_factor + lnp_new - mv_lnp_old > mv_logu;
            if (mv_acc) {
#pragma unroll
                for (int j = 0; j < ZPRE; ++j)
                    if (pc0 + j * RG < nin) a.mv_coords[(size_t)mv_wk * a.mv_ldc + pc0 + j * RG] = zr[j];
                if (pc0 == 0) {
                    a.mv_logp[mv_wk] = lnp_new;
                    if (a.mv_naccept) a.mv_naccept[mv_wk] += 1;
                }
            }
            if (a.mv_chain && rok) {
#pragma unroll
                for (int j = 0; j < ZPRE; ++j)
                    if (pc0 + j * RG < nin)
                        a.mv_chain[(size_t)mv_wk * nin + pc0 + j * RG] = mv_acc ? zr[j] : a.mv_coords[(size_t)mv_wk * a.mv_ldc + pc0 + j * RG];
                if (pc0 == 0) a.mv_lps[mv_wk] = mv_acc ? lnp_new : mv_lnp_old;
            }
        }
        if (a.TH && rok) {
#pragma unroll
            for (int j = 0; j < ZPRE; ++j)
                if (pc0 + j * RG < nin) a.TH[(size_t)(row0 + pr) * a.ldt + pc0 + j * RG] = theta[j];
            for (int c = pc0 + ZPRE * RG; c < nin; c += RG)
                a.TH[(size_t)(row0 + pr) * a.ldt + c] = ns_prior_theta(a.Z[(size_t)grow * a.ldz + c], a.is_flat[c], a.a1[c], a.a2[c]);
        }
    }
    NS_STAMP();
    NS_STAMPS_FLUSH();
#undef NS_STAMP
#undef NS_STAMPS_FLUSH
```

### linna_amd/nn.py

```python
import collections
import ctypes as C
import math

import numpy as np
import torch

from . import _lib

__all__ = ["ChtoModelv2", "ChtoModelv2_linear", "ChtoModelsimple", "MLP", "MLP4x512", "ResBlock_batchnorm"]


def _hidden(out_size):
    return 1000 if out_size > 30 else max(32, int(out_size * 32))


def _xavier_uniform(shape):
    bound = math.sqrt(3.0) * math.sqrt(2.0 / float(shape[0] + shape[1]))
    return torch.empty(shape, dtype=torch.float32).uniform_(-bound, bound)


def _consume(n):
    if n > 0:
        torch.empty(int(n), dtype=torch.float32).uniform_()

# ... 300 lines not shown
        h = _hidden(self.out_size)
        ops = [_Op(L, "layer1", self.in_size, h, relu=1)]
        for i, mult in enumerate((1, 2, 4)):
            ops.append(_Op(R, "layer%d" % (i + 2), h, h // 2, C=self.channel * mult))
            h //= 2
        h6 = 4 * h if self.wide_layer6 else h
        ops.append(_Op(L, "layer6", h, h6, relu=1))
        ops.append(_Op(L, "layer7", h6, self.out_size, relu=1))
        ops.append(_Op(L, "layer8", self.out_size, self.out_size, relu=0))
        return ops


class ChtoModelsimple(ChtoModelv2):
    channel = 4
    wide_layer6 = False


class ChtoModelv2_linear(ChtoModelv2):

    def _build_ops(self):
        ops = ChtoModelv2._build_ops(self)
        ops.append(_Op(_lib.OP_INSKIP, "linearlayer", self.in_size, self.out_size, alpha=1e-3))
        return ops

    def _post_init(self):
        self._view(self._flat, "linearlayer.bias").zero_()
        self._view(self._flat, "linearlayer.weight").fill_(1e-5)


class MLP(_Emulator):

    def __init__(self, in_size, out_size, linearmodel=None, docpu=False, width=512, depth=4):
        self.width, self.depth = int(width), int(depth)
        _Emulator.__init__(self, in_size, out_size, linearmodel, docpu)

    def _build_ops(self):
        ops, k = [], self.in_size
        for i in range(self.depth):
            ops.append(_Op(_lib.OP_LINEAR, "layer%d" % (i + 1), k, self.width, relu=1))
            k = self.width
        ops.append(_Op(_lib.OP_LINEAR, "layer%d" % (self.depth + 1), k, self.out_size, relu=0))
        return ops


MLP4x512 = MLP


class ResBlock_batchnorm(object):

    def __init__(self, in_size, channel, out_size):
        self.in_size, self.channel, self.out_size = in_size, channel, out_size
        self.op = _Op(_lib.OP_RESBLOCK, "block", in_size, out_size, C=channel)


def program_layers(model):
    arr = _lib.sized_array(_lib.Layer, len(model.ops))
    nxt = [4096]

    def fake(n):
        p = nxt[0]
        nxt[0] += 16 * ((int(n) + 3) // 4 + 1)
        return C.c_void_p(p)
    for i, op in enumerate(model.ops):
        L = arr[i]
        L.op, L.K, L.C, L.N, L.relu, L.alpha = op.op, op.K, op.C, op.N, op.relu, op.alpha
        if op.op == _lib.OP_RESBLOCK:
            L.W1, L.b1, L.W2, L.b2 = fake(op.C * op.K), fake(op.C), fake(op.N * op.C), fake(op.N)
            if op.K != op.N:
                L.Ws = fake(op.N * op.K)
        else:
            L.W, L.b = fake(op.N * op.K), fake(op.N)
    return arr


def describe_program(model, rows=16, dense_nout=0):
    arr = program_layers(model)
    buf = C.create_string_buffer(8192)
    n = _lib.load().linna_program_describe(arr, len(model.ops), model.in_size, int(rows), int(dense_nout), buf, len(buf))
    if n < 0:
        _lib.check(n)
    return n, buf.value.decode()


def describe_grad_bf16_program(model, rows=16):
    arr = program_layers(model)
    buf = C.create_string_buffer(8192)
    n = _lib.load().linna_program_describe_grad_bf16(arr, len(model.ops), model.in_size, int(rows), buf, len(buf))
    if n < 0:
        _lib.check(n)
    return n, buf.value.decode()
```

### linna_amd/util.py

```python
import ctypes as C
import io
import os
import pickle
from collections import OrderedDict
from copy import deepcopy

import numpy as np
import torch

from . import _lib
from . import nn as lnn
from . import predictor_gpu
from .nn import *

SQRT2 = float(np.sqrt(2.0))


def cpu_quota():
    try:
        n = len(os.sched_getaffinity(0))
    except Exception:
        n = os.cpu_count() or 1
    for path, parse in (("/sys/fs/cgroup/cpu.max", lambda t: t.split()),
                        ("/sys/fs/cgroup/cpu/cpu.cfs_quota_us", lambda t: (t.strip(), open("/sys/fs/cgroup/cpu/cpu.cfs_period_us").read().strip()))):
# ... 299 lines not shown
            k["S"] = f32(pad(S))
            k["Ssym"] = f32(pad(0.5 * (S.astype(np.float64) + S.astype(np.float64).T)))
            d.S, d.lds, d.Ssym = _lib.ptr(k["S"]), ldS, _lib.ptr(k["Ssym"])
            if os.environ.get("LINNA_DENSE_FACTORED", "1") != "0":
                try:
                    Lf = np.linalg.cholesky(0.5 * (S.astype(np.float64) + S.astype(np.float64).T))
                    k["Sfac"] = f32(pad(Lf))
                    d.Sfac = _lib.ptr(k["Sfac"])
                except np.linalg.LinAlgError:
                    pass
        d.gscale = _lib.ptr(k["gscale"])
        d.temperature = self.T
        h = C.c_void_p()
        _lib.call("linna_logprob_create", _lib.ctx(dev.index), net.net_handle(), C.byref(d), C.byref(h))
        rc = _lib.load().linna_logprob_set_precision(h, _lib.PRECISION[self.precision])
        if rc != 0:
            msg = _lib.load().linna_last_error().decode()
            _lib.load().linna_logprob_destroy(h)
            if rc == _lib.ERR_UNSUPPORTED:
                raise ValueError("Log_prob(precision=%r): %s" % (self.precision, msg))
            _lib.check(rc)
        if self._grad_precision != "fp32":
            rc = _lib.load().linna_logprob_set_grad_precision(h, _lib.PRECISION[self._grad_precision])
            if rc != 0:
                msg = _lib.load().linna_last_error().decode()
                _lib.load().linna_logprob_destroy(h)
                if rc in (_lib.ERR_UNSUPPORTED, _lib.ERR_INVALID):
                    raise ValueError("Log_prob(grad_precision=%r): %s" % (self._grad_precision, msg))
                _lib.check(rc)
        self._plan = dict(handle=h, keep=k, desc=d, dev=dev, nin=nin, nout=nout, net_sig=net._net_sig)
        self._ws = {}

    def _ensure(self):
        net = self.model.model
        if self._plan is None or self._plan["dev"] != net.device or net._net is None or net._net_sig != self._plan["net_sig"]:
            if self._plan is not None:
                _lib.load().linna_logprob_destroy(self._plan["handle"])
                self._plan = None
            self._build()
        return self._plan

    def _workspace(self, B, with_grad):
        key = (int(B), bool(with_grad))
        ws = self._ws.get(key)
        if ws is None:
            n = _lib.load().linna_logprob_ws_bytes(self._plan["handle"], int(B), 1 if with_grad else 0)
            ws = torch.empty(n // 4 + 4, dtype=torch.float32, device=self._plan["dev"])
            self._ws[key] = ws
        return ws

    def _to_device(self, x):
        p = self._ensure()
        if not torch.is_tensor(x):
            x = torch.from_numpy(np.ascontiguousarray(x, dtype=np.float32))
        z = x.detach().to(device=p["dev"], dtype=torch.float32)
        one = z.dim() == 1
        z = z.view(1, -1) if one else z
        if z.shape[1] != p["nin"]:
            raise ValueError("expected %d parameters per walker, got %d" % (p["nin"], z.shape[1]))
        return z.contiguous(), one

    @staticmethod
    def _check_rows(z, p):
        if not (torch.is_tensor(z) and z.is_cuda and z.dtype == torch.float32 and z.dim() == 2):
            raise _lib.LinnaHipError("expected a 2-D float32 device tensor of walker positions")
        if z.device != p["dev"]:
            raise _lib.LinnaHipError("walker positions on %s, log-probability on %s" % (z.device, p["dev"]))
        if z.shape[1] < p["nin"] or (z.shape[0] > 1 and z.stride(1) != 1) or (z.shape[1] > 1 and z.stride(1) != 1):
            raise _lib.LinnaHipError("walker rows must hold >= %d contiguous columns (got shape %s, strides %s)"
                                     % (p["nin"], tuple(z.shape), tuple(z.stride())))

    def evaluate(self, z, out=None, theta=None):
        p = self._ensure()
        self._check_rows(z, p)
        B = z.shape[0]
        if out is None:
            out = torch.empty(B, dtype=torch.float32, device=z.device)
        _lib.call("linna_logprob_eval", p["handle"], _lib.ptr(z) if z.is_contiguous() else C.c_void_p(z.data_ptr()),
                  z.stride(0), B, _lib.ptr(self._workspace(B, False)), _lib.ptr(out),
                  C.c_void_p(theta.data_ptr()) if theta is not None else None,
                  theta.stride(0) if theta is not None else 0, _lib.stream())
        return out

    def evaluate_with_grad(self, z, out=None, grad=None):
        if self.precision != "fp32" and self._grad_precision == "fp32":
            raise ValueError("Log_prob.evaluate_with_grad: no gradient in %s (serving only); use precision='fp32'" % self.precision)
        p = self._ensure()
        self._check_rows(z, p)
        B = z.shape[0]
        if out is None:
            out = torch.empty(B, dtype=torch.float32, device=z.device)
        if grad is None:
            grad = torch.empty((B, p["nin"]), dtype=torch.float32, device=z.device)
        _lib.call("linna_logprob_grad", p["handle"], C.c_void_p(z.data_ptr()), z.stride(0), B,
                  _lib.ptr(self._workspace(B, True)), _lib.ptr(out), C.c_void_p(grad.data_ptr()), grad.stride(0),
                  _lib.stream())
        return out, grad

    @property
    def grad_precision(self):
        return self._grad_precision

    @property
    def device_only(self):
        return self.loglikelihoodfunc is gaussianlogliklihood and self.externalloglike is None

    def evaluate_any(self, z):
        p = self._ensure()
        if self.device_only:
            return self.evaluate(z)
        zc = z[:, :p["nin"]].contiguous()
        if self.loglikelihoodfunc is not gaussianlogliklihood:
            return self._generic(zc).to(z.device)
        theta = torch.empty_like(zc)
        like = self.evaluate(zc, theta=theta)
        th = theta.cpu().numpy()
        ext = np.array([np.float32(self.externalloglike(t)) for t in th], np.float32)
        like = like + torch.from_numpy(ext).to(like.device)
        return torch.where(torch.isnan(like), torch.full_like(like, -float("inf")), like)

    def __call__(self, x, returntorch=True, inputnumpy=True):
        z, one = self._to_device(x)
        if z.shape[0] == 0:
            like = torch.empty(0, dtype=torch.float32)
            return like if returntorch else like.numpy()
        like = self.evaluate_any(z).cpu()
        if one:
            like = like[0]
        return like if returntorch else like.numpy()

    def _generic(self, z):
        theta = self.transform(z.cpu(), inputnumpy=False, returnnumpy=False).reshape(z.shape[0], -1)
        m = self.y_invtransform_data(self.model.predict(theta, no_grad=True)).cpu()
        data = torch.as_tensor(_np32(self.data_new))
        invcov = torch.as_tensor(_np32(self.invcov_new))
        out = []
        for i in range(z.shape[0]):
            v = self.loglikelihoodfunc(m[i:i + 1], data, invcov) / self.T + lnprior(z[i].cpu())
            if self.externalloglike is not None:
                v = v + np.float32(self.externalloglike(theta[i].numpy()))
            out.append(float(v))
        out = torch.tensor(out, dtype=torch.float32)
        return torch.where(torch.isnan(out), torch.full_like(out, -float("inf")), out)


class Dlnp(object):

    def __init__(self, data_new, invcov_new, model, y_invtransform_data, transform, temperature):
        self.log_prob = Log_prob(data_new, invcov_new, model, y_invtransform_data, transform, temperature)

    def __call__(self, x, lnP=None, returntorch=None, inputnumpy=None):
        z, one = self.log_prob._to_device(x)
        _, g = self.log_prob.evaluate_with_grad(z)
        g = g.cpu().numpy()
        return g[0] if one else g


class Ddlnp(object):

    def __init__(self, data_new, invcov_new, model, y_invtransform_data, transform, temperature, eps=1e-2):
        self.log_prob = Log_prob(data_new, invcov_new, model, y_invtransform_data, transform, temperature)
        self.eps = float(eps)

    def __call__(self, x):
        z, _ = self.log_prob._to_device(x)
        n = z.shape[1]
# ... 474 lines not shown
```

Baseline: 73.19 million evals/s.

## Add specialized plain fp32 serve kernel with compile-time pruned branches

Adds a dedicated net_stream_plain_kernel instantiation, selected when the serve program is a simple wide/split MLP with a diagonal Gaussian likelihood, 16 rows, and no gate, theta, data or cpost outputs. Inside it, runtime checks for gating, x0 columns, zext/kslice handling, side loads, dense likelihood and optional outputs are removed at compile time, and segment descriptors are prefetched one segment ahead by packing ncg_log2 into the type field. The aim is lower scalar and branch overhead and fewer registers in the hot serve loop. The cost is another kernel variant to maintain, plus eligibility logic that must exactly match the pruned assumptions, with a global toggle that is on by default.

New measurement: 75.49 million evals/s (median of 6 runs). +3.1%, better.

```diff
diff --git a/include/linna_hip.h b/include/linna_hip.h
--- a/include/linna_hip.h
+++ b/include/linna_hip.h
@@ -163,6 +163,9 @@
 int linna_logprob_grad_precision(const linna_logprob_t* lp, int* out);
 int linna_engine_rows(int rows);
 int linna_dense_tri(int mode);
+int linna_serve_plain(int on);
+int linna_program_plain(const linna_layer_t* layers, int nlayers, int in_size, int rows, int dense_nout);
+int linna_logprob_serve_plain(linna_logprob_t* lp, int B, int* out);
 int linna_slice_fusion(int mask);
 int linna_program_describe(const linna_layer_t* layers, int nlayers, int in_size, int rows, int dense_nout, char* buf,
                            size_t n);
diff --git a/linna_amd/_lib.py b/linna_amd/_lib.py
--- a/linna_amd/_lib.py
+++ b/linna_amd/_lib.py
@@ -127,6 +127,9 @@
     "linna_logprob_grad_precision": (_I, [_V, _V]),
     "linna_engine_rows": (_I, [_I]),
     "linna_dense_tri": (_I, [_I]),
+    "linna_serve_plain": (_I, [_I]),
+    "linna_program_plain": (_I, [_V, _I, _I, _I, _I]),
+    "linna_logprob_serve_plain": (_I, [_V, _I, _V]),
     "linna_slice_fusion": (_I, [_I]),
     "linna_net_train_launches": (_I, [_V, _I]),
     "linna_net_set_train_precision": (_I, [_V, _I]),
@@ -338,6 +341,13 @@
     return prev
 
 
+def serve_plain(on=-1):
+    prev = load().linna_serve_plain(int(on))
+    if prev < 0:
+        check(prev)
+    return prev
+
+
 def engine_rows(rows=0):
     prev = load().linna_engine_rows(int(rows))
     if prev < 0:
diff --git a/linna_amd/csrc/api.hip b/linna_amd/csrc/api.hip
--- a/linna_amd/csrc/api.hip
+++ b/linna_amd/csrc/api.hip
@@ -926,6 +926,14 @@
     return loglike_dense_impl(w + L.d, ldd, r.B, d.nout, lp->dense(), r.Z, r.ldz, d.nin, d.temperature, w + L.part, r.lnP, stream);
 }
 
+static bool lp_serves_fused(const linna_logprob* lp, bool keep_activations) {
+    const linna_logprob_desc_t& d = lp->d;
+    return !keep_activations && lp->fused_on && lp->packed.ready() && (!d.outmap.cexp || (d.outmap.cpost && d.outmap.cshift2 && !lp->dense_fused));
+}
+static LpRun lp_fused_run(const linna_logprob* lp, const LpRun& r, float* w, const LpLayout& L) {
+    const linna_logprob_desc_t& d = lp->d;
+    return LpRun{r.Z, r.ldz, r.B, d.w ? r.lnP : nullptr, r.gate, r.TH, r.ldt, d.w ? nullptr : w + L.d, ld4(d.nout)};
+}
 static int lp_forward(linna_logprob* lp, const LpRun& r, float* w, const LpLayout& L, void* stream, bool keep_activations) {
     const linna_logprob_desc_t& d = lp->d;
     const int ldx = ld4(d.nin), ldd = ld4(d.nout), B = r.B;
@@ -938,11 +946,11 @@
         TRY(lp_refresh_stream(lp, B, stream, &packed, &rows));
         return lp_launch(lp, packed, rows, r, nullptr, nullptr, stream);
     }
-    if (!keep_activations && lp->fused_on && lp->packed.ready() && (!d.outmap.cexp || (d.outmap.cpost && d.outmap.cshift2 && !lp->dense_fused))) {
+    if (lp_serves_fused(lp, keep_activations)) {
         const float* packed = nullptr; int rows = 16;
         TRY(lp_refresh_stream(lp, B, stream, &packed, &rows));
         if (lp->dense_fused) return lp_launch(lp, packed, rows, r, nullptr, nullptr, stream);
-        TRY(lp_launch(lp, packed, rows, LpRun{r.Z, r.ldz, B, d.w ? r.lnP : nullptr, r.gate, r.TH, r.ldt, d.w ? nullptr : w + L.d, ldd}, nullptr, nullptr, stream));
+        TRY(lp_launch(lp, packed, rows, lp_fused_run(lp, r, w, L), nullptr, nullptr, stream));
         return d.w ? LINNA_OK : lp_likelihood(lp, r, w, L, stream);
     }
     TRY(launch_prior_map_fwd(r.Z, r.ldz, B, d.nin, d.is_flat, d.a1, d.a2, d.log10_flag, d.xmean, d.xstd, w + L.x0, ldx, r.TH, r.ldt, S(stream)));
@@ -1060,6 +1068,26 @@
     NsDense dn{&dummy, (dn_cols + 3) & ~3, nullptr, nullptr, dense_nout < -1 ? 1 : 0, net_stream_dense_tri(-1)};
     if (dn_cols > 0) return net_stream_describe(NS_SERVE_DENSE, layers, nlayers, in_size, &dn, rows, buf, n);
     return net_stream_describe(NS_SERVE, layers, nlayers, in_size, nullptr, rows, buf, n);
+} LINNA_CATCH_INT
+int linna_serve_plain(int on) try {
+    if (on < -1 || on > 1) { set_error("linna_serve_plain: %d (-1 query, 0 or 1)", on); return LINNA_ERR_INVALID; }
+    return net_stream_serve_plain(on);
+} LINNA_CATCH_INT
+int linna_program_plain(const linna_layer_t* layers, int nlayers, int in_size, int rows, int dense_nout) try {
+    if (!layers || nlayers < 1) { set_error("program_plain: bad arguments"); return LINNA_ERR_INVALID; }
+    TRY(check_layers(layers, nlayers, "program_plain"));
+    if (dense_nout != 0) return 0;
+    return net_stream_program_plain(NS_SERVE, layers, nlayers, in_size, nullptr, rows) ? 1 : 0;
+} LINNA_CATCH_INT
+int linna_logprob_serve_plain(linna_logprob_t* lp, int B, int* out) try {
+    if (!lp || !out || B < 1) { set_error("logprob_serve_plain: bad arguments"); return LINNA_ERR_INVALID; }
+    static float dummy[4];
+    const LpRun r = lp_fused_run(lp, LpRun{dummy, 0, B, dummy}, dummy, LpLayout{});
+    const NsDense dn = lp->dense();
+    *out = !lp->bf16() && lp_serves_fused(lp, false) && !lp->dense_fused &&
+           net_stream_takes_plain(lp->kind(), net_layers(lp->net, lp->kind()), lp_output(lp), r.lnP, r.D, r.TH, nullptr, nullptr, r.gate,
+                                  net_stream_rows(B), lp->kind() == NS_SERVE_DENSE ? &dn : nullptr);
+    return LINNA_OK;
 } LINNA_CATCH_INT
 int linna_dense_tri(int mode) try {
     if (mode < -1 || mode > 2) { set_error("linna_dense_tri: %d (-1 query, 0, 1 or 2)", mode); return LINNA_ERR_INVALID; }
diff --git a/linna_amd/csrc/common.h b/linna_amd/csrc/common.h
--- a/linna_amd/csrc/common.h
+++ b/linna_amd/csrc/common.h
@@ -307,6 +307,9 @@
 int launch_net_stream_pack(NsKind kind, const linna_layer_t* layers, int nl, int in_size, float* packed, int rows, const NsDense* dn,
                            hipStream_t s);
 int net_stream_describe(NsKind kind, const linna_layer_t* layers, int nl, int in_size, const NsDense* dn, int rows, char* buf, size_t n);
+int net_stream_serve_plain(int on);
+bool net_stream_program_plain(NsKind kind, const linna_layer_t* layers, int nl, int in_size, const NsDense* dn, int rows);
+bool net_stream_launch_plain_ok(bool cscale, bool cshift, bool w, bool cexp, bool lnP, bool D, bool TH, bool gate);
 struct NsNet { const linna_layer_t* layers; int nl, in_size; };
 struct NsInput { int nin; const int* is_flat; const float* a1; const float* a2; const int* lg; const float* xmean; const float* xstd; };
 struct NsOutput { const float* cscale; const float* cshift; const float* cpost; const float* cshift2; const float* w; float T; };
@@ -374,6 +377,8 @@
                          float eps, hipStream_t s, bool bf = false);
 int launch_net_stream_grad2(const NsNet& net, const float* packed, const float* Z, int ldz, int B, const NsInput& in, const NsOutput& out,
                             float* lnP, const NsGrad& gr, int rows, hipStream_t s, bool bf = false);
+bool net_stream_takes_plain(NsKind kind, const NsNet& net, const NsOutput& out, const float* lnP, const float* D, const float* TH,
+                            const NsMove* mv, const NsGrad* gr, const int* gate, int rows, const NsDense* dn);
 int launch_net_stream(NsKind kind, const NsNet& net, const float* packed, const float* Z, int ldz, int B, const NsInput& in,
                       const NsOutput& out, float* lnP, float* D, int ldd, float* TH, int ldt, const NsMove* mv, const NsGrad* gr,
                       const int* gate, int rows, const NsDense* dn, hipStream_t s);
diff --git a/linna_amd/csrc/net_program.h b/linna_amd/csrc/net_program.h
--- a/linna_amd/csrc/net_program.h
+++ b/linna_amd/csrc/net_program.h
@@ -61,6 +61,7 @@
 typedef std::shared_ptr<const NsProgram> NsProgramRef;
 NsProgramRef ns_program(NsKind kind, const linna_layer_t* layers, int nl, int in_size, const NsDense* dn, int rows);
 
+bool ns_program_plain(const NsProgram& p);
 int ns_seg_cols(const NsProgram& p, const linna_layer_t* layers, int i);
 struct NsGates {
     int gbit[NS_MAXSEG], mbit[NS_MAXSEG];
diff --git a/linna_amd/csrc/net_program.hip b/linna_amd/csrc/net_program.hip
--- a/linna_amd/csrc/net_program.hip
+++ b/linna_amd/csrc/net_program.hip
@@ -402,6 +402,24 @@
     cache.emplace(std::move(key), p);
     return p;
 }
+
+bool ns_program_plain(const NsProgram& p) {
+    if (!p.ok || p.bf || p.dense || p.x0_keep || p.side_f4 || p.nseg_f < 1) return false;
+    for (int i = 0; i < p.nseg_f; ++i) {
+        const NsSeg& g = p.seg[i];
+        if (g.type != NS_WIDE && g.type != NS_SPLIT) return false;
+        if (g.x0_col || (g.type == NS_WIDE && (g.zext || g.kslice))) return false;
+    }
+    return true;
+}
+bool net_stream_program_plain(NsKind kind, const linna_layer_t* layers, int nl, int in_size, const NsDense* dn, int rows) {
+    return kind == NS_SERVE && rows == 16 && ns_program_plain(*ns_program(kind, layers, nl, in_size, dn, rows));
+}
+bool net_stream_launch_plain_ok(bool cscale, bool cshift, bool w, bool cexp, bool lnP, bool D, bool TH, bool gate) {
+    return cscale && cshift && w && !cexp && lnP && !D && !TH && !gate;
+}
+static std::atomic<int> g_serve_plain{1};
+int net_stream_serve_plain(int on) { return on < 0 ? g_serve_plain.load() : g_serve_plain.exchange(on ? 1 : 0); }
 
 int ns_seg_cols(const NsProgram& p, const linna_layer_t* layers, int i) {
     const linna_layer_t& l = layers[p.seg_op[i]];
diff --git a/linna_amd/csrc/net_stream.hip b/linna_amd/csrc/net_stream.hip
--- a/linna_amd/csrc/net_stream.hip
+++ b/linna_amd/csrc/net_stream.hip
@@ -184,25 +184,31 @@
 
 template <int R, int MOVE, bool GRAD, int STORE, int ROWS, bool BF = false>
 __global__ __launch_bounds__(64 * NS_NW, 1) void net_stream_kernel(NsArgs a) {
-    constexpr bool EPS = false;
+    constexpr bool EPS = false, PLAIN = false;
 #include "net_stream_body.inc"
 }
 template <int R, int MOVE, bool GRAD, int STORE, int ROWS, bool BF>
 __global__ __launch_bounds__(64 * NS_NW, 1) void net_stream_eps_kernel(NsArgs a) {
     static_assert(!BF && GRAD && (STORE == 0 || STORE == 2) && MOVE == 0, "the fp32 one-launch gradients only");
-    constexpr bool EPS = true;
+    constexpr bool EPS = true, PLAIN = false;
+#include "net_stream_body.inc"
+}
+template <int R>
+__global__ __launch_bounds__(64 * NS_NW, 1) void net_stream_plain_kernel(NsArgs a) {
+    constexpr int MOVE = 0, STORE = 0, ROWS = 16;
+    constexpr bool GRAD = false, BF = false, EPS = false, PLAIN = true;
 #include "net_stream_body.inc"
 }
 template <int R, int MOVE, bool GRAD, int STORE, int ROWS, bool BF>
 __global__ __launch_bounds__(64 * NS_NW, 1) void net_stream_train_bf16_kernel(NsArgs a) {
     static_assert(BF && GRAD && STORE == 3 && ROWS == 4 && MOVE == 0, "the bf16 training step only");
-    constexpr bool EPS = false;
+    constexpr bool EPS = false, PLAIN = false;
 #include "net_stream_body.inc"
 }
 template <int R, int MOVE, bool GRAD, int STORE, int ROWS, bool BF>
 __global__ __launch_bounds__(64 * NS_NW, 1) void net_stream_slice_bf16_kernel(NsArgs a) {
     static_assert(BF && !GRAD && STORE == 0 && MOVE == 2, "the bf16 slice evaluation only");
-    constexpr bool EPS = false;
+    constexpr bool EPS = false, PLAIN = false;
 #define NS_BODY_SLICE_BF16
 #include "net_stream_body.inc"
 #undef NS_BODY_SLICE_BF16
@@ -210,7 +216,7 @@
 template <int R, int MOVE, bool GRAD, int STORE, int ROWS, bool BF>
 __global__ __launch_bounds__(64 * NS_NW, 1) void net_stream_grad_bf16_kernel(NsArgs a) {
     static_assert(BF && GRAD && STORE == 2 && MOVE == 0, "the bf16 one-launch gradient only");
-    constexpr bool EPS = false;
+    constexpr bool EPS = false, PLAIN = false;
 #define NS_BODY_GRAD_BF16
 #include "net_stream_body.inc"
 #undef NS_BODY_GRAD_BF16
@@ -218,7 +224,7 @@
 template <int R, int MOVE, bool GRAD, int STORE, int ROWS, bool BF>
 __global__ __launch_bounds__(64 * NS_NW, 1) void net_stream_eps_bf16_kernel(NsArgs a) {
     static_assert(BF && GRAD && STORE == 2 && MOVE == 0, "the bf16 one-launch gradient only");
-    constexpr bool EPS = true;
+    constexpr bool EPS = true, PLAIN = false;
 #define NS_BODY_GRAD_BF16
 #include "net_stream_body.inc"
 #undef NS_BODY_GRAD_BF16
@@ -285,7 +291,8 @@
     else return ns_launch<net_stream_kernel<NS_R, MOVE, GRAD, STORE, ROWS, BF>>(a, (B + ROWS - 1) / ROWS + extra, lds_bytes, s, "net_stream launch");
 }
 template <int MOVE, bool GRAD, int STORE = 0, bool BF = false, bool EPS = false>
-static int ns_launch_kernel(const NsArgs& a0, int B, const NsProgram& p, int rows, hipStream_t s, int extra = 0, size_t lds_extra = 0) {
+static int ns_launch_kernel(const NsArgs& a0, int B, const NsProgram& p, int rows, hipStream_t s, int extra = 0, size_t lds_extra = 0,
+                            bool plain = false) {
     const size_t lds = p.lds_for(rows, GRAD) + lds_extra;
 #ifdef NS_STAMPS
     NsArgs a = a0;
@@ -294,6 +301,9 @@
 #else
     const NsArgs& a = a0;
 #endif
+    if constexpr (MOVE == 0 && !GRAD && STORE == 0 && !BF && !EPS) {
+        if (plain && rows == 16) return ns_launch<net_stream_plain_kernel<NS_R>>(a, (B + 15) / 16, lds, s, "net_stream plain launch");
+    }
     if (rows == 4) return ns_launch_rows<MOVE, GRAD, STORE, 4, BF, EPS>(a, B, lds, s, extra);
     if constexpr (BF) {
         if (rows == 8) return ns_launch_rows<MOVE, GRAD, STORE, 8, BF, EPS>(a, B, lds, s, extra);
@@ -463,6 +473,13 @@
     a.gscale = gr.gscale; a.Gout = gr.G; a.ldg = gr.ldg;
     const NsLeap& l = gr.leap;
     a.hm_p = l.P; a.hm_ldp = l.ldp; a.hm_q = l.Q; a.hm_mass = l.mass; a.hm_ek = l.ek; a.hm_ed = l.ed; a.hm_eps = l.eps;
+}
+
+bool net_stream_takes_plain(NsKind kind, const NsNet& net, const NsOutput& out, const float* lnP, const float* D, const float* TH,
+                            const NsMove* mv, const NsGrad* gr, const int* gate, int rows, const NsDense* dn) {
+    if (kind != NS_SERVE || rows != 16 || mv || gr || dn || !net_stream_serve_plain(-1)) return false;
+    if (!net_stream_launch_plain_ok(out.cscale, out.cshift, out.w, out.cpost, lnP, D, TH, gate)) return false;
+    return ns_program_plain(*ns_program(kind, net.layers, net.nl, net.in_size, dn, rows));
 }
 
 int launch_net_stream(NsKind kind, const NsNet& net, const float* packed, const float* Z, int ldz, int B, const NsInput& in,
@@ -510,7 +527,9 @@
         if (a.hm_p && a.hm_eps) return ns_launch_kernel<0, true, 0, false, true>(a, B, p, rows, s);
         return ns_launch_kernel<0, true>(a, B, p, rows, s);
     }
-    return ns_launch_kernel<0, false>(a, B, p, rows, s);
+    const bool plain = net_stream_takes_plain(kind, net, out, lnP, D, TH, mv, gr, gate, rows, dn);
+    if (plain) for (int i = 0; i < a.nseg; ++i) a.seg[i].type |= a.seg[i].ncg_log2 << 8;
+    return ns_launch_kernel<0, false>(a, B, p, rows, s, 0, 0, plain);
 }
 
 int launch_net_stream_store(const NsNet& net, const float* packed, const float* X, int ldx, int B, const NsOpBufs* ops,
diff --git a/linna_amd/csrc/net_stream_body.inc b/linna_amd/csrc/net_stream_body.inc
--- a/linna_amd/csrc/net_stream_body.inc
+++ b/linna_amd/csrc/net_stream_body.inc
@@ -36,7 +36,9 @@
     const int wave = __builtin_amdgcn_readfirstlane(tid >> 6);
     const int li = lane & 15, kq = lane >> 4;
     const int row0 = blockIdx.x * ROWS;
-    if (a.gate && a.gate[0] == 0) return;
+    if constexpr (!PLAIN) {
+        if (a.gate && a.gate[0] == 0) return;
+    }
     int mv_rows = a.B;
     if constexpr (MOVE == 2) {
         if (a.mv_C) {
@@ -93,6 +95,11 @@
         zden = a.t_den[zsrc];
     }
     const int kpad0 = a.kpad0, nin = a.nin, nout = a.nout, nseg = a.nseg;
+    int seg_warm = 0;
+    if constexpr (PLAIN) {
+#pragma unroll
+        for (int i = 1; i < 8; ++i) seg_warm |= a.seg[i].type | a.seg[i].zext;
+    }
     const int nlast = (TRB ? a.nseg_f : nseg) - 2;
     constexpr int ZPRE = 2;
     float zr[ZPRE], za1[ZPRE], za2[ZPRE], zxm[ZPRE], zxs[ZPRE]; int zfl[ZPRE], zlg[ZPRE];
@@ -212,9 +219,13 @@
     for (int i = 0; i < FIN; ++i) {
         const int cc = min(pc0 + i * RG, nout - 1);
         if constexpr (GRAD && !TRB) fgs[i] = a.gscale[cc]; else fgs[i] = 0.f;
+        if constexpr (PLAIN) {
+            fcs[i] = a.cscale[cc]; fct[i] = a.cshift[cc]; fw[i] = a.w[cc];
+        } else {
         const int c1 = a.cscale ? cc : 0, c2 = a.cshift ? cc : 0, c3 = a.w ? cc : 0;
         const float cs = csp[c1], ct = ctp[c2], ww = wtp[c3];
         fcs[i] = a.cscale ? cs : 1.f; fct[i] = a.cshift ? ct : 0.f; fw[i] = a.w ? ww : 0.f;
+        }
     }
 
     const char* const wbase = reinterpret_cast<const char*>(a.packed) + (size_t)wave * a.Gstride * NS_STEP_B;
@@ -350,6 +361,7 @@
         if (prow && pc0 == 0) { lsrc[pr] = zsrc; lden[pr] = zden; }
     }
     float* const lx0 = lden + 16;
+    if constexpr (!PLAIN) {
     if (a.x0_keep && prow) {
 #pragma unroll
         for (int i = 0; i < ZPRE; ++i) {
@@ -357,6 +369,7 @@
             if constexpr (BF) lx0[pr * 64 + c] = c < nin ? act[pr * LD + c] + act[pr * LD + nin + c] : 0.f;
             else lx0[pr * 64 + c] = (c < kpad0) ? act[pr * LD + c] : 0.f;
         }
+    }
     }
     asm volatile("s_waitcnt lgkmcnt(0)" ::: "memory");
     __builtin_amdgcn_s_barrier();
@@ -391,12 +404,18 @@
         if constexpr (DXE) { const int j = __builtin_amdgcn_readfirstlane(si); s_gmask = ka->gmask[j]; s_gmld = ka->gmld[j]; }
         if constexpr (LB) { const int j = __builtin_amdgcn_readfirstlane(si); s_gbit = ka->gbit[j]; s_mbit = ka->mbit[j]; }
     };
+    NsSeg nxp;
+    auto plain_request = [&]() { nxp = ka->seg[__builtin_amdgcn_readfirstlane(min(si + 1, nseg - 1))]; };
+    auto plain_take = [&](const NsSeg& X) {
+        s_type = X.type & 255; s_ncgl = X.type >> 8; kleft = s_steps = X.steps; s_passes = X.passes; s_bias = X.bias_off;
+        s_dst = X.dst_col; s_relu = X.relu; s_kslice = X.kslice; s_zext = X.zext;
+    };
     auto begin_run = [&]() {
         const int arow = SM ? sm_arow : li, ak = AK * (SM ? 4 * sm_achunk : 4 * kq);
 #pragma unroll
         for (int t = 0; t < NACC; ++t) acc[t] = f32x4{0.f, 0.f, 0.f, 0.f};
         if (s_type == NS_WIDE) {
-            const int blk = s_zext < 0 ? (pass ? 15 - wave : wave) : 8 * pass + wave;
+            const int blk = !PLAIN && s_zext < 0 ? (pass ? 15 - wave : wave) : 8 * pass + wave;
             if constexpr (SM) {
                 const float b = lbias[s_bias + 64 * blk + lane];
 #pragma unroll
@@ -408,8 +427,8 @@
                     acc[t] = f32x4{b, b, b, b};
                 }
             }
-            if (s_zext < 0) kleft = s_steps - 4 * blk;
-            ap = act_lds + 4u * (uint32_t)(P * ABUF + arow * LD + ak + (s_zext < 0 ? 64 * blk : (pass ? s_kslice : 0)));
+            if (!PLAIN && s_zext < 0) kleft = s_steps - 4 * blk;
+            ap = act_lds + 4u * (uint32_t)(P * ABUF + arow * LD + ak + (PLAIN ? 0 : s_zext < 0 ? 64 * blk : (pass ? s_kslice : 0)));
         } else {
             ap = act_lds + 4u * (uint32_t)(P * ABUF + arow * LD + ak + (wave >> s_ncgl) * s_kslice);
         }
@@ -422,9 +441,15 @@
         __builtin_amdgcn_s_barrier();
         asm volatile("" ::: "memory");
     };
+    if constexpr (PLAIN) {
+        asm volatile("" :: "s"(seg_warm));
+        plain_take(ka->seg[0]); begin_run(); a_read(Aq[0]); plain_request();
+    }
+    else {
     load_seg();
     begin_run();
     a_read(Aq[0]);
+    }
 
     auto step = [&](auto Uc, auto Refill) {
         constexpr int U = decltype(Uc)::value;
@@ -532,6 +557,7 @@
                 kleft = X.steps;
             };
             auto take_next = [&]() {
+                if constexpr (PLAIN) { plain_take(nxp); return; }
                 take_seg(NX);
                 if constexpr (STORE) { s_gout = nx_gout; s_gld = nx_gld; s_gn = nx_gn; }
                 if constexpr (DXE) { s_gmask = nx_gmask; s_gmld = nx_gmld; }
@@ -539,7 +565,7 @@
             };
             f32x4 sdw[2][NT];
             bool side_next = false;
-            if constexpr (K4) {
+            if constexpr (K4 && !PLAIN) {
 #pragma unroll
                 for (int s2 = 0; s2 < 2; ++s2)
 #pragma unroll
@@ -570,7 +596,7 @@
 #define q_row(q, e) (SM ? 4 * (q) + (e) : 4 * kq + (e))
 #define q_col(q) (SM ? lane : 16 * (q) + li)
             if (s_type == NS_WIDE) {
-                float* const nxt = act + (P ^ 1) * ABUF + s_dst + (s_zext < 0 ? 64 * (pass ? 15 - wave : wave) : 512 * pass + 64 * wave);
+                float* const nxt = act + (P ^ 1) * ABUF + s_dst + (!PLAIN && s_zext < 0 ? 64 * (pass ? 15 - wave : wave) : 512 * pass + 64 * wave);
                 float ty[NQ][4];
                 if constexpr (STORE == 3) {
                     if (si == nlast) {
@@ -684,7 +710,7 @@
                     P ^= 1; pass = 0; ++si;
                     take_next();
                 } else {
-                    kleft = s_zext > 0 ? s_zext : cur_steps;
+                    kleft = !PLAIN && s_zext > 0 ? s_zext : cur_steps;
                     seg_done = false;
                 }
             } else {
@@ -903,7 +929,7 @@
 #undef fin
 #undef q_row
 #undef q_col
-            if (seg_done && si < nseg && s_x0col > 0) {
+            if (!PLAIN && seg_done && si < nseg && s_x0col > 0) {
                 if (prow) {
                     float* const dstp = act + P * ABUF + pr * LD + s_x0col;
 #pragma unroll
@@ -912,7 +938,7 @@
                 }
                 lds_barrier();
             }
-            if constexpr (K4) {
+            if constexpr (K4 && !PLAIN) {
                 if (side_next && seg_done) {
 #pragma unroll
                     for (int t = 0; t < NT; ++t) acc[t] = f32x4{0.f, 0.f, 0.f, 0.f};
@@ -1020,6 +1046,7 @@
             if (si < nseg) {
                 begin_run();
                 a_read(Aq[(U + 1) & 1]);
+                if constexpr (PLAIN) { if (seg_done) plain_request(); }
             }
 #ifdef NS_STAMPS_FINE
             if (fine) { asm volatile("s_waitcnt lgkmcnt(0)" ::: "memory"); NS_STAMP(); }
@@ -1109,11 +1136,11 @@
         float chi = 0.f;
         auto column = [&](int c, float cs, float ct, float ww) {
             float d = F[c] * cs + ct;
-            if (a.cpost) d = expf(d) * a.cpost[c] + a.cshift2[c];
-            if (a.D && rok) a.D[(size_t)(row0 + pr) * a.ldd + c] = isnan(zz) ? zz : d;
+            if (!PLAIN && a.cpost) d = expf(d) * a.cpost[c] + a.cshift2[c];
+            if (!PLAIN && a.D && rok) a.D[(size_t)(row0 + pr) * a.ldd + c] = isnan(zz) ? zz : d;
             chi += (d * ww) * d;
         };
-        if (a.dense) {
+        if (!PLAIN && a.dense) {
             const float* const Dv = a.u_same ? F : act + (P ^ 1) * ABUF + pr * LD;
             const float* const U = a.u_same ? F + a.u_col : F;
             const bool fac = a.dense == 2;
@@ -1128,7 +1155,7 @@
             for (int i = 0; i < FIN; ++i)
                 if (pc0 + i * RG < nout) column(pc0 + i * RG, fcs[i], fct[i], fw[i]);
             for (int c = pc0 + FIN * RG; c < nout; c += RG)
-                column(c, a.cscale ? a.cscale[c] : 1.f, a.cshift ? a.cshift[c] : 0.f, a.w ? a.w[c] : 0.f);
+                column(c, PLAIN || a.cscale ? a.cscale[c] : 1.f, PLAIN || a.cshift ? a.cshift[c] : 0.f, PLAIN || a.w ? a.w[c] : 0.f);
         }
 #pragma unroll
         for (int o = RG / 2; o >= 1; o >>= 1) chi += __shfl_xor(chi, o, 64);
@@ -1137,7 +1164,7 @@
         if constexpr (MOVE == 2) {
             if (a.lnP && pc0 == 0 && prow && row0 + pr < mv_rows) a.lnP[a.mv_C ? grow : row0 + pr] = lnp_new;
         } else {
-            if (a.lnP && (a.w || a.dense) && pc0 == 0 && rok) a.lnP[row0 + pr] = lnp_new;
+            if ((PLAIN || (a.lnP && (a.w || a.dense))) && pc0 == 0 && rok) a.lnP[row0 + pr] = lnp_new;
         }
         if constexpr (MOVE == 1) {
             const bool mv_acc = rok && mv_factor + lnp_new - mv_lnp_old > mv_logu;
@@ -1158,7 +1185,7 @@
                 if (pc0 == 0) a.mv_lps[mv_wk] = mv_acc ? lnp_new : mv_lnp_old;
             }
         }
-        if (a.TH && rok) {
+        if (!PLAIN && a.TH && rok) {
 #pragma unroll
             for (int j = 0; j < ZPRE; ++j)
                 if (pc0 + j * RG < nin) a.TH[(size_t)(row0 + pr) * a.ldt + pc0 + j * RG] = theta[j];
diff --git a/linna_amd/nn.py b/linna_amd/nn.py
--- a/linna_amd/nn.py
+++ b/linna_amd/nn.py
@@ -406,6 +406,13 @@
     return n, buf.value.decode()
 
 
+def program_is_plain(model, rows=16, dense_nout=0):
+    n = _lib.load().linna_program_plain(program_layers(model), len(model.ops), model.in_size, int(rows), int(dense_nout))
+    if n < 0:
+        _lib.check(n)
+    return bool(n)
+
+
 def describe_grad_bf16_program(model, rows=16):
     arr = program_layers(model)
     buf = C.create_string_buffer(8192)
diff --git a/linna_amd/util.py b/linna_amd/util.py
--- a/linna_amd/util.py
+++ b/linna_amd/util.py
@@ -405,6 +405,11 @@
                   theta.stride(0) if theta is not None else 0, _lib.stream())
         return out
 
+    def serves_plain(self, B):
+        out = C.c_int(0)
+        _lib.call("linna_logprob_serve_plain", self._ensure()["handle"], int(B), C.byref(out))
+        return bool(out.value)
+
     def evaluate_with_grad(self, z, out=None, grad=None):
         if self.precision != "fp32" and self._grad_precision == "fp32":
             raise ValueError("Log_prob.evaluate_with_grad: no gradient in %s (serving only); use precision='fp32'" % self.precision)
```
